# oksuman/sorting-fhe

Measured on AMD Instinct MI355X. Metric: encrypted rank-sort homomorphic comparisons/s (N^2 per DirectSort<N>::sort), higher is better.
Workload: dtype u64 (RNS residues, 40/60-bit primes); 1 GPU; directsort_n256_2e16; N=256, ring_dim=65536, mult_depth=34, scale_bits=40, parallelism=replicas x1

## Files before the change

### sorting-fhe_amd/csrc/core/chebyshev.cpp

```cpp
#include <algorithm>
#include <cmath>
#include <cstdio>
#include <cstdlib>
#include <map>

#include "state.h"

namespace lbcrypto {

uint32_t ChebyshevPSDepth(uint32_t d) {
    if (d <= 1) return 1;
    if (d == 2) return 2;
    static const uint32_t ub[] = {5, 13, 27, 59, 119, 247, 495, 1007, 2031, 4031, 8127, 16255, 32511, 65023};
    for (uint32_t i = 0; i < sizeof(ub) / sizeof(ub[0]); ++i)
        if (d <= ub[i]) return 3 + i;
    SFHE_THROW("Chebyshev degree too large");
}

std::vector<double> EvalChebyshevCoefficients(std::function<double(double)> func, double a,
                                              double b, uint32_t degree) {
    if (!degree) SFHE_THROW("degree must be positive");
    const double bMinusA = 0.5 * (b - a), bPlusA = 0.5 * (b + a);
    const double piByDeg = M_PI / (double)degree;
    std::vector<double> fx(degree);
    for (uint32_t j = 0; j < degree; ++j) fx[j] = func(std::cos(piByDeg * (j + 0.5)) * bMinusA + bPlusA);
    const uint64_t P = 4ull * degree;
    std::vector<double> ctab(P);
    for (uint64_t m = 0; m < P; ++m) ctab[m] = std::cos(M_PI * (double)m / (2.0 * degree));
    std::vector<double> c(degree, 0.0);
    const double mult = 2.0 / (double)degree;
    ParallelFor(degree, [&](size_t i) {
        double acc = 0.0;
        uint64_t step = (2ull * i) % P, idx = i % P;
        for (uint32_t j = 0; j < degree; ++j) {
            acc += fx[j] * ctab[idx];
            idx += step;
            if (idx >= P) idx -= P;
        }
        c[i] = acc * mult;
    });
    return c;
}

namespace {

using Ct = Ciphertext<DCRTPoly>;

struct Val {
    bool isConst = true;
    double c = 0.0;
    Ct ct;
    int node = -1;
};

bool psWaves() {
    static const bool on = [] {
        const char* v = std::getenv("SFHE_PS_WAVES");
        return !v || *v != '0';
    }();
    return on;
}

class PSEvaluator {
  public:
    PSEvaluator(CryptoContextImpl<DCRTPoly>* cc, const Ct& y, uint32_t l, uint32_t D)
        : cc(cc), l(l), k(1u << l), D(D) {
        T.resize(k + 1);
        T[1] = y;
        for (uint32_t half = 1; half < k; half *= 2) {
            const uint32_t lo = half + 1, hi = std::min(k, 2 * half);
            std::vector<Ct> as, bs;
            for (uint32_t j = lo; j <= hi; ++j) {
                as.push_back(doubled(j / 2));
                bs.push_back(j % 2 == 0 ? T[j / 2] : T[j / 2 + 1]);
            }
            std::vector<Ct> prods;
            if (psWaves()) {
                prods = cc->EvalMultMany(as, bs);
            } else {
                for (size_t i = 0; i < as.size(); ++i) prods.push_back(cc->EvalMult(as[i], bs[i]));
            }
            for (uint32_t j = lo; j <= hi; ++j) {
                const Ct& prod = prods[j - lo];
                T[j] = (j % 2 == 0) ? cc->EvalAdd(prod, -1.0) : cc->EvalSub(prod, atLevel(1, prod->GetLevel()));
            }
        }
        giant[l] = T[k];
    }

    void precomputeLeaves(const std::vector<double>& p, uint32_t depth) {
        std::vector<std::pair<std::vector<double>, uint32_t>> leaves;
        plan(p, depth, 0, leaves);
        std::map<uint32_t, std::vector<size_t>> byLevel;
        for (size_t i = 0; i < leaves.size(); ++i) byLevel[leaves[i].second].push_back(i);
        pre.assign(leaves.size(), nullptr);
        for (auto& kv : byLevel) {
            const uint32_t L = kv.first;
            std::vector<uint32_t> js;
            for (uint32_t j = 1; j <= k; ++j)
                for (size_t i : kv.second)
                    if (j < leaves[i].first.size() && leaves[i].first[j] != 0.0) {
                        js.push_back(j);
                        break;
                    }
            std::vector<const uint64_t*> ins0, ins1;
            std::vector<double> sc;
            std::vector<DeviceBufferPtr> keep;
            for (uint32_t j : js) {
                const Ct& t = T[j];
                const uint64_t *r0, *r1;
                cc->RowsAt(t, L, &r0, &r1, keep);
                ins0.push_back(r0);
                ins1.push_back(r1);
                sc.push_back(t->scale);
            }
            for (size_t b0 = 0; b0 < kv.second.size(); b0 += 64) {
                std::vector<std::vector<double>> w;
                const size_t b1 = std::min(kv.second.size(), b0 + 64);
                for (size_t t = b0; t < b1; ++t) {
                    const auto& pl = leaves[kv.second[t]].first;
                    std::vector<double> row;
                    for (uint32_t j : js) row.push_back(j < pl.size() ? pl[j] : 0.0);
                    w.push_back(std::move(row));
                }
                auto cts = cc->LinearWSumRescaleMulti(ins0, ins1, w, L, T[1]->GetSlots(), &sc);
                for (size_t t = b0; t < b1; ++t) pre[kv.second[t]] = cts[t - b0];
            }
        }
        nextLeaf = 0;
    }

    Val eval(std::vector<double> p, uint32_t depth, uint32_t want = 0, int lane = 0, int span = 1) {
        trim(p);
        if (p.empty()) return Val{true, 0.0, nullptr};
        const uint32_t deg = (uint32_t)p.size() - 1;
        if (deg == 0) return Val{true, p[0], nullptr};
        if (deg <= k) return leaf(p, want);
        if (depth >= 1 && deg + (1u << l) <= (1u << (depth - 1))) return eval(p, depth - 1, want, lane, span);
        const uint32_t M = deg >= (1u << (depth - 1)) ? (1u << (depth - 1)) : (1u << (depth - 2));
        std::vector<double> q, r;
        divide(p, M, q, r);
        const uint32_t Lp = productLevel(q, depth, M, want);
        const int half = span / 2;
        if (half) cc->SetLane(lane + half);
        Val qv = eval(q, depth - 1, Lp - 1, half ? lane + half : lane, half ? half : 1);
        const Ct& TM = alignedPower(M, Lp - 1);
        Val out;
        out.isConst = false;
        if (qv.isConst)
            out.ct = cc->EvalMult(TM, qv.c);
        else
            out.ct = cc->EvalMult(qv.ct, TM);
        if (half) cc->SetLane(lane);
        Val rv = eval(r, depth, Lp, lane, half ? half : 1);
        if (std::getenv("SFHE_PS_DEBUG"))
            std::fprintf(stderr, "PSNODE deg %u M %u | q %s lvl %d | TM lvl %u | prod lvl %u | r %s lvl %d\n", deg, M,
                         qv.isConst ? "const" : "ct", qv.isConst ? -1 : (int)qv.ct->GetLevel(), TM->GetLevel(),
                         out.ct->GetLevel(), rv.isConst ? "const" : "ct", rv.isConst ? -1 : (int)rv.ct->GetLevel());
        if (rv.isConst) {
            if (rv.c != 0.0) out.ct = cc->EvalAdd(out.ct, rv.c);
        } else {
            out.ct = cc->EvalAdd(out.ct, rv.ct);
        }
        return out;
    }

    Val build(std::vector<double> p, uint32_t depth, uint32_t want = 0) {
        trim(p);
        if (p.empty()) return Val{true, 0.0, nullptr};
        const uint32_t deg = (uint32_t)p.size() - 1;
        if (deg == 0) return Val{true, p[0], nullptr};
        if (deg <= k) return leaf(p, want);
        if (depth >= 1 && deg + (1u << l) <= (1u << (depth - 1))) return build(p, depth - 1, want);
        const uint32_t M = deg >= (1u << (depth - 1)) ? (1u << (depth - 1)) : (1u << (depth - 2));
        std::vector<double> q, r;
        divide(p, M, q, r);
        const uint32_t Lp = productLevel(q, depth, M, want);
        Node nd;
        nd.q = build(q, depth - 1, Lp - 1);
        nd.r = build(r, depth, Lp);
        nd.M = M;
        nd.Lp = Lp;
        nodes.push_back(std::move(nd));
        Val v;
        v.isConst = false;
        v.node = (int)nodes.size() - 1;
        return v;
    }

    Val run(const Val& root) {
        if (root.node < 0) return root;
        auto ready = [&](const Val& v) { return v.isConst || v.node < 0 || nodes[v.node].hasOut; };
        auto value = [&](const Val& v) -> const Ct& { return v.node < 0 ? v.ct : nodes[v.node].out; };
        while (!nodes[root.node].hasOut) {
            bool progress = false;
            std::map<std::pair<uint32_t, uint32_t>, std::vector<size_t>> waves;
            for (size_t i = 0; i < nodes.size(); ++i)
                if (!nodes[i].hasProd && ready(nodes[i].q)) waves[{nodes[i].M, nodes[i].Lp}].push_back(i);
            for (auto& w : waves) {
                const Ct& TM = alignedPower(w.first.first, w.first.second - 1);
                std::vector<Ct> as, bs;
                std::vector<size_t> which;
                for (size_t i : w.second) {
                    Node& nd = nodes[i];
                    if (nd.q.isConst) {
                        nd.prod = cc->EvalMult(TM, nd.q.c);
                        nd.hasProd = true;
                        continue;
                    }
                    as.push_back(value(nd.q));
                    bs.push_back(TM);
                    which.push_back(i);
                }
                auto prods = cc->EvalMultMany(as, bs);
                for (size_t t = 0; t < which.size(); ++t) {
                    nodes[which[t]].prod = prods[t];
                    nodes[which[t]].hasProd = true;
                }
                progress = true;
            }
            std::vector<Node*> sums;
            for (auto& nd : nodes)
                if (!nd.hasOut && nd.hasProd && ready(nd.r)) sums.push_back(&nd);
            for (size_t b0 = 0; b0 < sums.size(); b0 += batchWidth()) {
                const size_t b1 = std::min(sums.size(), b0 + batchWidth());
                BatchScope bs(cc, (uint32_t)(b1 - b0));
                for (size_t t = b0; t < b1; ++t) {
                    Node& nd = *sums[t];
                    bs.lane((uint32_t)(t - b0));
                    if (nd.r.isConst)
                        nd.out = nd.r.c != 0.0 ? cc->EvalAdd(nd.prod, nd.r.c) : nd.prod;
                    else
                        nd.out = cc->EvalAdd(nd.prod, value(nd.r));
                    nd.hasOut = true;
                    nd.prod = nullptr;
                }
                progress = true;
            }
            if (!progress) SFHE_THROW("internal: Chebyshev wave evaluation stalled");
        }
        Val out;
        out.isConst = false;
        out.ct = nodes[root.node].out;
        nodes.clear();
        return out;
    }

  private:
    struct Node {
        Val q, r;
        uint32_t M = 0, Lp = 0;
        Ct prod, out;
        bool hasProd = false, hasOut = false;
    };
    std::vector<Node> nodes;

    static void divide(const std::vector<double>& p, uint32_t M, std::vector<double>& q, std::vector<double>& r) {
        const uint32_t deg = (uint32_t)p.size() - 1;
        q.assign(deg - M + 1, 0.0);
        r.assign(p.begin(), p.begin() + M);
        for (uint32_t j = M; j <= deg; ++j) {
            if (j == M) {
                q[0] += p[j];
            } else {
                q[j - M] += 2.0 * p[j];
                r[2 * M - j] -= p[j];
            }
        }
    }

    void plan(std::vector<double> p, uint32_t depth, uint32_t want,
              std::vector<std::pair<std::vector<double>, uint32_t>>& leaves) {
        trim(p);
        if (p.size() <= 1) return;
        const uint32_t deg = (uint32_t)p.size() - 1;
        if (deg <= k) {
            const int lv = leafSumLevel(p, want);
            if (lv >= 0) leaves.emplace_back(p, (uint32_t)lv);
            return;
        }
        if (depth >= 1 && deg + (1u << l) <= (1u << (depth - 1))) return plan(p, depth - 1, want, leaves);
        const uint32_t M = deg >= (1u << (depth - 1)) ? (1u << (depth - 1)) : (1u << (depth - 2));
        std::vector<double> q, r;
        divide(p, M, q, r);
        const uint32_t Lp = productLevel(q, depth, M, want);
        plan(q, depth - 1, Lp - 1, leaves);
        plan(r, depth, Lp, leaves);
    }

    uint32_t productLevel(const std::vector<double>& q, uint32_t depth, uint32_t M, uint32_t want) const {
        if (naturalOnly()) want = 0;
        const int nq = natural(q, depth - 1);
        const uint32_t nat = (uint32_t)std::max(nq, (int)powerLevel(M)) + 1;
        return std::max(nat, want);
    }

    int natural(std::vector<double> p, uint32_t depth) const {
        trim(p);
        if (p.size() <= 1) return -1;
        const uint32_t deg = (uint32_t)p.size() - 1;
        if (deg <= k) {
            const int lv = leafSumLevel(p, 0);
            return lv < 0 ? -1 : lv + 1;
        }
        if (depth >= 1 && deg + (1u << l) <= (1u << (depth - 1))) return natural(p, depth - 1);
        const uint32_t M = deg >= (1u << (depth - 1)) ? (1u << (depth - 1)) : (1u << (depth - 2));
        std::vector<double> q, r;
        divide(p, M, q, r);
        const int lp = (int)productLevel(q, depth, M, 0);
        return std::max(lp, natural(r, depth));
    }

    int leafSumLevel(const std::vector<double>& p, uint32_t want) const {
        if (naturalOnly()) want = 0;
        int lev = -1;
        for (uint32_t j = 1; j < p.size(); ++j)
            if (p[j] != 0.0) lev = std::max(lev, (int)T[j]->GetLevel());
        if (lev < 0) return -1;
        return std::max(lev, (int)want - 1);
    }

    static bool naturalOnly() {
        static const bool on = [] {
            const char* v = std::getenv("SFHE_PS_NATURAL");
            return v && *v == '1';
        }();
        return on;
    }

    static void trim(std::vector<double>& p) {
        while (!p.empty() && p.back() == 0.0) p.pop_back();
    }

    uint32_t powerLevel(uint32_t M) const {
        if (M <= k) return T[M]->GetLevel();
        return powerLevel(M / 2) + 1;
    }

    const Ct& power(uint32_t M) {
        if (M <= k) return T[M];
        uint32_t i = (uint32_t)__builtin_ctz(M);
        auto it = giant.find(i);
        if (it != giant.end()) return it->second;
        const Ct& half = power(M / 2);
        const Ct twice = cc->EvalAdd(half, half);
        return giant[i] = cc->EvalAdd(cc->EvalMult(twice, half), -1.0);
    }

    const Ct& doubled(uint32_t j) {
        auto it = twice.find(j);
        if (it != twice.end()) return it->second;
        return twice[j] = cc->EvalAdd(T[j], T[j]);
    }

    const Ct& alignedPower(uint32_t M, uint32_t level) {
        const Ct& t = power(M);
        if (t->GetLevel() >= level) return t;
        auto key = std::make_pair(M, level);
        auto it = alignedPow.find(key);
        if (it != alignedPow.end()) return it->second;
        return alignedPow[key] = cc->AdjustLevel(t, level);
    }

    const Ct& atLevel(uint32_t j, uint32_t level) {
        auto key = std::make_pair(j, level);
        auto it = aligned.find(key);
        if (it != aligned.end()) return it->second;
        return aligned[key] = (T[j]->GetLevel() == level ? T[j] : cc->AdjustLevel(T[j], level));
    }

    Val leaf(const std::vector<double>& p, uint32_t want) {
        if (!pre.empty()) {
            bool any = false;
            for (uint32_t j = 1; j < p.size(); ++j) any = any || p[j] != 0.0;
            if (!any) return Val{true, p[0], nullptr};
            if (nextLeaf >= pre.size()) SFHE_THROW("internal: Chebyshev leaf plan mismatch");
            Val out;
            out.isConst = false;
            out.ct = pre[nextLeaf];
            pre[nextLeaf++] = nullptr;
            if (p[0] != 0.0) out.ct = cc->EvalAdd(out.ct, p[0]);
            return out;
        }
        const int lv = leafSumLevel(p, want);
        if (lv < 0) return Val{true, p[0], nullptr};
        std::vector<const uint64_t*> ins0, ins1;
        std::vector<double> w, sc;
        std::vector<DeviceBufferPtr> keep;
        for (uint32_t j = 1; j < p.size(); ++j) {
            if (p[j] == 0.0) continue;
            const Ct& t = T[j];
            const uint64_t *r0, *r1;
            cc->RowsAt(t, (uint32_t)lv, &r0, &r1, keep);
            ins0.push_back(r0);
            ins1.push_back(r1);
            w.push_back(p[j]);
            sc.push_back(t->scale);
        }
        Val out;
        out.isConst = false;
        out.ct = cc->LinearWSumRescale(ins0, ins1, w, (uint32_t)lv, T[1]->GetSlots(), &sc);
        if (p[0] != 0.0) out.ct = cc->EvalAdd(out.ct, p[0]);
        return out;
    }

    CryptoContextImpl<DCRTPoly>* cc;
    uint32_t l, k, D;
    std::vector<Ct> pre;
    size_t nextLeaf = 0;
    std::vector<Ct> T;
    std::map<uint32_t, Ct> giant;
    std::map<std::pair<uint32_t, uint32_t>, Ct> aligned, alignedPow;
    std::map<uint32_t, Ct> twice;
};

}

Ciphertext<DCRTPoly> CryptoContextImpl<DCRTPoly>::EvalChebyshevSeriesPS(
    const Ciphertext<DCRTPoly>& x, const std::vector<double>& coeffs, double a, double b) {
    OpLock g(st.get());
    static const bool lazyPs = [] {
        const char* v = std::getenv("SFHE_LAZY_PS");
        return v && *v == '1';
    }();
    struct Hold {
        SfheContextState* s;
        bool on;
        ~Hold() {
            if (on) --s->lazyHold;
        }
    } hold{st.get(), !lazyPs};
    if (hold.on) ++st->lazyHold;
    std::vector<double> p(coeffs);
    while (!p.empty() && p.back() == 0.0) p.pop_back();
    if (p.empty()) SFHE_THROW("empty Chebyshev series");
    p[0] *= 0.5;
    Ciphertext<DCRTPoly> y = x;
    if (a != -1.0 || b != 1.0) {
        y = EvalMult(x, 2.0 / (b - a));
        y = EvalAdd(y, -(a + b) / (b - a));
    }
    const uint32_t d = (uint32_t)p.size() - 1;
    if (d == 0) return EvalAdd(EvalMult(y, 0.0), p[0]);
    const uint32_t D = ChebyshevPSDepth(d);
    uint32_t bestL = 1;
    double bestCost = 1e300;
    for (uint32_t l = 1; l + 1 <= D && l <= 6; ++l) {
        if ((1ull << D) - (1ull << l) < d) continue;
        double cost = (double)((1u << l) - 1) + (double)(D - 1 - l) + std::ceil((double)d / (1u << l));
        if (cost < bestCost) {
            bestCost = cost;
            bestL = l;
        }
    }
    static const uint32_t forceL = [] {
        const char* v = std::getenv("SFHE_PS_L");
        return v ? (uint32_t)std::atoi(v) : 0u;
    }();
    if (forceL && d >= 64 && (1ull << D) - (1ull << forceL) >= d && forceL + 1 <= D) bestL = forceL;
    const uint32_t l = std::min(bestL, (uint32_t)(31 - __builtin_clz(std::max<uint32_t>(d, 2))));
    Ciphertext<DCRTPoly> out;
    {
        static const int psLanes = [] {
            const char* v = std::getenv("SFHE_PS_LANES");
            return v ? std::atoi(v) : 0;
        }();
        int lanes = 1;
        if (psLanes > 1 && !st->forkedLanes && d >= 64) {
            lanes = std::min(psLanes, LaneCount());
            lanes = lanes >= 4 ? 4 : (lanes >= 2 ? 2 : 1);
        }
        struct LaneRegion {
            CryptoContextImpl<DCRTPoly>* cc;
            int lanes;
            LaneRegion(CryptoContextImpl<DCRTPoly>* c, int k) : cc(c), lanes(k) {
                if (lanes > 1) cc->ForkLanes(lanes);
            }
            ~LaneRegion() {
                if (lanes > 1) {
                    cc->SetLane(0);
                    cc->JoinLanes();
                }
            }
        } region(this, lanes);
        PSEvaluator ps(this, y, l, D);
        static const bool batched = std::getenv("SFHE_PS_UNBATCHED") == nullptr;
        if (batched) ps.precomputeLeaves(p, D);
        auto v = (lanes == 1 && psWaves()) ? ps.run(ps.build(p, D)) : ps.eval(p, D, 0, 0, lanes);
        out = v.isConst ? EvalAdd(EvalMult(y, 0.0), v.c) : v.ct;
    }
    const uint32_t target = y->GetLevel() + D;
    if (out->GetLevel() > target)
        SFHE_THROW("internal: Chebyshev evaluation exceeded OpenFHE depth");
    if (out->GetLevel() < target) out = AdjustLevel(out, target);
    return out;
}

Ciphertext<DCRTPoly> CryptoContextImpl<DCRTPoly>::EvalChebyshevFunction(
    std::function<double(double)> f, const Ciphertext<DCRTPoly>& x, double a, double b,
    uint32_t degree) {
    auto c = EvalChebyshevCoefficients(f, a, b, degree + 1);
    return EvalChebyshevSeriesPS(x, c, a, b);
}

Ciphertext<DCRTPoly> CryptoContextImpl<DCRTPoly>::EvalPolyLinear(
    const Ciphertext<DCRTPoly>& x, const std::vector<double>& coeffs) {
    OpLock g(st.get());
    std::vector<double> p(coeffs);
    while (!p.empty() && p.back() == 0.0) p.pop_back();
    if (p.size() < 2) SFHE_THROW("EvalPolyLinear needs degree >= 1");
    const uint32_t d = (uint32_t)p.size() - 1;
    std::vector<char> need(d + 1, 0);
    for (uint32_t j = d; j >= 1; --j)
        if (p[j] != 0.0 || need[j]) {
            need[j] = 1;
            if (j >= 2) need[j / 2] = need[j - j / 2] = 1;
        }
    std::vector<Ciphertext<DCRTPoly>> pw(d + 1);
    pw[1] = x;
    for (uint32_t half = 1; half < d; half *= 2) {
        std::vector<Ciphertext<DCRTPoly>> as, bs;
        std::vector<uint32_t> js;
        for (uint32_t j = half + 1; j <= std::min(d, 2 * half); ++j)
            if (need[j]) {
                as.push_back(pw[j / 2]);
                bs.push_back(pw[j - j / 2]);
                js.push_back(j);
            }
        if (psWaves()) {
            auto prods = EvalMultMany(as, bs);
            for (size_t t = 0; t < js.size(); ++t) pw[js[t]] = prods[t];
        } else {
            for (size_t t = 0; t < js.size(); ++t) pw[js[t]] = EvalMult(as[t], bs[t]);
        }
    }
    uint32_t lev = 0;
    for (uint32_t j = 1; j <= d; ++j)
        if (p[j] != 0.0) lev = std::max(lev, pw[j]->GetLevel());
    std::vector<const uint64_t*> i0, i1;
    std::vector<double> w, sc;
    std::vector<DeviceBufferPtr> keep;
    for (uint32_t j = 1; j <= d; ++j) {
        if (p[j] == 0.0) continue;
        const uint64_t *r0, *r1;
        RowsAt(pw[j], lev, &r0, &r1, keep);
        i0.push_back(r0);
        i1.push_back(r1);
        w.push_back(p[j]);
        sc.push_back(pw[j]->scale);
    }
    auto out = LinearWSumRescale(i0, i1, w, lev, x->GetSlots(), &sc);
    if (p[0] != 0.0) out = EvalAdd(out, p[0]);
    return out;
}

}
```

### sorting-fhe_amd/csrc/core/context.cpp

```cpp
#include <algorithm>
#include <atomic>
#include <cmath>
#include <cstdio>
#include <cstdlib>
#include <cstring>
#include <random>

#include "state.h"

namespace lbcrypto {

namespace {

u64 mulmod(u64 a, u64 b, u64 m) { return (u64)((u128)a * b % m); }
u64 powmod(u64 a, u64 e, u64 m) {
    u64 r = 1 % m;
    a %= m;
    while (e) {
        if (e & 1) r = mulmod(r, a, m);
        a = mulmod(a, a, m);
        e >>= 1;
    }
    return r;
}
// ... 333 lines not shown
        if (!lazy(s) || !(isLazy(a) || isLazy(b))) return nullptr;
        const Ct* lz[2] = {&a, &b};
        bool liftIdx[2] = {false, false};
        if (isLazy(a) && isLazy(b)) {
            if (a->level != b->level) return nullptr;
        } else {
            const Ct& c = isLazy(a) ? b : a;
            const Ct& p = isLazy(a) ? a : b;
            if (c->level >= p->level) return nullptr;
            liftIdx[isLazy(a) ? 1 : 0] = true;
        }
        const uint32_t level = a->level > b->level ? a->level : b->level;
        for (int i = 0; i < 2; ++i) {
            materialize(**lz[i], !liftIdx[i]);
            s->dep((*lz[i])->buf.get());
        }
        const uint32_t ell = s->ellOf(level) + 1;
        const sfp_limbs m = s->qmap(ell);
        Ct out = newPendingCt(cc, level, std::max(a->slots, b->slots));
        const uint64_t* x0[2];
        const uint64_t* x1[2];
        std::vector<u64> w(2 * (size_t)m.count);
        DeviceBufferPtr gathered;
        for (int i = 0; i < 2; ++i) {
            const Ct& c = *lz[i];
            x0[i] = c->c0;
            x1[i] = c->c1;
            if (liftIdx[i] && s->shardAt(s->ellOf(c->level)) && !s->shardAt(ell)) {
                gathered = gatherRows(s, c->c0, c->c1, ell);
                x0[i] = gathered->ptr;
                x1[i] = gathered->ptr + (size_t)ell * s->n;
            }
            const std::vector<u64> k = liftIdx[i] ? constResidues(s, s->preScale(level) / c->scale, ell)
                                                  : std::vector<u64>(m.count, 1);
            for (uint32_t r = 0; r < m.count; ++r) {
                const u64 q = s->primes[s->qprime(r, ell)];
                w[(size_t)i * m.count + r] = (sub && i == 1) ? (k[r] ? q - k[r] : 0) : k[r];
            }
        }
        sfp_lin_wsum_multi(s->dev, out->c0, 0, (size_t)(out->c1 - out->c0), x0, x1, 2, w.data(), 1, m);
        s->stats.add++;
        s->countBytes(6.0 * ell * s->n * 8);
        return out;
    }

    static sfp_limbs Q(uint32_t ell) { return sfp_limbs{ell, ell, 0}; }
    static bool packed(const SfheContextState* s, std::initializer_list<const uint64_t*> c0s,
                       std::initializer_list<const uint64_t*> c1s, uint32_t level) {
        const size_t pw = s->polyWords(level);
        auto a = c0s.begin();
        for (auto b = c1s.begin(); b != c1s.end(); ++a, ++b)
            if (*b != *a + pw) return false;
        return true;
    }
    static sfp_limbs both(const SfheContextState* s, uint32_t ell) {
        sfp_limbs m = s->qmap(ell);
        m.count *= 2;
        m.pbase = m.base;
        return m;
    }
    static sfp_limbs Range(uint32_t lo, uint32_t cnt) { return sfp_limbs{cnt, 0, lo}; }

    static Ct newCt(CC* cc, uint32_t level, uint32_t slots) {
        SfheContextState* s = cc->st.get();
        auto ct = std::make_shared<CiphertextImpl<DCRTPoly>>();
        const size_t pw = s->polyWords(level);
        ct->cc = cc->shared_from_this();
        ct->buf = s->alloc(2 * pw);
        ct->c0 = ct->buf->ptr;
        ct->c1 = ct->c0 + pw;
        ct->level = level;
        ct->slots = slots;
        ct->scale = s->scale[level];
        return ct;
    }

    static std::vector<u64> constResidues(SfheContextState* s, double v, uint32_t ell) {
        std::vector<u64> k(s->rows(ell));
        for (uint32_t i = 0; i < k.size(); ++i) k[i] = residueOf(v, s->primes[s->qprime(i, ell)]);
        return k;
    }

    static Ct rescale(CC* cc, const uint64_t* c0, const uint64_t* c1, uint32_t level,
                      uint32_t slots) {
        SfheContextState* s = cc->st.get();
        uint32_t ell = s->ellOf(level);
        if (ell < 2) SFHE_THROW("no levels left to rescale (multiplicative depth exhausted)");
        Ct out = newCt(cc, level + 1, slots);
        if (c1 - c0 < 0) SFHE_THROW("internal: layout");
        if (s->shardAt(ell))
            rescaleShard(s, out->c0, c0, ell, 2, (size_t)(c1 - c0), (size_t)(out->c1 - out->c0));
        else
            sfp_rescale(s->dev, out->c0, c0, ell, s->qInvTable[ell].data(), 2, (size_t)(c1 - c0),
                        (size_t)(out->c1 - out->c0));
        s->stats.rescale++;
        s->countBytes(4.0 * ell * s->n * 8 * 2 / 2);
        return out;
    }

    static Ct adjust(CC* cc, const Ct& ct, uint32_t target, double factor = 1.0) {
        SfheContextState* s = cc->st.get();
        if (target == ct->level && factor == 1.0) return ct;
        if (target <= ct->level && factor != 1.0) SFHE_THROW("a scaled adjustment needs a level to consume");
        if (target < ct->level) SFHE_THROW("cannot raise a ciphertext's level");
        if (target > s->L) SFHE_THROW("target level beyond multiplicative depth");
        uint32_t mid = target - 1;
        uint32_t ell = s->ellOf(mid);
        double K = factor * s->scale[target] * (double)s->primes[ell - 1] / ct->scale;
        auto k = constResidues(s, K, ell);
        s->stats.constmult++;
        s->countBytes(4.0 * ell * s->n * 8);
        if (s->shardAt(s->ellOf(ct->level)) && !s->shardAt(ell)) {
            auto full = gatherRows(s, ct->c0, ct->c1, ell);
            auto v = view(cc, full, full->ptr, full->ptr + (size_t)ell * s->n, ct->level, ct->scale, ct->slots);
            return mulRescale(cc, v, mid, k.data(), nullptr, ct->slots);
        }
        return mulRescale(cc, ct, mid, k.data(), nullptr, ct->slots);
    }

    static bool fusedRescale() {
        static const bool on = [] {
            const char* v = std::getenv("SFHE_FUSED_RESCALE");
            return !v || *v != '0';
        }();
        return on;
    }

    static Ct mulRescale(CC* cc, const Ct& ct, uint32_t level, const u64* k, const uint64_t* m,
                         uint32_t slots) {
        SfheContextState* s = cc->st.get();
        const uint32_t ell = s->ellOf(level);
        if (ell < 2) SFHE_THROW("no levels left to rescale (multiplicative depth exhausted)");
        if (!fusedRescale() || s->shardAt(ell)) {
            const size_t pw = s->polyWords(level);
            auto tmp = s->alloc(2 * pw);
            uint64_t* t0 = tmp->ptr;
            uint64_t* t1 = t0 + pw;
            if (k) {
                sfp_mul_const(s->dev, t0, ct->c0, k, s->qmap(ell));
                sfp_mul_const(s->dev, t1, ct->c1, k, s->qmap(ell));
            } else {
                sfp_mul(s->dev, t0, ct->c0, m, s->qmap(ell));
                sfp_mul(s->dev, t1, ct->c1, m, s->qmap(ell));
            }
            return rescale(cc, t0, t1, level, slots);
        }
        Ct out = newCt(cc, level + 1, slots);
        const size_t inStride = (size_t)(ct->c1 - ct->c0), outStride = (size_t)(out->c1 - out->c0);
        if (k)
            sfp_mul_const_rescale(s->dev, out->c0, ct->c0, k, ell, s->qInvTable[ell].data(), 2, inStride,
                                  outStride);
        else
            sfp_mul_rescale(s->dev, out->c0, ct->c0, m, ell, s->qInvTable[ell].data(), 2, inStride,
                            outStride);
        s->stats.rescale++;
        s->countBytes(4.0 * ell * s->n * 8 * 2 / 2);
        return out;
    }

    static void align(CC* cc, Ct& a, Ct& b) {
        uint32_t l = std::max(a->level, b->level);
        a = adjust(cc, a, l);
        b = adjust(cc, b, l);
    }

    static std::vector<uint32_t> naturalOrder(const SfheContextState* s, uint32_t count, uint32_t per,
                                              uint32_t blocks = 1, uint32_t block = 0) {
        std::vector<uint32_t> r(count);
        for (uint32_t g = 0; g < count; ++g)
            r[g] = ((g % s->world) * blocks + block) * per + g / s->world;
        return r;
    }

    static DeviceBufferPtr gatherRows(SfheContextState* s, const uint64_t* c0, const uint64_t* c1, uint32_t ell) {
// ... 231 lines not shown
        const uint32_t lo = s->owned(ell - 1);
        std::vector<u64> qlinv(lo);
        for (uint32_t i = 0; i < lo; ++i) qlinv[i] = s->qInvTable[ell][s->qprimeShard(i)];
        if (s->shardAt(ell - 1)) {
            sfp_rescale_rows(s->dev, out, in, last->ptr, drop, s->shardMap(ell - 1), qlinv.data(), npoly, inStride,
                             outStride, n);
            return;
        }
        const uint32_t per = (ell - 1 + s->world - 1) / s->world;
        auto mine = s->alloc((size_t)npoly * per * n);
        sfp_rescale_rows(s->dev, mine->ptr, in, last->ptr, drop, s->shardMap(ell - 1), qlinv.data(), npoly, inStride,
                         (size_t)per * n, n);
        auto all = s->alloc((size_t)npoly * per * s->world * n);
        sfp_allgather(s->dev, mine->ptr, all->ptr, (size_t)npoly * per * n * 8);
        for (uint32_t p = 0; p < npoly; ++p) {
            auto idx = naturalOrder(s, ell - 1, per, npoly, p);
            sfp_gather_rows(s->dev, out + p * outStride, all->ptr, idx.data(), ell - 1);
        }
    }

    static Ct localize(CC* cc, const Ct& full) {
        SfheContextState* s = cc->st.get();
        const uint32_t ell = s->ellOf(full->level);
        if (!s->shardAt(ell)) return full;
        const uint32_t lr = s->rows(ell);
        Ct out = newCt(cc, full->level, full->slots);
        out->scale = full->scale;
        std::vector<uint32_t> idx(lr);
        for (uint32_t i = 0; i < lr; ++i) idx[i] = s->qprimeShard(i);
        sfp_gather_rows(s->dev, out->c0, full->c0, idx.data(), lr);
        sfp_gather_rows(s->dev, out->c1, full->c1, idx.data(), lr);
        return out;
    }

    static DeviceBufferPtr gatherFull(SfheContextState* s, const Ct& a) {
        const uint32_t ell = s->ellOf(a->level);
        if (s->shardAt(ell)) return gatherRows(s, a->c0, a->c1, ell);
        auto full = s->alloc((size_t)2 * ell * s->n);
        sfp_d2d(s->dev, full->ptr, a->c0, (size_t)ell * s->n * 8);
        sfp_d2d(s->dev, full->ptr + (size_t)ell * s->n, a->c1, (size_t)ell * s->n * 8);
        return full;
    }

    static int modupInner(CC* cc, uint64_t* acc, const uint64_t* d, uint32_t ell, const DeviceBufferPtr& key,
                          const uint64_t* fold0, const uint64_t* fold1, u64 foldK, int accum,
                          uint32_t invFrom = ~0u) {
        SfheContextState* s = cc->st.get();
        const uint32_t n = s->n, K = s->Kof(key->ksTier);
        const uint32_t beta = (ell + s->alpha - 1) / s->alpha;
        const size_t stride = (size_t)(ell + K) * n;
        auto ext = s->alloc(stride * beta);
        auto scratch = s->alloc((size_t)ell * n);
        auto& convs = modupConv(cc, ell, key->ksTier);
        if (sfp_modup_inner(s->dev, acc, acc + stride, d, ell, K, s->Lq, s->alpha, convs.data(), key->ptr, fold0,
                            fold1, foldK, accum, invFrom, ext->ptr, scratch->ptr) == 0)
            return invFrom != ~0u;
        sfp_modup(s->dev, ext->ptr, d, ell, K, s->Lq, s->alpha, convs.data(), scratch->ptr);
        if (fold0)
            sfp_ks_inner_fold(s->dev, acc, acc + stride, ext->ptr, stride, key->ptr, beta, ell, K, s->Lq, fold0, fold1,
                              foldK);
        else
            (accum ? sfp_ks_inner_acc : sfp_ks_inner)(s->dev, acc, acc + stride, ext->ptr, stride, key->ptr, beta,
                                                       ell, K, s->Lq);
        return 0;
    }

    static void keySwitch(CC* cc, const uint64_t* d, uint32_t ell, const DeviceBufferPtr& key,
                          uint64_t* out0, uint64_t* out1, int add0, int add1) {
        SfheContextState* s = cc->st.get();
        if (s->shardAt(ell)) return keySwitchShard(cc, d, ell, key, out0, out1, add0, add1);
        const int tier = key->ksTier;
        const uint32_t n = s->n, K = s->Kof(tier);
        const uint32_t beta = (ell + s->alpha - 1) / s->alpha;
        const size_t stride = (size_t)(ell + K) * n;
        auto acc = s->alloc(2 * stride);
        const int rowDone = modupInner(cc, acc->ptr, d, ell, key, nullptr, nullptr, 0, 0, ell);
        auto md = s->alloc((size_t)2 * ell * n);
        sfp_moddown2(s->dev, out0, out1, acc->ptr, stride, ell, K, s->Lq, s->moddownConvOf(tier), s->pInvModQof(tier),
                     add0, add1, md->ptr, rowDone);
        s->stats.keyswitch++;
        s->countBytes((3.0 * ell + 2.0 * beta * (ell + K)) * n * 8);
    }

    static Ct relinRescale(CC* cc, uint64_t* d0, uint64_t* d1, const uint64_t* d2, uint32_t level,
                           uint32_t slots) {
        SfheContextState* s = cc->st.get();
        const uint32_t ell = s->ellOf(level);
        if (ell < 2) SFHE_THROW("no levels left to rescale (multiplicative depth exhausted)");
        if (s->shardAt(ell)) {
            keySwitchShard(cc, d2, ell, s->relinKey, d0, d1, 1, 1);
            return rescale(cc, d0, d1, level, slots);
        }
        const DeviceBufferPtr& key = s->relinFor(ell);
        const int tier = key->ksTier;
        const uint32_t n = s->n, K = s->Kof(tier);
        const uint32_t beta = (ell + s->alpha - 1) / s->alpha;
        const size_t stride = (size_t)(ell + K) * n;
        auto acc = s->alloc(2 * stride);
        const int rowDone = modupInner(cc, acc->ptr, d2, ell, key, d0, d1, s->pModQof(tier)[ell - 1], 0, ell - 1);
        Ct out = newCt(cc, level + 1, slots);
        auto scratch = s->alloc((size_t)2 * (ell - 1) * n);
        sfp_moddown_rescale(s->dev, out->c0, out->c1, d0, d1, acc->ptr, stride, ell, K, s->Lq,
                            s->moddownConvOf(tier), s->pInvModQof(tier), s->pModQof(tier),
                            s->qInvTable[ell].data(), scratch->ptr, rowDone);
        s->stats.keyswitch++;
        s->stats.rescale++;
        s->countBytes((3.0 * ell + 2.0 * beta * (ell + K)) * n * 8);
        s->countBytes(4.0 * ell * n * 8);
        return out;
    }

    static Ct multRelinRescale(CC* cc, const uint64_t* a0, const uint64_t* a1, const uint64_t* b0,
                               const uint64_t* b1, uint32_t level, uint32_t slots) {
        SfheContextState* s = cc->st.get();
        const uint32_t ell = s->ellOf(level);
        if (ell < 2) SFHE_THROW("no levels left to rescale (multiplicative depth exhausted)");
        const size_t pw = s->polyWords(level);
        if (!s->shardAt(ell)) {
            const DeviceBufferPtr& key = s->relinFor(ell);
            const int tier = key->ksTier;
            const uint32_t n = s->n, K = s->Kof(tier), beta = (ell + s->alpha - 1) / s->alpha;
            const size_t stride = (size_t)(ell + K) * n;
            Ct out = newCt(cc, level + 1, slots);
            auto acc = s->alloc(2 * stride);
            auto ext = s->alloc(stride * beta);
            auto scratch = s->alloc((size_t)2 * ell * n);
            auto& convs = modupConv(cc, ell, tier);
            if (sfp_mult_relin_rescale(s->dev, out->c0, out->c1, a0, a1, b0, b1, ell, K, s->Lq, s->alpha,
                                       convs.data(), key->ptr, s->moddownConvOf(tier), s->pInvModQof(tier),
                                       s->pModQof(tier), s->qInvTable[ell].data(), acc->ptr, ext->ptr,
                                       scratch->ptr) == 0) {
                s->stats.keyswitch++;
                s->stats.rescale++;
                s->countBytes((3.0 * ell + 2.0 * beta * (ell + K)) * n * 8);
                s->countBytes(4.0 * ell * n * 8);
                return out;
            }
        }
        auto t = s->alloc(3 * pw);
        uint64_t* d0 = t->ptr;
        uint64_t* d1 = d0 + pw;
        uint64_t* d2 = d1 + pw;
        sfp_tensor(s->dev, d0, d1, d2, a0, a1, b0, b1, s->qmap(ell));
        return relinRescale(cc, d0, d1, d2, level, slots);
    }

    static std::vector<Ct> multRelinRescaleMany(CC* cc, const std::vector<const CiphertextImpl<DCRTPoly>*>& a,
                                                const std::vector<const CiphertextImpl<DCRTPoly>*>& b, uint32_t level,
                                                const std::vector<uint32_t>& slots) {
        SfheContextState* s = cc->st.get();
        const size_t cnt = a.size();
        const uint32_t ell = s->ellOf(level);
        std::vector<Ct> out(cnt);
        if (ell < 2) SFHE_THROW("no levels left to rescale (multiplicative depth exhausted)");
        const DeviceBufferPtr& key = s->relinFor(ell);
        const int tier = key->ksTier;
        const uint32_t n = s->n, K = s->Kof(tier), beta = (ell + s->alpha - 1) / s->alpha;
        const size_t stride = (size_t)(ell + K) * n;
        auto& convs = modupConv(cc, ell, tier);
        size_t done = 0;
        {
        BatchScope bs(cc, s->shardAt(ell) ? 0 : (uint32_t)cnt);
        if (bs) {
            for (; done < cnt; ++done) {
                out[done] = newCt(cc, level + 1, slots[done]);
                auto acc = s->alloc(2 * stride);
                auto ext = s->alloc(stride * beta);
                auto scratch = s->alloc((size_t)2 * ell * n);
                bs.lane((uint32_t)done);
                if (sfp_mult_relin_rescale(s->dev, out[done]->c0, out[done]->c1, a[done]->c0, a[done]->c1,
                                           b[done]->c0, b[done]->c1, ell, K, s->Lq, s->alpha, convs.data(),
                                           key->ptr, s->moddownConvOf(tier), s->pInvModQof(tier), s->pModQof(tier),
                                           s->qInvTable[ell].data(), acc->ptr, ext->ptr, scratch->ptr) != 0)
                    break;
                s->stats.keyswitch++;
                s->stats.rescale++;
                s->countBytes((3.0 * ell + 2.0 * beta * (ell + K)) * n * 8);
                s->countBytes(4.0 * ell * n * 8);
            }
        }
        }
        for (size_t i = done; i < cnt; ++i)
            out[i] = multRelinRescale(cc, a[i]->c0, a[i]->c1, b[i]->c0, b[i]->c1, level, slots[i]);
        return out;
    }

    static void innerAndModDown(CC* cc, const uint64_t* ext, size_t stride, uint32_t beta,
                                uint32_t ell, const DeviceBufferPtr& key, uint64_t* out0,
                                uint64_t* out1, int add0, int add1, uint32_t gal = 0) {
        SfheContextState* s = cc->st.get();
        if (s->shardAt(ell)) {
            if (gal) SFHE_THROW("internal: a permuted inner product at a sharded level");
            return innerModDownShard(s, ext, stride, beta, ell, key, out0, out1, add0, add1);
        }
        const int tier = key->ksTier;
        const uint32_t n = s->n, K = s->Kof(tier);
        const size_t accStride = (size_t)(ell + K) * n;
        if (stride != accStride) SFHE_THROW("internal: extended digits of another special-prime tier");
        auto acc = s->alloc(2 * accStride);
        if (gal)
            sfp_ks_inner_aut(s->dev, acc->ptr, acc->ptr + accStride, ext, stride, key->ptr, beta, ell, K, s->Lq, gal);
        else
            sfp_ks_inner(s->dev, acc->ptr, acc->ptr + accStride, ext, stride, key->ptr, beta, ell, K, s->Lq);
        auto scratch = s->alloc((size_t)2 * ell * n);
        sfp_moddown2(s->dev, out0, out1, acc->ptr, accStride, ell, K, s->Lq, s->moddownConvOf(tier),
                     s->pInvModQof(tier), add0, add1, scratch->ptr, 0);
    }

    static std::vector<sfp_conv*>& modupConv(CC* cc, uint32_t ell, int tier = -1) {
        SfheContextState* s = cc->st.get();
        auto& cache = tier < 0 ? s->modupConv : s->tiers[(size_t)tier].modupConv;
        auto it = cache.find(ell);
        if (it != cache.end()) return it->second;
        std::vector<sfp_conv*> v;
        const uint32_t K = s->Kof(tier);
        uint32_t beta = (ell + s->alpha - 1) / s->alpha;
        for (uint32_t j = 0; j < beta; ++j) {
            uint32_t lo = j * s->alpha, hi = std::min(lo + s->alpha, ell);
            std::vector<uint32_t> src, dst, row;
            for (uint32_t i = lo; i < hi; ++i) src.push_back(i);
            for (uint32_t i = 0; i < ell; ++i)
                if (i < lo || i >= hi) dst.push_back(i);
            for (uint32_t k = 0; k < K; ++k) dst.push_back(s->Lq + k);
            for (uint32_t p : dst) row.push_back(p < s->Lq ? p : ell + (p - s->Lq));
            v.push_back(makeConv(s, src, dst, row.data()));
        }
        return cache[ell] = v;
    }

    static void buildTiers(SfheContextState* s) {
        const char* v = std::getenv("SFHE_KS_TIERS");
        const std::string spec = v ? v : "2,4,6,8,10";
        std::vector<uint32_t> bounds;
        for (size_t i = 0; i < spec.size();) {
            size_t j = spec.find(',', i);
            if (j == std::string::npos) j = spec.size();
            const long b = std::strtol(spec.substr(i, j - i).c_str(), nullptr, 10);
            if (b > 0) bounds.push_back((uint32_t)b);
            i = j + 1;
        }
        std::sort(bounds.begin(), bounds.end());
        for (uint32_t b : bounds) {
            if (b > s->alpha || b > s->Lq) break;
            double bits = 0;
            for (uint32_t i = 0; i < b; ++i) bits += std::log2((double)s->primes[i]);
            uint32_t K = 0;
            for (double bp = 0; bp < bits + 20.0 && K < s->K; ++K) bp += std::log2((double)s->primes[s->Lq + K]);
            if (K + 1 >= s->K || (!s->tiers.empty() && K <= s->tiers.back().K)) continue;
            KsTier t;
            t.maxEll = b;
            t.K = K;
            t.pModQ.resize(s->Lq);
            t.pInvModQ.resize(s->Lq);
            for (uint32_t i = 0; i < s->Lq; ++i) {
                const u64 qi = s->primes[i];
                u64 pr = 1;
                for (uint32_t k = 0; k < K; ++k) pr = mulmod(pr, s->primes[s->Lq + k] % qi, qi);
                t.pModQ[i] = pr;
                t.pInvModQ[i] = invmod(pr, qi);
            }
            std::vector<uint32_t> src, dst;
            for (uint32_t k = 0; k < K; ++k) src.push_back(s->Lq + k);
            for (uint32_t i = 0; i < s->Lq; ++i) dst.push_back(i);
            t.moddownConv = makeConv(s, src, dst);
            s->tiers.push_back(std::move(t));
        }
// ... 1473 lines not shown
    const uint64_t* m = SfheInternal::encoded(this, p, a->level);
    return SfheInternal::traced(
        this, SfheInternal::mulRescale(this, a, a->level, nullptr, m, std::max(a->slots, p->slots)), "EvalMult");
}

void CryptoContextImpl<DCRTPoly>::EvalMultInPlace(Ciphertext<DCRTPoly>& a, const Plaintext& p) {
    a = EvalMult(a, p);
}

Ciphertext<DCRTPoly> CryptoContextImpl<DCRTPoly>::EvalMult(const Ciphertext<DCRTPoly>& a0,
                                                          const Ciphertext<DCRTPoly>& b0) {
    OpLock g(st.get());
    SfheInternal::deps(st.get(), {&a0, &b0});
    SfheContextState* s = st.get();
    if (!s->relinKey) SFHE_THROW("EvalMultKeyGen must be called before EvalMult");
    auto a = a0, b = b0;
    SfheInternal::align(this, a, b);
    const uint32_t ell = s->ellOf(a->level);
    if (ell < 2) SFHE_THROW("no levels left (multiplicative depth exhausted)");
    const size_t pw = s->polyWords(a->level);
    s->stats.tensor++;
    s->countBytes(7.0 * ell * s->n * 8);
    const uint32_t slots = std::max(a->slots, b->slots);
    if (SfheInternal::lazy(s) && SfheInternal::fusedRescale()) {
        auto op = std::make_shared<DeferredRelin>();
        op->pa = a->buf;
        op->pb = b->buf;
        op->a0 = a->c0;
        op->a1 = a->c1;
        op->b0 = b->c0;
        op->b1 = b->c1;
        op->level = a->level;
        op->slots = slots;
        return SfheInternal::deferredCt(this, a->level + 1, slots, op);
    }
    if (SfheInternal::fusedRescale())
        return SfheInternal::traced(
            this, SfheInternal::multRelinRescale(this, a->c0, a->c1, b->c0, b->c1, a->level, slots), "EvalMult");
    auto t = s->alloc(3 * pw);
    uint64_t* d0 = t->ptr;
    uint64_t* d1 = d0 + pw;
    uint64_t* d2 = d1 + pw;
    sfp_tensor(s->dev, d0, d1, d2, a->c0, a->c1, b->c0, b->c1, st->qmap(ell));
    SfheInternal::keySwitch(this, d2, ell, s->relinFor(ell), d0, d1, 1, 1);
    return SfheInternal::traced(this, SfheInternal::rescale(this, d0, d1, a->level, slots), "EvalMult");
}

Ciphertext<DCRTPoly> CryptoContextImpl<DCRTPoly>::EvalSquare(const Ciphertext<DCRTPoly>& a) {
    return EvalMult(a, a);
}

std::vector<Ciphertext<DCRTPoly>> CryptoContextImpl<DCRTPoly>::EvalMultMany(
    const std::vector<Ciphertext<DCRTPoly>>& a0, const std::vector<Ciphertext<DCRTPoly>>& b0) {
    OpLock g(st.get());
    SfheContextState* s = st.get();
    if (a0.size() != b0.size()) SFHE_THROW("operand count mismatch");
    const size_t cnt = a0.size();
    std::vector<Ciphertext<DCRTPoly>> out(cnt);
    if (cnt < 2 || !SfheInternal::fusedRescale()) {
        for (size_t i = 0; i < cnt; ++i) out[i] = EvalMult(a0[i], b0[i]);
        return out;
    }
    if (!s->relinKey) SFHE_THROW("EvalMultKeyGen must be called before EvalMult");
    std::vector<Ciphertext<DCRTPoly>> A(a0), B(b0);
    for (size_t i = 0; i < cnt; ++i) {
        SfheInternal::deps(s, {&a0[i], &b0[i]});
        SfheInternal::align(this, A[i], B[i]);
        if (s->ellOf(A[i]->level) < 2) SFHE_THROW("no levels left (multiplicative depth exhausted)");
        s->stats.tensor++;
        s->countBytes(7.0 * s->ellOf(A[i]->level) * s->n * 8);
    }
    for (size_t i = 0; i < cnt;) {
        size_t j = i + 1;
        while (j < cnt && j - i < batchWidth() && A[j]->level == A[i]->level) ++j;
        std::vector<const CiphertextImpl<DCRTPoly>*> pa, pb;
        std::vector<uint32_t> slots;
        for (size_t k = i; k < j; ++k) {
            pa.push_back(A[k].get());
            pb.push_back(B[k].get());
            slots.push_back(std::max(A[k]->slots, B[k]->slots));
        }
        auto r = SfheInternal::multRelinRescaleMany(this, pa, pb, A[i]->level, slots);
        for (size_t k = i; k < j; ++k) out[k] = SfheInternal::traced(this, r[k - i], "EvalMult");
        i = j;
    }
    return out;
}

Ciphertext<DCRTPoly> CryptoContextImpl<DCRTPoly>::EvalMultAddPlain(
    const std::vector<Ciphertext<DCRTPoly>>& a, const std::vector<Plaintext>& p) {
    OpLock g(st.get());
    SfheInternal::depsv(st.get(), a);
    SfheContextState* s = st.get();
    if (a.empty() || a.size() != p.size()) SFHE_THROW("operand count mismatch");
    uint32_t level = 0, slots = 0;
    for (size_t i = 0; i < a.size(); ++i) {
        level = std::max(level, a[i]->level);
        slots = std::max(slots, std::max(a[i]->slots, p[i]->slots));
    }
    const uint32_t ell = s->ellOf(level);
    if (ell < 2) SFHE_THROW("no levels left (multiplicative depth exhausted)");
    std::vector<Ciphertext<DCRTPoly>> al(a.size());
    std::vector<const uint64_t*> x0, x1, m;
    for (size_t i = 0; i < a.size(); ++i) {
        al[i] = SfheInternal::adjust(this, a[i], level);
        x0.push_back(al[i]->c0);
        x1.push_back(al[i]->c1);
    }
    s->stats.ptmult += a.size();
    if (SfheInternal::lazy(s)) {
        auto op = std::make_shared<DeferredMacPlain>();
        for (auto& c : al) op->pins.push_back(c->buf);
        op->x0 = x0;
        op->x1 = x1;
        op->pts = p;
        op->level = level;
        op->slots = slots;
        s->countBytes((3.0 * a.size() + 2.0) * ell * s->n * 8);
        return SfheInternal::deferredCt(this, level + 1, slots, op);
    }
    SfheInternal::encodeBatch(this, p, level);
    for (size_t i = 0; i < a.size(); ++i) m.push_back(SfheInternal::encoded(this, p[i], level));
    const size_t pw = s->polyWords(level);
    auto tmp = s->alloc(2 * pw);
    uint64_t* t0 = tmp->ptr;
    uint64_t* t1 = t0 + pw;
    for (size_t done = 0; done < a.size(); done += SFP_MAX_WSUM) {
        uint32_t take = (uint32_t)std::min<size_t>(SFP_MAX_WSUM, a.size() - done);
        if (done == 0) {
            sfp_mac_plain2(s->dev, t0, t1, x0.data(), x1.data(), m.data(), take, st->qmap(ell));
        } else {
            auto part = s->alloc(2 * pw);
            sfp_mac_plain2(s->dev, part->ptr, part->ptr + pw, x0.data() + done, x1.data() + done,
                           m.data() + done, take, st->qmap(ell));
            sfp_add(s->dev, t0, t0, part->ptr, st->qmap(ell));
            sfp_add(s->dev, t1, t1, part->ptr + pw, st->qmap(ell));
        }
    }
    s->countBytes((3.0 * a.size() + 2.0) * ell * s->n * 8);
    return SfheInternal::traced(this, SfheInternal::rescale(this, t0, t1, level, slots), "EvalMultAddPlain");
}


Ciphertext<DCRTPoly> CryptoContextImpl<DCRTPoly>::EvalRotate(const Ciphertext<DCRTPoly>& a,
                                                            int32_t r) {
    OpLock g(st.get());
    SfheContextState* s = st.get();
    if (!(SfheInternal::lazy(s) && SfheInternal::isLazy(a))) SfheInternal::deps(s, {&a});
    uint32_t gal = GaloisForRotation(r);
    if (gal == 1) return a->Clone();
    if (!s->rotKeys.count(gal))
        SFHE_THROW("EvalKey for index [" + std::to_string(gal) + "] (rotation " +
                   std::to_string(r) + ") is not found");
    const bool pend = SfheInternal::lazy(s) && SfheInternal::isLazy(a);
    if (pend) {
        SfheInternal::materialize(*a, true);
        s->dep(a->buf.get());
    }
    const uint32_t ell = SfheInternal::ctEll(s, *a);
    auto out = pend ? SfheInternal::newPendingCt(this, a->level, a->slots) : SfheInternal::newCt(this, a->level, a->slots);
    auto t = s->alloc((size_t)s->rows(ell) * s->n);
    sfp_automorph(s->dev, out->c0, a->c0, gal, st->qmap(ell));
    sfp_automorph(s->dev, t->ptr, a->c1, gal, st->qmap(ell));
    s->stats.automorph++;
    s->countBytes(3.0 * ell * s->n * 8);
    SfheInternal::keySwitch(this, t->ptr, ell, *s->rotFor(gal, ell), out->c0, out->c1, 1, 0);
// ... 257 lines not shown
                auto scratch = s->alloc((size_t)ell * n);
                sfp_modup(s->dev, ext->ptr, a[t]->c1, ell, K, s->Lq, s->alpha,
                          SfheInternal::modupConv(this, ell).data(), scratch->ptr);
            }
            auto rc0 = s->alloc(pw);
            sfp_automorph(s->dev, rc0->ptr, a[t]->c0, gal, q);
            x0.push_back(rc0->ptr);
            m0.push_back(m);
            keep.push_back(rc0);
            static const bool autFused = [] {
                const char* v = std::getenv("SFHE_KS_AUT");
                return !v || *v != '0';
            }();
            if (autFused) {
                sfp_ks_inner_mul_aut(s->dev, acc->ptr, acc->ptr + stride, ext->ptr, stride, it->second->ptr, beta, ell,
                                     K, s->Lq, SfheInternal::encodedExt(this, pt, level), accOn ? 1 : 0, gal);
            } else {
                auto rext = s->alloc(stride * beta);
                const uint32_t rows = beta * (ell + K);
                sfp_automorph(s->dev, rext->ptr, ext->ptr, gal, sfp_limbs{rows, rows, 0, 0});
                sfp_ks_inner_mul(s->dev, acc->ptr, acc->ptr + stride, rext->ptr, stride, it->second->ptr, beta, ell,
                                 K, s->Lq, SfheInternal::encodedExt(this, pt, level), accOn ? 1 : 0);
            }
            accOn = true;
            s->stats.keyswitch++;
            s->stats.automorph++;
            s->countBytes((3.0 * ell + (2.0 * beta + 5.0) * (ell + K)) * n * 8);
        }
    }
    auto macInto = [&](uint64_t* out, const std::vector<const uint64_t*>& x, const std::vector<const uint64_t*>& m) {
        if (x.empty()) {
            sfp_zero(s->dev, out, pw * 8);
            return;
        }
        for (size_t done = 0; done < x.size(); done += SFP_MAX_WSUM) {
            const uint32_t take = (uint32_t)std::min<size_t>(SFP_MAX_WSUM, x.size() - done);
            if (done == 0) {
                sfp_mac_plain(s->dev, out, x.data(), m.data(), take, q);
            } else {
                auto part = s->alloc(pw);
                sfp_mac_plain(s->dev, part->ptr, x.data() + done, m.data() + done, take, q);
                sfp_add(s->dev, out, out, part->ptr, q);
            }
        }
    };
    macInto(t0, x0, m0);
    macInto(t1, x1, m1);
    s->stats.ptmult += x0.size() + x1.size();
    s->countBytes((2.0 * x0.size() + 2.0 * x1.size() + 2.0) * ell * n * 8);
    if (accOn) {
        auto scratch = s->alloc((size_t)2 * ell * n);
        sfp_moddown2(s->dev, t0, t1, acc->ptr, stride, ell, K, s->Lq, s->moddownConv, s->pInvModQ.data(), 1, 1,
                     scratch->ptr, 0);
    }
    return SfheInternal::traced(this, SfheInternal::rescale(this, t0, t1, level, slots), "EvalRotMultAddHoisted");
}


namespace {
void weightResidues(const SfheContextState* s, double w, uint32_t level, uint32_t ell,
                    std::vector<uint64_t>& kk, double inScale = 0.0) {
    const double K = inScale > 0.0 ? w * s->scale[level] * (s->scale[level] / inScale) : w * s->scale[level];
    const double r = std::nearbyint(K);
    const bool neg = r < 0;
    const double a = std::fabs(r);
    u128 v;
    if (a < 1.8e19) {
        v = (u128)(u64)a;
    } else {
        const double hi = std::floor(std::ldexp(a, -64));
        v = ((u128)(u64)hi << 64) + (u128)(u64)(a - std::ldexp(hi, 64));
    }
    for (uint32_t i = 0; i < s->rows(ell); ++i) {
        const u64 q = s->primes[s->qprime(i, ell)];
        const u64 m = (u64)(v % q);
        kk.push_back(neg ? (m ? q - m : 0) : m);
    }
}
}

std::vector<Ciphertext<DCRTPoly>> CryptoContextImpl<DCRTPoly>::LinearWSumRescaleMulti(
    const std::vector<const uint64_t*>& in0, const std::vector<const uint64_t*>& in1,
    const std::vector<std::vector<double>>& w, uint32_t level, uint32_t slots, const std::vector<double>* inScale) {
    OpLock g(st.get());
    SfheContextState* s = st.get();
    const uint32_t ell = s->ellOf(level), n = s->n;
    const uint32_t nin = (uint32_t)in0.size(), nout = (uint32_t)w.size();
    if (ell < 2) SFHE_THROW("no levels left (multiplicative depth exhausted)");
    if (nin == 0 || nin > SFP_MAX_WSUM || nout == 0) SFHE_THROW("LinearWSumRescaleMulti: bad sizes");
    if (inScale && inScale->size() != nin) SFHE_THROW("LinearWSumRescaleMulti: scale count");
    std::vector<uint64_t> kk;
    kk.reserve((size_t)nout * nin * s->rows(ell));
    for (const auto& row : w) {
        if (row.size() != nin) SFHE_THROW("LinearWSumRescaleMulti: weight row size");
        for (uint32_t j = 0; j < nin; ++j) weightResidues(s, row[j], level, ell, kk, inScale ? (*inScale)[j] : 0.0);
    }
    const size_t pw = s->polyWords(level);
    auto sums = s->alloc((size_t)nout * 2 * pw);
    sfp_lin_wsum_multi(s->dev, sums->ptr, 2 * pw, pw, in0.data(), in1.data(), nin, kk.data(), nout,
                       s->qmap(ell));
    const size_t qw = s->polyWords(level + 1);
    auto res = s->alloc((size_t)nout * 2 * qw);
    if (s->shardAt(ell))
        SfheInternal::rescaleShard(s, res->ptr, sums->ptr, ell, 2 * nout, pw, qw);
    else
        sfp_rescale(s->dev, res->ptr, sums->ptr, ell, s->qInvTable[ell].data(), 2 * nout, pw, qw);
    std::vector<Ciphertext<DCRTPoly>> out(nout);
    for (uint32_t o = 0; o < nout; ++o) {
        auto ct = std::make_shared<CiphertextImpl<DCRTPoly>>();
        ct->cc = shared_from_this();
        ct->buf = res;
        ct->c0 = res->ptr + (size_t)o * 2 * qw;
        ct->c1 = ct->c0 + qw;
        ct->level = level + 1;
        ct->slots = slots;
        ct->scale = s->scale[level + 1];
        out[o] = ct;
    }
    s->stats.wsum_terms += (uint64_t)nin * nout;
    s->stats.rescale += 2 * nout;
    s->countBytes(((double)nin + nout) * 2.0 * pw * 8 + 4.0 * pw * 8 * nout);
    return out;
}

Ciphertext<DCRTPoly> CryptoContextImpl<DCRTPoly>::LinearWSumRescale(
    const std::vector<const uint64_t*>& in0, const std::vector<const uint64_t*>& in1,
    const std::vector<double>& w, uint32_t level, uint32_t slots, const std::vector<double>* inScale) {
    OpLock g(st.get());
    SfheContextState* s = st.get();
    const uint32_t ell = s->ellOf(level);
    if (ell < 2) SFHE_THROW("no levels left (multiplicative depth exhausted)");
    if (inScale && inScale->size() != w.size()) SFHE_THROW("LinearWSumRescale: scale count");
    const size_t pw = s->polyWords(level);
    auto tmp = s->alloc(2 * pw);
    uint64_t* t0 = tmp->ptr;
    uint64_t* t1 = t0 + pw;
    const sfp_limbs q = s->qmap(ell);
    size_t done = 0;
    bool first = true;
    while (done < w.size()) {
        size_t take = std::min<size_t>(w.size() - done, SFP_MAX_WSUM - (first ? 0 : 1));
        std::vector<const uint64_t*> a0, a1;
        std::vector<uint64_t> kk;
        if (!first) {
            a0.push_back(t0);
            a1.push_back(t1);
            for (uint32_t i = 0; i < s->rows(ell); ++i) kk.push_back(1);
        }
        for (size_t j = done; j < done + take; ++j) {
            a0.push_back(in0[j]);
            a1.push_back(in1[j]);
            weightResidues(s, w[j], level, ell, kk, inScale ? (*inScale)[j] : 0.0);
        }
        sfp_lin_wsum(s->dev, t0, a0.data(), kk.data(), (uint32_t)a0.size(), q);
        sfp_lin_wsum(s->dev, t1, a1.data(), kk.data(), (uint32_t)a1.size(), q);
        s->stats.wsum_terms += take;
        s->countBytes((double)(a0.size() + 1) * 2.0 * ell * s->n * 8);
        done += take;
        first = false;
    }
    return SfheInternal::traced(this, SfheInternal::rescale(this, t0, t1, level, slots), "LinearWSumRescale");
}



Ciphertext<DCRTPoly> CryptoContextImpl<DCRTPoly>::Rescale(const Ciphertext<DCRTPoly>& a) {
    Settle(a);
    return a->Clone();
}

void CryptoContextImpl<DCRTPoly>::Settle(const Ciphertext<DCRTPoly>& ct) {
    if (!ct) return;
    OpLock g(st.get());
    SfheInternal::deps(st.get(), {&ct});
}

void CryptoContextImpl<DCRTPoly>::LevelReduceInPlace(Ciphertext<DCRTPoly>& a, std::nullptr_t,
                                                     size_t levels) {
    a = AdjustLevel(a, a->level + (uint32_t)levels);
}

Ciphertext<DCRTPoly> CryptoContextImpl<DCRTPoly>::AdjustLevel(const Ciphertext<DCRTPoly>& a,
                                                             uint32_t targetLevel) {
    OpLock g(st.get());
    SfheInternal::deps(st.get(), {&a});
    auto r = SfheInternal::adjust(this, a, targetLevel);
    return r == a ? a->Clone() : r;
}

Ciphertext<DCRTPoly> CryptoContextImpl<DCRTPoly>::AdjustLevelScaled(const Ciphertext<DCRTPoly>& a,
                                                                   uint32_t targetLevel, double factor) {
    OpLock g(st.get());
    SfheInternal::deps(st.get(), {&a});
    auto r = SfheInternal::adjust(this, a, targetLevel, factor);
    return r == a ? a->Clone() : r;
}

Ciphertext<DCRTPoly> CryptoContextImpl<DCRTPoly>::ModRaise(const Ciphertext<DCRTPoly>& a) {
    OpLock g(st.get());
    SfheInternal::deps(st.get(), {&a});
    SfheContextState* s = st.get();
    if (s->sharded) SFHE_THROW("bootstrapping a limb-sharded context is not supported");
    if (s->ellOf(a->level) != 1) SFHE_THROW("ModRaise needs a ciphertext at the last level (one limb)");
    const uint32_t n = s->n;
    auto t = s->alloc(2 * (size_t)n);
    sfp_d2d(s->dev, t->ptr, a->c0, (size_t)n * 8);
    sfp_d2d(s->dev, t->ptr + n, a->c1, (size_t)n * 8);
    sfp_ntt(s->dev, t->ptr, sfp_limbs{1, 1, 0, 0, 0}, 1);
    sfp_ntt(s->dev, t->ptr + n, sfp_limbs{1, 1, 0, 0, 0}, 1);
    auto out = SfheInternal::newCt(this, 0, a->slots);
    const size_t pw = s->polyWords(0);
    auto zero = s->alloc(2 * pw);
    sfp_zero(s->dev, zero->ptr, 2 * pw * 8);
    std::vector<uint64_t> minus1(s->Lq);
    for (uint32_t i = 0; i < s->Lq; ++i) minus1[i] = s->primes[i] - 1;
    sfp_rescale_rows(s->dev, out->c0, zero->ptr, t->ptr, 0, s->qmap(s->Lq), minus1.data(), 2, pw,
                     (size_t)(out->c1 - out->c0), n);
    s->wrote(out->buf.get());
    return SfheInternal::traced(this, out, "ModRaise");
}

Ciphertext<DCRTPoly> CryptoContextImpl<DCRTPoly>::EvalConjugate(const Ciphertext<DCRTPoly>& a) {
    OpLock g(st.get());
    SfheInternal::deps(st.get(), {&a});
    SfheContextState* s = st.get();
    const uint32_t gal = 2 * s->n - 1;
    auto it = s->rotKeys.find(gal);
    if (it == s->rotKeys.end()) SFHE_THROW("conjugation key not found (EvalConjugateKeyGen)");
    const uint32_t ell = s->ellOf(a->level);
    auto out = SfheInternal::newCt(this, a->level, a->slots);
    auto t = s->alloc(s->polyWords(a->level));
    sfp_automorph(s->dev, out->c0, a->c0, gal, st->qmap(ell));
    sfp_automorph(s->dev, t->ptr, a->c1, gal, st->qmap(ell));
    s->stats.automorph++;
    SfheInternal::keySwitch(this, t->ptr, ell, it->second, out->c0, out->c1, 1, 0);
    return SfheInternal::traced(this, out, "EvalConjugate");
}

void CryptoContextImpl<DCRTPoly>::EvalConjugateKeyGen(const PrivateKey<DCRTPoly>& sk) {
    OpLock g(st.get());
    SfheContextState* s = st.get();
    const uint32_t gal = 2 * s->n - 1;
    if (s->rotKeys.count(gal)) return;
    const uint32_t NP = s->Lq + s->K;
// ... 256 lines not shown
```

### sorting-fhe_amd/csrc/core/openfhe.h

```cpp
#pragma once

#include <algorithm>
#include <charconv>
#include <complex>
#include <cstddef>
#include <locale>
#include <fstream>
#include <cstdint>
#include <functional>
#include <iostream>
#include <map>
#include <memory>
#include <mutex>
#include <set>
#include <stdexcept>
#include <string>
#include <thread>
#include <vector>

#include "prims.h"

namespace lbcrypto {

using usint = uint32_t;
// ... 203 lines not shown
class CryptoContextImpl<DCRTPoly> : public std::enable_shared_from_this<CryptoContextImpl<DCRTPoly>> {
  public:
    explicit CryptoContextImpl(const CCParams<CryptoContextCKKSRNS>& p);
    ~CryptoContextImpl();

    void Enable(PKESchemeFeature f) { enabled |= f; }
    void Enable(uint32_t mask) { enabled |= mask; }

    uint32_t GetRingDimension() const;
    uint32_t GetCyclotomicOrder() const { return 2 * GetRingDimension(); }
    EncodingParams GetEncodingParams() const;
    uint32_t GetMultiplicativeDepth() const;

    KeyPair<DCRTPoly> KeyGen();
    void EvalMultKeyGen(const PrivateKey<DCRTPoly>& sk);
    void EvalRotateKeyGen(const PrivateKey<DCRTPoly>& sk, const std::vector<int32_t>& idx,
                          const PublicKey<DCRTPoly>& pk = nullptr);
    void EvalAtIndexKeyGen(const PrivateKey<DCRTPoly>& sk, const std::vector<int32_t>& idx) {
        EvalRotateKeyGen(sk, idx);
    }
    void ClearEvalMultKeys();
    void ClearEvalAutomorphismKeys();
    static bool SerializeEvalMultKey(std::ostream& os, SerType::Kind k, const std::string& keyTag = "");
    static bool DeserializeEvalMultKey(std::istream& is, SerType::Kind k);
    static bool SerializeEvalAutomorphismKey(std::ostream& os, SerType::Kind k, const std::string& keyTag = "");
    static bool DeserializeEvalAutomorphismKey(std::istream& is, SerType::Kind k);
    uint64_t Fingerprint() const;
    uint64_t KeyTag() const;
    const CCParams<CryptoContextCKKSRNS>& GetParams() const;
    uint32_t GetEnabledMask() const { return enabled; }

    Plaintext MakeCKKSPackedPlaintext(const std::vector<double>& v, uint32_t scaleDeg = 1,
                                      uint32_t level = 0, const void* params = nullptr,
                                      uint32_t slots = 0) const;
    Plaintext MakeCKKSPackedPlaintext(const std::vector<std::complex<double>>& v,
                                      uint32_t scaleDeg = 1, uint32_t level = 0,
                                      const void* params = nullptr, uint32_t slots = 0) const;
    Ciphertext<DCRTPoly> Encrypt(const PublicKey<DCRTPoly>& pk, const Plaintext& pt);
    Ciphertext<DCRTPoly> Encrypt(const Plaintext& pt, const PublicKey<DCRTPoly>& pk) {
        return Encrypt(pk, pt);
    }
    void Decrypt(const PrivateKey<DCRTPoly>& sk, const Ciphertext<DCRTPoly>& ct, Plaintext* out);
    void Decrypt(const Ciphertext<DCRTPoly>& ct, const PrivateKey<DCRTPoly>& sk, Plaintext* out) {
        Decrypt(sk, ct, out);
    }

    Ciphertext<DCRTPoly> EvalAdd(const Ciphertext<DCRTPoly>& a, const Ciphertext<DCRTPoly>& b);
    Ciphertext<DCRTPoly> EvalAdd(const Ciphertext<DCRTPoly>& a, double c);
    Ciphertext<DCRTPoly> EvalAdd(double c, const Ciphertext<DCRTPoly>& a) { return EvalAdd(a, c); }
    Ciphertext<DCRTPoly> EvalAdd(const Ciphertext<DCRTPoly>& a, const Plaintext& p);
    Ciphertext<DCRTPoly> EvalAdd(const Plaintext& p, const Ciphertext<DCRTPoly>& a) {
        return EvalAdd(a, p);
    }
    void EvalAddInPlace(Ciphertext<DCRTPoly>& a, const Ciphertext<DCRTPoly>& b);
    void EvalAddInPlace(Ciphertext<DCRTPoly>& a, double c);
    void EvalAddInPlace(Ciphertext<DCRTPoly>& a, const Plaintext& p);
    Ciphertext<DCRTPoly> EvalSub(const Ciphertext<DCRTPoly>& a, const Ciphertext<DCRTPoly>& b);
    Ciphertext<DCRTPoly> EvalSub(const Ciphertext<DCRTPoly>& a, double c) { return EvalAdd(a, -c); }
    Ciphertext<DCRTPoly> EvalSub(double c, const Ciphertext<DCRTPoly>& a);
    Ciphertext<DCRTPoly> EvalSub(const Ciphertext<DCRTPoly>& a, const Plaintext& p);
    Ciphertext<DCRTPoly> EvalSub(const Plaintext& p, const Ciphertext<DCRTPoly>& a);
    void EvalSubInPlace(Ciphertext<DCRTPoly>& a, const Ciphertext<DCRTPoly>& b);
    void EvalSubInPlace(Ciphertext<DCRTPoly>& a, double c) { EvalAddInPlace(a, -c); }
    Ciphertext<DCRTPoly> EvalNegate(const Ciphertext<DCRTPoly>& a);
    void EvalNegateInPlace(Ciphertext<DCRTPoly>& a);
    Ciphertext<DCRTPoly> EvalAddMany(const std::vector<Ciphertext<DCRTPoly>>& v);

    Ciphertext<DCRTPoly> EvalMult(const Ciphertext<DCRTPoly>& a, const Ciphertext<DCRTPoly>& b);
    Ciphertext<DCRTPoly> EvalMult(const Ciphertext<DCRTPoly>& a, double c);
    Ciphertext<DCRTPoly> EvalMult(double c, const Ciphertext<DCRTPoly>& a) { return EvalMult(a, c); }
    Ciphertext<DCRTPoly> EvalMult(const Ciphertext<DCRTPoly>& a, const Plaintext& p);
    Ciphertext<DCRTPoly> EvalMult(const Plaintext& p, const Ciphertext<DCRTPoly>& a) {
        return EvalMult(a, p);
    }
    void EvalMultInPlace(Ciphertext<DCRTPoly>& a, double c);
    void EvalMultInPlace(Ciphertext<DCRTPoly>& a, const Plaintext& p);
    Ciphertext<DCRTPoly> EvalMultAndRelinearize(const Ciphertext<DCRTPoly>& a,
                                                const Ciphertext<DCRTPoly>& b) {
        return EvalMult(a, b);
    }
    Ciphertext<DCRTPoly> EvalSquare(const Ciphertext<DCRTPoly>& a);
    std::vector<Ciphertext<DCRTPoly>> EvalMultMany(const std::vector<Ciphertext<DCRTPoly>>& a,
                                                   const std::vector<Ciphertext<DCRTPoly>>& b);
    Ciphertext<DCRTPoly> EvalMultAddPlain(const std::vector<Ciphertext<DCRTPoly>>& a,
                                          const std::vector<Plaintext>& p);

    Ciphertext<DCRTPoly> EvalRotate(const Ciphertext<DCRTPoly>& a, int32_t r);
    Ciphertext<DCRTPoly> EvalAtIndex(const Ciphertext<DCRTPoly>& a, int32_t r) {
        return EvalRotate(a, r);
    }
    std::shared_ptr<FastRotationPrecomp> EvalFastRotationPrecompute(const Ciphertext<DCRTPoly>& a);
    Ciphertext<DCRTPoly> EvalFastRotation(const Ciphertext<DCRTPoly>& a, int32_t r, uint32_t m,
                                          const std::shared_ptr<FastRotationPrecomp>& pre);
    Ciphertext<DCRTPoly> EvalRotateSum(const std::vector<Ciphertext<DCRTPoly>>& a,
                                       const std::vector<int32_t>& r);
    Ciphertext<DCRTPoly> EvalRotMultAddHoisted(
        const std::vector<Ciphertext<DCRTPoly>>& a,
        const std::vector<std::vector<std::pair<int32_t, Plaintext>>>& terms);

    Ciphertext<DCRTPoly> EvalChebyshevSeriesPS(const Ciphertext<DCRTPoly>& x,
                                               const std::vector<double>& coeffs, double a,
                                               double b);
    Ciphertext<DCRTPoly> EvalChebyshevSeries(const Ciphertext<DCRTPoly>& x,
                                             const std::vector<double>& coeffs, double a,
                                             double b) {
        return EvalChebyshevSeriesPS(x, coeffs, a, b);
    }
    Ciphertext<DCRTPoly> EvalChebyshevFunction(std::function<double(double)> f,
                                               const Ciphertext<DCRTPoly>& x, double a, double b,
                                               uint32_t degree);
    Ciphertext<DCRTPoly> EvalPolyLinear(const Ciphertext<DCRTPoly>& x,
                                        const std::vector<double>& coeffs);
    Ciphertext<DCRTPoly> EvalPoly(const Ciphertext<DCRTPoly>& x,
                                  const std::vector<double>& coeffs) {
        return EvalPolyLinear(x, coeffs);
    }

    Ciphertext<DCRTPoly> Rescale(const Ciphertext<DCRTPoly>& a);
    Ciphertext<DCRTPoly> ModReduce(const Ciphertext<DCRTPoly>& a) { return Rescale(a); }
    void LevelReduceInPlace(Ciphertext<DCRTPoly>& a, std::nullptr_t, size_t levels);
    Ciphertext<DCRTPoly> AdjustLevel(const Ciphertext<DCRTPoly>& a, uint32_t targetLevel);
    Ciphertext<DCRTPoly> AdjustLevelScaled(const Ciphertext<DCRTPoly>& a, uint32_t targetLevel, double factor);
    Ciphertext<DCRTPoly> ModRaise(const Ciphertext<DCRTPoly>& a);
    Ciphertext<DCRTPoly> EvalConjugate(const Ciphertext<DCRTPoly>& a);
    void EvalConjugateKeyGen(const PrivateKey<DCRTPoly>& sk);

    void EvalBootstrapSetup(std::vector<uint32_t> levelBudget, std::vector<uint32_t> dim1 = {0, 0},
                            uint32_t slots = 0, uint32_t correctionFactor = 0);
    void EvalBootstrapKeyGen(const PrivateKey<DCRTPoly>& sk, uint32_t slots);
    Ciphertext<DCRTPoly> EvalBootstrap(const Ciphertext<DCRTPoly>& ct, uint32_t numIterations = 1,
                                       uint32_t precision = 0);
    uint32_t GetBootstrapDepth(const std::vector<uint32_t>& levelBudget, uint32_t slots = 0) const;
    Ciphertext<DCRTPoly> BootstrapOnce(const Ciphertext<DCRTPoly>& ct, double inFactor, double outFactor);
    Ciphertext<DCRTPoly> bootstrapIters(const Ciphertext<DCRTPoly>& ct, uint32_t numIterations, uint32_t precision);
    Ciphertext<DCRTPoly> bootstrapReplay(const Ciphertext<DCRTPoly>& ct, uint32_t numIterations, uint32_t precision);
    size_t BootstrapGraphs() const;
    using BootstrapSlotMap = std::map<uint32_t, std::vector<std::complex<double>>>;
    using BootstrapTap =
        std::function<void(const char* stage, const Ciphertext<DCRTPoly>& ct, const BootstrapSlotMap* map)>;
    void SetBootstrapTap(BootstrapTap tap) { bootTap = std::move(tap); }
    static double BootstrapOverflowBound();
    static uint32_t BootstrapDoubleAngles();
    static uint32_t BootstrapChebDegree();

    SfheContextState* state() const { return st.get(); }
    uint32_t GaloisForRotation(int32_t r) const;
    bool HasRotationKey(int32_t r) const;
    Ciphertext<DCRTPoly> LinearWSumRescale(const std::vector<const uint64_t*>& in0,
                                           const std::vector<const uint64_t*>& in1,
                                           const std::vector<double>& w, uint32_t level,
                                           uint32_t slots, const std::vector<double>* inScale = nullptr);
    std::vector<Ciphertext<DCRTPoly>> LinearWSumRescaleMulti(
        const std::vector<const uint64_t*>& in0, const std::vector<const uint64_t*>& in1,
        const std::vector<std::vector<double>>& w, uint32_t level, uint32_t slots,
        const std::vector<double>* inScale = nullptr);
    void Synchronize();
    void Settle(const Ciphertext<DCRTPoly>& ct);
    int LaneCount() const;
    void EnableSharding(int rank, int world, bool shardAtOne = false);
    int ShardRank() const;
    int ShardWorld() const;
    bool IsSharded() const;
    uint32_t ShardTailLimbs() const;
    uint32_t SwitchKeyRows() const;
    void EnableBatchGroups(int group, int groups, bool gatherAtOne = false);
    int BatchGroup() const;
    int BatchGroups() const;
    bool BatchGather() const;
    std::vector<Ciphertext<DCRTPoly>> GatherGroups(const Ciphertext<DCRTPoly>& ct);
    void RowsAt(const Ciphertext<DCRTPoly>& ct, uint32_t level, const uint64_t** c0, const uint64_t** c1,
                std::vector<DeviceBufferPtr>& keep);
    void DownloadRows(const Ciphertext<DCRTPoly>& ct, uint64_t* out);
    void ForkLanes(int count, bool stacked = false);
    bool BeginBatch(uint32_t count);
    void BatchLane(uint32_t i);
    void EndBatch();
    uint32_t BatchWidth() const;
    void SetLane(int lane);
    void JoinLanes();
    void SetPlaintextCache(bool on);
    struct OpStats {
        uint64_t keyswitch = 0, rescale = 0, tensor = 0, ptmult = 0, constmult = 0, add = 0,
                 automorph = 0, ntt_limbs = 0, wsum_terms = 0;
        uint64_t dev_encodes = 0, host_encodes = 0;
        double algo_bytes = 0.0;
        uint64_t pool_bytes = 0;
    };
    OpStats GetOpStats() const;
    void ResetOpStats();
    struct CapturedGraph;
    bool BeginCapture();
    std::shared_ptr<CapturedGraph> EndCapture(const Ciphertext<DCRTPoly>& keep);
    void Launch(const std::shared_ptr<CapturedGraph>& g);
    void ReleaseGraph(CapturedGraph& g);
    static int LiveContexts();
    void releaseBootstrapGraphs();
    size_t GraphNodes(const std::shared_ptr<CapturedGraph>& g) const;
    bool GraphFamilyTime(const std::shared_ptr<CapturedGraph>& g, uint32_t family, int reps, double* ms,
                         uint64_t* launches, double* bytes);
    void CopyCiphertextInto(const Ciphertext<DCRTPoly>& dst, const Ciphertext<DCRTPoly>& src);

  private:
    std::unique_ptr<SfheContextState> st;
    uint32_t enabled = 0;
    BootstrapTap bootTap;
    friend class SfheInternal;
};

class BatchScope {
  public:
    BatchScope(CryptoContextImpl<DCRTPoly>* cc, uint32_t count)
        : cc_(cc), on_(count > 1 && cc->BeginBatch(count)) {}
    ~BatchScope() {
        if (on_) cc_->EndBatch();
    }
    BatchScope(const BatchScope&) = delete;
    BatchScope& operator=(const BatchScope&) = delete;
    explicit operator bool() const { return on_; }
    void lane(uint32_t i) {
        if (on_) cc_->BatchLane(i);
    }

  private:
    CryptoContextImpl<DCRTPoly>* cc_;
    bool on_;
};

void RegisterCryptoContext(const CryptoContext<DCRTPoly>& cc);

#define SFHE_FACADE_ABI_VERSION 5
#ifndef SFHE_LAYOUT_SALT
#define SFHE_LAYOUT_SALT 0
#endif
#pragma GCC diagnostic push
#pragma GCC diagnostic ignored "-Winvalid-offsetof"
inline uint64_t SfheFacadeLayout() {
    uint64_t h = 1469598103934665603ull;
    auto mix = [&h](uint64_t x) { h = (h ^ x) * 1099511628211ull; };
    using Ct = CiphertextImpl<DCRTPoly>;
    using Pk = PublicKeyImpl<DCRTPoly>;
    using Sk = PrivateKeyImpl<DCRTPoly>;
    using Cc = CryptoContextImpl<DCRTPoly>;
    const uint64_t v[] = {
        SFHE_FACADE_ABI_VERSION, SFHE_LAYOUT_SALT,
        sizeof(std::string), sizeof(std::mutex), sizeof(std::shared_ptr<int>), sizeof(std::vector<int>),
        sizeof(std::map<int, int>), sizeof(std::set<int>), sizeof(std::function<void()>), sizeof(std::complex<double>),
        sizeof(CCParams<CryptoContextCKKSRNS>), alignof(CCParams<CryptoContextCKKSRNS>),
        sizeof(EncodingParamsImpl), sizeof(KeyPair<DCRTPoly>),
        sizeof(PlaintextImpl), alignof(PlaintextImpl), offsetof(PlaintextImpl, values), offsetof(PlaintextImpl, slots),
        offsetof(PlaintextImpl, level), offsetof(PlaintextImpl, length), offsetof(PlaintextImpl, logPrecision),
        offsetof(PlaintextImpl, logError), offsetof(PlaintextImpl, realCache), offsetof(PlaintextImpl, encoded),
        offsetof(PlaintextImpl, encMutex),
        sizeof(Ct), alignof(Ct), offsetof(Ct, cc), offsetof(Ct, buf), offsetof(Ct, c0), offsetof(Ct, c1),
        offsetof(Ct, level), offsetof(Ct, slots), offsetof(Ct, scale), offsetof(Ct, def), offsetof(Ct, pend),
        offsetof(Ct, undo), sizeof(Ct::CaptureUndo),
        sizeof(Pk), offsetof(Pk, b), offsetof(Pk, a), offsetof(Pk, cc), offsetof(Pk, tag),
        sizeof(Sk), offsetof(Sk, s), offsetof(Sk, ternary), offsetof(Sk, cc), offsetof(Sk, tag),
        sizeof(FastRotationPrecomp), offsetof(FastRotationPrecomp, ext), offsetof(FastRotationPrecomp, level),
        offsetof(FastRotationPrecomp, pend), offsetof(FastRotationPrecomp, beta), offsetof(FastRotationPrecomp, stride),
        offsetof(FastRotationPrecomp, pinBuf), offsetof(FastRotationPrecomp, pinC0),
        sizeof(Cc), alignof(Cc), sizeof(Cc::OpStats), sizeof(Cc::BootstrapTap),
    };
    for (uint64_t x : v) mix(x);
    return h;
}
#pragma GCC diagnostic pop
void SfheCheckLayout(uint64_t callerStamp);

inline CryptoContext<DCRTPoly> GenCryptoContext(const CCParams<CryptoContextCKKSRNS>& p) {
    SfheCheckLayout(SfheFacadeLayout());
    auto cc = std::make_shared<CryptoContextImpl<DCRTPoly>>(p);
    RegisterCryptoContext(cc);
    return cc;
}

class Serial {
  public:
    static bool Serialize(const CryptoContext<DCRTPoly>& cc, std::ostream& os, SerType::Kind k);
    static bool Deserialize(CryptoContext<DCRTPoly>& cc, std::istream& is, SerType::Kind k);
    static bool Serialize(const PublicKey<DCRTPoly>& pk, std::ostream& os, SerType::Kind k);
    static bool Deserialize(PublicKey<DCRTPoly>& pk, std::istream& is, SerType::Kind k);
    static bool Serialize(const PrivateKey<DCRTPoly>& sk, std::ostream& os, SerType::Kind k);
    static bool Deserialize(PrivateKey<DCRTPoly>& sk, std::istream& is, SerType::Kind k);
    static bool Serialize(const Ciphertext<DCRTPoly>& ct, std::ostream& os, SerType::Kind k);
    static bool Deserialize(Ciphertext<DCRTPoly>& ct, std::istream& is, SerType::Kind k);

    template <class T>
    static bool SerializeToFile(const std::string& path, const T& obj, SerType::Kind k) {
        std::ofstream f(path, std::ios::out | std::ios::binary | std::ios::trunc);
        if (!f.is_open()) return false;
        return Serialize(obj, f, k) && f.good();
    }
    template <class T>
    static bool DeserializeFromFile(const std::string& path, T& obj, SerType::Kind k) {
        std::ifstream f(path, std::ios::in | std::ios::binary);
        if (!f.is_open()) return false;
        return Deserialize(obj, f, k);
    }
};

template <class E>
class CryptoContextFactory {
  public:
// ... 59 lines not shown
```

### sorting-fhe_amd/csrc/core/state.h

```cpp
#pragma once
#include <algorithm>
#include <atomic>
#include <cmath>
#include <cstdlib>
#include <cstring>
#include <map>
#include <mutex>
#include <thread>
#include <unordered_map>
#include <unordered_set>
#include <vector>

#include "modarith.h"
#include "openfhe.h"

namespace lbcrypto {

class DeviceBuffer {
  public:
    DeviceBuffer(SfheContextState* s, uint64_t* p, size_t w, int l, uint64_t r)
        : st(s), ptr(p), words(w), lane(l), region(r) {}
    ~DeviceBuffer();
    SfheContextState* st;
    uint64_t* ptr;
// ... 43 lines not shown
    uint32_t extIdx = 0;
    std::vector<uint64_t> extInvModQ;
    std::vector<uint64_t> extModQ;
    std::vector<sf_barrett> bar;
    std::vector<double> scale;
    sfp_dev* dev = nullptr;

    std::map<uint32_t, std::vector<sfp_conv*>> modupConv;
    sfp_conv* moddownConv = nullptr;
    std::vector<uint64_t> pInvModQ;
    std::vector<uint64_t> pModQ;
    std::vector<std::vector<uint64_t>> qInvTable;
    uint32_t tablePrimes() const { return Lq + K + (ext ? 1 : 0); }

    uint64_t keyTag = 0;
    DeviceBufferPtr relinKey;
    std::map<uint32_t, DeviceBufferPtr> rotKeys;
    std::set<int32_t> rotIndices;
    std::vector<KsTier> tiers;
    bool tiersReady = true;
    int tierAt(uint32_t ell) const {
        if (!tiersReady || shardAt(ell)) return -1;
        for (size_t t = 0; t < tiers.size(); ++t)
            if (ell <= tiers[t].maxEll) return (int)t;
        return -1;
    }
    uint32_t Kof(int t) const { return t < 0 ? K : tiers[(size_t)t].K; }
    const uint64_t* pModQof(int t) const { return t < 0 ? pModQ.data() : tiers[(size_t)t].pModQ.data(); }
    const uint64_t* pInvModQof(int t) const { return t < 0 ? pInvModQ.data() : tiers[(size_t)t].pInvModQ.data(); }
    sfp_conv* moddownConvOf(int t) const { return t < 0 ? moddownConv : tiers[(size_t)t].moddownConv; }
    const DeviceBufferPtr& relinFor(uint32_t ell) const {
        const int t = tierAt(ell);
        return t >= 0 && tiers[(size_t)t].relinKey ? tiers[(size_t)t].relinKey : relinKey;
    }
    const DeviceBufferPtr* rotFor(uint32_t gal, uint32_t ell) const {
        const int t = tierAt(ell);
        if (t >= 0) {
            auto it = tiers[(size_t)t].rotKeys.find(gal);
            if (it != tiers[(size_t)t].rotKeys.end()) return &it->second;
        }
        auto it = rotKeys.find(gal);
        return it == rotKeys.end() ? nullptr : &it->second;
    }
    std::map<uint32_t, std::shared_ptr<BootstrapPrecomp>> boot;

    std::mutex poolMu;
    std::map<size_t, std::vector<uint64_t*>> freeList[SFP_MAX_LANES];
    std::vector<std::pair<size_t, uint64_t*>> deferredFree;
    struct BatchFreed {
        size_t words;
        uint64_t* ptr;
        int lane;
        uint64_t region;
    };
    uint32_t batchDepth = 0;
    std::thread::id batchThread;
    std::vector<BatchFreed> batchFree;
    void poolReturn(size_t words, uint64_t* p, int lane, uint64_t region, int freer);
    std::map<size_t, std::vector<uint64_t*>> forkPool;
    int lane = 0;
    int forkedLanes = 0;
    uint64_t region = 0;
    uint64_t regionCount = 0;
    uint64_t laneSeq[SFP_MAX_LANES] = {};
    uint64_t synced[SFP_MAX_LANES][SFP_MAX_LANES] = {};
    uint64_t regionDepWaits = 0;
    void laneWait(int waiter, int waitee);
    int myLane() const;
    void setMyLane(int l);
    void dep(DeviceBuffer* b);
    void wrote(DeviceBuffer* b);
    size_t poolBytes = 0;

    std::recursive_mutex opMu;

    bool ptCacheOn = true;
    size_t ptCacheBytes = 0;
    size_t ptCacheLimit = (size_t)48 << 30;
    std::unordered_map<uint64_t, std::vector<PtCacheEntry>> ptCache;

    bool capturing = false;
    uint64_t captureEpoch = 0, epochCount = 0;
    uint32_t lazyHold = 0;
    std::set<uint64_t> abandonedEpochs;
    std::vector<std::pair<uint64_t*, size_t>> capAllocs;
    std::unordered_map<uint64_t*, bool> graphOwned;

    std::atomic<uint64_t> seedCounter{1};
    uint64_t seed = 0;
    CryptoContextImpl<DCRTPoly>::OpStats stats;

    int rank = 0, world = 1;
    int bgroup = 0, bgroups = 1;
    bool bgatherAtOne = false;
    bool sharded = false;
    uint32_t tailLimbs = 0;
    bool fullScope = false;
    std::vector<DeviceBufferPtr> scopeKeep;
    sfp_key_geom kgeom{};
    uint32_t keyRows() const { return kgeom.rows ? kgeom.rows : Lq + K; }
    std::map<uint32_t, std::vector<sfp_conv*>> modupConvShard;
    std::map<uint32_t, std::vector<std::pair<sfp_conv*, sfp_conv*>>> modupConvSplit;
    sfp_conv* moddownConvShard = nullptr;

    uint32_t ellOf(uint32_t level) const { return Lq - level; }
    double preScale(uint32_t level) const { return scale[level] * (double)primes[ellOf(level)]; }
    uint32_t owned(uint32_t count) const {
        return (uint32_t)rank < count ? (count - rank + world - 1) / world : 0;
    }
    bool shardAt(uint32_t ell) const { return sharded && ell > tailLimbs; }
    uint32_t rows(uint32_t ell) const { return shardAt(ell) ? owned(ell) : ell; }
    uint32_t prows(uint32_t ell) const { return shardAt(ell) ? owned(K) : K; }
    uint32_t qprime(uint32_t i, uint32_t ell) const { return shardAt(ell) ? rank + i * world : i; }
    uint32_t qprimeShard(uint32_t i) const { return rank + i * world; }
    sfp_limbs shardMap(uint32_t ell) const {
        return sfp_limbs{owned(ell), owned(ell), 0, (uint32_t)rank, (uint32_t)world};
    }
    sfp_limbs qmap(uint32_t ell) const { return shardAt(ell) ? shardMap(ell) : sfp_limbs{ell, ell, 0, 0, 1}; }
    sfp_limbs extmap(uint32_t ell) const {
        return shardAt(ell) ? sfp_limbs{owned(ell) + owned(K), owned(ell), Lq + (uint32_t)rank, (uint32_t)rank,
                                        (uint32_t)world}
                            : sfp_limbs{ell + K, ell, Lq, 0, 1};
    }
    size_t polyWords(uint32_t level) const { return (size_t)rows(ellOf(level)) * n; }
    uint64_t nextSeed() { return seed ^ (0x9E3779B97F4A7C15ULL * (seedCounter++)); }
    DeviceBufferPtr alloc(size_t words);
    void releaseAll();
    void countBytes(double b) { stats.algo_bytes += b; }
};

class FullScope {
  public:
    explicit FullScope(SfheContextState* s)
        : s_(s), rank_(s->rank), world_(s->world), sharded_(s->sharded), was_(s->fullScope) {
        s->rank = 0;
        s->world = 1;
        s->sharded = false;
        s->fullScope = true;
    }
    ~FullScope() {
        s_->rank = rank_;
        s_->world = world_;
        s_->sharded = sharded_;
        s_->fullScope = was_;
        if (!was_) s_->scopeKeep.clear();
    }

  private:
    SfheContextState* s_;
    int rank_, world_;
    bool sharded_, was_;
};

inline uint32_t batchWidth() {
    static const uint32_t w = [] {
        const char* v = std::getenv("SFHE_BATCH_WIDTH");
        const long x = v && *v ? std::strtol(v, nullptr, 10) : SFP_BATCH_MAX;
        return (uint32_t)std::max(2L, std::min<long>(x, SFP_BATCH_MAX));
    }();
    return w;
}

class OpLock {
  public:
    explicit OpLock(SfheContextState* s) : s_(s), g_(s->opMu) {
        s_->lane = s_->myLane();
        sfp_set_lane(s_->dev, s_->lane);
    }

  private:
    SfheContextState* s_;
    std::lock_guard<std::recursive_mutex> g_;
};

static inline uint64_t sf_splitmix64(uint64_t x) {
    x += 0x9E3779B97F4A7C15ULL;
    x = (x ^ (x >> 30)) * 0xBF58476D1CE4E5B9ULL;
    x = (x ^ (x >> 27)) * 0x94D049BB133111EBULL;
    return x ^ (x >> 31);
}

int ckks_encode(const std::vector<std::complex<double>>& v, uint32_t slots, uint32_t n,
                double scale, std::vector<int64_t>& coeffs);
void ckks_decode(const std::vector<double>& coeffs, uint32_t slots, uint32_t n,
                 std::vector<std::complex<double>>& out);
void ckks_encoder_tables(uint32_t n, const uint64_t** rot, const double** ksi);

}
```

### sorting-fhe_amd/csrc/hip/prims_hip.hip

```cpp
#include <hip/hip_runtime.h>
#include <dlfcn.h>
#include <rccl/rccl.h>

#include <algorithm>
#include <cstdio>
#include <cstdlib>
#include <cstring>
#include <functional>
#include <map>
#include <memory>
#include <mutex>
#include <unordered_set>
#include <unordered_map>
#include <string>
#include <type_traits>
#include <vector>

#include "../modarith.h"
#include "../prims.h"

#define SFP_CHECK(call)                                                     \
    do {                                                                    \
        hipError_t e_ = (call);                                             \
        if (e_ != hipSuccess) record(d, #call, e_);                          \
// ... 549 lines not shown
            }
        }
#pragma unroll
        for (int j = 0; j < M; ++j) s[a0 ^ ldsOff<COL>(j * h, Cc)] = v[j];
    }
}

template <bool INV, bool COL, int LE, int TILE>
__device__ __forceinline__ void nttRoundDynFP(int b, double* s, const NttTile& T, uint32_t S0, uint32_t k0,
                                              double q, const double* w, double qinv) {
    if constexpr (LE >= 4) {
        if (b == 4) return nttRoundFP<INV, COL, LE, 4, TILE>(s, T, S0, k0, q, w, qinv);
    }
    if constexpr (LE >= 3) {
        if (b == 3) return nttRoundFP<INV, COL, LE, 3, TILE>(s, T, S0, k0, q, w, qinv);
    }
    if (b == 2) return nttRoundFP<INV, COL, LE, 2, TILE>(s, T, S0, k0, q, w, qinv);
    nttRoundFP<INV, COL, LE, 1, TILE>(s, T, S0, k0, q, w, qinv);
}


struct RowTw {
    double L[12];
    double R[2];
};
__device__ __forceinline__ void rowTwIssue(RowTw& W, const double* __restrict__ gd, const double* __restrict__ rd,
                                           const NttTile& T, uint32_t S0) {
    const uint32_t gid = threadIdx.x;
    const uint32_t row = __builtin_amdgcn_readfirstlane(T.r0 + (gid >> 6));
    const uint32_t rowsLog = __builtin_amdgcn_readfirstlane(T.logn - 8);
#pragma unroll
    for (int t = 0; t < 2; ++t) W.R[t] = rd[((uint32_t)(6 + t) << rowsLog) + row];
#pragma unroll
    for (int r = 0; r < 4; ++r) {
        const uint32_t k0 = 2 * r, logh = 8 - k0 - 2;
        const uint32_t lo = gid & ((1u << logh) - 1);
        const uint32_t hi = (gid >> logh) & ((1u << k0) - 1);
        const uint32_t u = hi * (256u >> k0) + lo;
        const uint32_t x0 = (T.r0 + (gid >> 6)) * 256u + u;
#pragma unroll
        for (int t = 0; t < 2; ++t) {
            const uint32_t k = k0 + t;
            const uint32_t b = r == 3 ? (1u << (S0 + k)) + (u >> (8 - k)) : (1u << (S0 + k)) + (x0 >> (8 - k));
#pragma unroll
            for (int qd = 0; qd < (1 << t); ++qd) W.L[3 * r + (1 << t) - 1 + qd] = gd[b + qd];
        }
    }
}
__device__ __forceinline__ void rowTwFinish(double* PW, const RowTw& W, double q, double qi) {
#pragma unroll
    for (int i = 0; i < 9; ++i) PW[i] = W.L[i];
#pragma unroll
    for (int t = 0; t < 2; ++t) {
        const double rf = W.R[t], rfq = rf * qi;
#pragma unroll
        for (int qd = 0; qd < (1 << t); ++qd) {
            const int i = 9 + (1 << t) - 1 + qd;
            PW[i] = fpMulMod(W.L[i], rf, rfq, q);
        }
    }
}

struct RowPtr {
    const u64* base;
    long long ps, is;
};
struct RowGroup {
    uint32_t P, R;
    sfp_limbs pm;
    RowPtr src, dst, copy, ein, eout;
    uint32_t copyByAlpha;
    uint32_t alpha;
    uint32_t skipEll;
    uint32_t lift, liftPrime;
    uint32_t epi, addMask;
    RowPtr eadd;
    const u64 *tA0, *tA1, *tB0, *tB1;
    RowPtr pre, emul;
    const u64 *k, *kS, *k2, *k2S, *liftSub, *preK, *preKS, *emK, *emKS;
    const u64* cy;
    const double *cmD, *cmQ, *chD, *chQ;
    const u64* cmI;
    uint32_t cRows, cBig;
    const u64 *postK, *postKS;
    const double *postD, *postQ;
    const struct MdColArgs* md;
    uint32_t icol;
    const u64 *iTw, *iTwS;
    const double* iTwD;
};

template <class T, int NG>
struct ArgSet {
    T a[NG];
    uint32_t start[NG];
    uint32_t inter;
};
template <class T, int NG>
__device__ __forceinline__ uint32_t argSel(const ArgSet<T, NG>& S, uint32_t& row) {
    const uint32_t y = blockIdx.y;
    if (NG == 1) {
        row = y;
        return 0;
    }
    if (S.inter) {
        row = y / NG;
        return y % NG;
    }
    uint32_t sel = 0;
#pragma unroll
    for (int i = 1; i < NG; ++i)
        if (y >= S.start[i]) sel = (uint32_t)i;
    row = y - S.start[sel];
    return sel;
}
template <int NG>
using RowGroupSet = ArgSet<RowGroup, NG>;

__device__ __forceinline__ u64* rowAt(const RowPtr& r, uint32_t p, uint32_t i) {
    return const_cast<u64*>(r.base) + p * r.ps + i * r.is;
}

#ifdef SFHE_NTT_TRACE
constexpr int kTraceSlots = 256;
__device__ unsigned long long g_nttTrace[kTraceSlots][4][8];
__device__ unsigned long long g_mdrsTrace[kTraceSlots][8];
#define NTT_MARK(i)                                                          \
    {                                                                        \
        const unsigned long long t_ = clock64();                             \
        tacc[(i)] += t_ - tprev;                                             \
        tprev = t_;                                                          \
    }
#else
#define NTT_MARK(i)
#endif

template <bool INV, bool COL, int LE, int TILE, int NG = 1, bool CONV = false, bool ICOL = false>
__global__ __launch_bounds__(TILE >> LE) void k_ntt(const RowGroupSet<NG> GS, const sf_barrett* __restrict__ bar,
                                                  const u64* __restrict__ tw, const u64* __restrict__ twS,
                                                  const u64* __restrict__ ninv,
                                                  const u64* __restrict__ ninvS, uint32_t logn,
                                                  const double* __restrict__ twD,
                                                  const double* __restrict__ qinvD,
                                                  const double* __restrict__ ninvD,
                                                  const double* __restrict__ ninvQ, int useFp,
                                                  const double* __restrict__ rowD) {
    __shared__ u64 s[TILE];
    __shared__ u64 tW[COL ? kNttColTw : 1], tX[COL ? kNttColTw : 1];
    __shared__ u64 tWi[ICOL ? kNttColTw : 1], tXi[ICOL ? kNttColTw : 1];
    static_assert(!ICOL || (!INV && COL && !CONV), "the inverse COL prologue feeds the forward COL pass");
#ifdef SFHE_NTT_TRACE
    unsigned long long tprev = clock64(), tacc[6] = {0, 0, 0, 0, 0, 0};
#endif
    constexpr bool FIRST = (COL != INV);
    const uint32_t n = 1u << logn;
    const uint32_t logR = logn - 8;
    uint32_t rid;
    const RowGroup& G = GS.a[argSel(GS, rid)];
    const uint32_t pp = rid / G.R, ii = rid % G.R;
    if (G.skipEll && ii >= G.alpha * pp && ii < min(G.alpha * (pp + 1), G.skipEll)) return;
    const uint32_t prime = primeOf(G.pm, ii);
    NttTile T;
    T.logn = logn;
    T.d = COL ? logR : 8u;
    T.logC = COL ? (uint32_t)__builtin_ctz(TILE) - logR : 0u;
    T.C = 1u << T.logC;
    const uint32_t tile = (gridDim.x & 7) ? blockIdx.x : (blockIdx.x & 7) * (gridDim.x >> 3) + (blockIdx.x >> 3);
    T.c0 = COL ? tile * T.C : 0u;
    T.r0 = COL ? 0u : tile * (TILE / 256);
    const uint32_t S0 = COL ? 0u : logR;
    constexpr int NT = TILE >> LE, NPAIR = (1 << LE) / 2;

    const u64* in = FIRST ? rowAt(G.src, pp, ii) : rowAt(G.dst, pp, ii);
    const u64* pre = FIRST && G.pre.base ? rowAt(G.pre, pp, ii) : nullptr;
    const bool epi = !FIRST && G.epi;
    const u64* ein = epi ? rowAt(G.ein, pp, ii) : nullptr;
    auto tileOff = [&](int k) -> size_t {
        const uint32_t e = 2 * (threadIdx.x + k * NT);
        return COL ? (size_t)(e >> T.logC) * 256 + T.c0 + (e & (T.C - 1)) : (size_t)T.r0 * 256 + e;
    };
    ulonglong2 xr[NPAIR], mr[NPAIR];
    if constexpr (CONV) {
        static_assert(!INV && COL, "the conversion feeds the forward COL pass");
        const uint32_t ns = min(G.alpha, G.skipEll - pp * G.alpha);
        const u64* yb = G.cy + (size_t)pp * G.alpha * n;
        const size_t tb = (size_t)pp * G.alpha * G.cRows + ii;
        const u64 qc = bar[prime].q;
        const bool big0 = G.cBig && pp == 0;
        constexpr int GRP = 4;
        if (useFp && qc < kFpPrimeBound) {
            const double qd = (double)qc, qi = qinvD[prime];
            double acc[2 * NPAIR];
#pragma unroll
            for (int w = 0; w < 2 * NPAIR; ++w) acc[w] = 0.0;
            for (uint32_t s0 = 0; s0 < ns; s0 += GRP) {
                ulonglong2 v[GRP][NPAIR];
#pragma unroll
                for (int g = 0; g < GRP; ++g)
                    if (s0 + g < ns)
#pragma unroll
// ... 180 lines not shown
        for (uint32_t ri = 0; ri < nr; ++ri) {
            const uint32_t r = nr - 1 - ri;
            const uint32_t k0 = LE * r;
            const int b = (int)min((uint32_t)LE, T.d - k0);
            if (fpL)
                nttRoundDynFP<true, true, LE, TILE>(b, reinterpret_cast<double*>(s), T, 0u, k0, qLd,
                                                    reinterpret_cast<const double*>(tWi), qLi);
            else
                nttRoundDyn<true, true, LE, TILE>(b, s, T, 0u, k0, qL, tWi, tXi);
            __syncthreads();
        }
        const u64 niL = ninv[lp], niLS = ninvS[lp];
        const double niLD = ninvD[lp], niLQ = ninvQ[lp];
#pragma unroll
        for (int k = 0; k < NPAIR; ++k) {
            const uint32_t e = 2 * (threadIdx.x + k * NT);
#pragma unroll
            for (int h = 0; h < 2; ++h) {
                u64 v = s[ldsSw(e + h)];
                if (fpL) {
                    v = d2u(fpReduce(fpMulMod(__longlong_as_double(v), niLD, niLQ, qLd), qLd, qLi));
                } else {
                    v = sf_mul_shoup_lazy(v, niL, niLS, qL);
                    v = v >= qL ? v - qL : v;
                }
                u64 rr = sf_reduce128(v, 0, &LB);
                if (v > lhalf) rr = sf_sub(rr, lsub, q);
                s[ldsSw(e + h)] = fp ? __double_as_longlong(u2d(rr)) : rr;
            }
        }
        __syncthreads();
    }
    if constexpr (kPfBuild) {
        if (rowPf) {
#pragma unroll
            for (int ri = 0; ri < kPfRounds; ++ri) {
                const int r = INV ? kPfRounds - 1 - ri : ri;
                nttRoundFP<INV, false, 2, 2, TILE, true, 8>(reinterpret_cast<double*>(s), T, S0, 2 * r,
                                                            (double)q, nullptr, qinvD[prime], PW + 3 * r);
                __syncthreads();
                NTT_MARK(1 + ri);
            }
        }
    }
    constexpr bool kColUnrollBuild = COL && LE == 2;
    const bool colUnroll = kColUnrollBuild && fp && T.d == 8u;
    if constexpr (kColUnrollBuild) {
        if (colUnroll) {
#pragma unroll
            for (int ri = 0; ri < 4; ++ri) {
                const int r = INV ? 3 - ri : ri;
                nttRoundFP<INV, true, 2, 2, TILE, false, 8>(reinterpret_cast<double*>(s), T, S0, 2 * r, (double)q,
                                                            reinterpret_cast<const double*>(rw), qinvD[prime]);
                __syncthreads();
                NTT_MARK(1 + ri);
            }
        }
    }
    for (uint32_t ri = 0; ri < ((rowPf || colUnroll) ? 0u : nr); ++ri) {
        const uint32_t r = INV ? nr - 1 - ri : ri;
        const uint32_t k0 = LE * r;
        const int b = (int)min((uint32_t)LE, T.d - k0);
        if (fp)
            nttRoundDynFP<INV, COL, LE, TILE>(b, reinterpret_cast<double*>(s), T, S0, k0, (double)q,
                                              reinterpret_cast<const double*>(rw), qinvD[prime]);
        else
            nttRoundDyn<INV, COL, LE, TILE>(b, s, T, S0, k0, q, rw, rx);
        __syncthreads();
        NTT_MARK(1 + ri);
    }
    const bool scale = INV && COL;
    const bool post = scale && G.postK;
    const u64 ni = post ? G.postK[ii] : scale ? ninv[prime] : 0, niS = post ? G.postKS[ii] : scale ? ninvS[prime] : 0;
    u64* out = epi ? rowAt(G.eout, pp, ii) : rowAt(G.dst, pp, ii);
    const u64 ek = epi ? G.k[ii] : 0, ekS = epi ? G.kS[ii] : 0;
    const u64* ead = epi && G.eadd.base ? rowAt(G.eadd, pp, ii) : nullptr;
    const bool tens = epi && G.tA0;
    const u64 ek2 = (ead || tens) ? G.k2[ii] : 0, ek2S = (ead || tens) ? G.k2S[ii] : 0;
    const u64* emul = epi && G.emul.base ? rowAt(G.emul, pp, ii) : nullptr;
    const bool emK = epi && G.emK;
    const u64 emk = emK ? G.emK[ii] : 0, emkS = emK ? G.emKS[ii] : 0;
    const sf_barrett EB = (emul || tens) ? loadBar(bar, prime) : sf_barrett{};
    const size_t trow = (size_t)ii << logn;
#pragma unroll
    for (int k = 0; k < NPAIR; ++k) {
        const uint32_t e = 2 * (threadIdx.x + k * NT);
        const size_t g = tileOff(k);
        ulonglong2 x;
        x.x = s[ldsSw(e)];
        x.y = s[ldsSw(e + 1)];
        if (fp) {
            const double qd = (double)q, qi = qinvD[prime];
            double a0 = __longlong_as_double(x.x), a1 = __longlong_as_double(x.y);
            if (post) {
                const double pd = G.postD[ii], pq = G.postQ[ii];
                x.x = __double_as_longlong(fpReduce(fpMulMod(a0, pd, pq, qd), qd, qi));
                x.y = __double_as_longlong(fpReduce(fpMulMod(a1, pd, pq, qd), qd, qi));
            } else {
                if (scale) {
                    a0 = fpMulMod(a0, ninvD[prime], ninvQ[prime], qd);
                    a1 = fpMulMod(a1, ninvD[prime], ninvQ[prime], qd);
                }
                x.x = d2u(fpReduce(a0, qd, qi));
                x.y = d2u(fpReduce(a1, qd, qi));
            }
        } else if (!FIRST) {
            if (scale) {
                x.x = sf_mul_shoup_lazy(x.x, ni, niS, q);
                x.y = sf_mul_shoup_lazy(x.y, ni, niS, q);
            } else {
                x.x = x.x >= 2 * q ? x.x - 2 * q : x.x;
                x.y = x.y >= 2 * q ? x.y - 2 * q : x.y;
            }
            x.x = x.x >= q ? x.x - q : x.x;
            x.y = x.y >= q ? x.y - q : x.y;
        }
        if (epi) {
            ulonglong2 a = *reinterpret_cast<const ulonglong2*>(ein + g);
            if (emul) {
                const ulonglong2 m = *reinterpret_cast<const ulonglong2*>(emul + g);
                a.x = bmul(a.x, m.x, EB);
                a.y = bmul(a.y, m.y, EB);
            }
            if (emK) {
                a.x = sf_mul_shoup(a.x, emk, emkS, q);
                a.y = sf_mul_shoup(a.y, emk, emkS, q);
            }
            x.x = sf_mul_shoup(sf_sub(a.x, x.x, q), ek, ekS, q);
            x.y = sf_mul_shoup(sf_sub(a.y, x.y, q), ek, ekS, q);
            if ((G.addMask >> pp) & 1u) {
                const ulonglong2 o = *reinterpret_cast<const ulonglong2*>(out + g);
                x.x = sf_add(x.x, o.x, q);
                x.y = sf_add(x.y, o.y, q);
            }
            if (ead || tens) {
                ulonglong2 o;
                if (tens) {
                    const ulonglong2 a0 = *reinterpret_cast<const ulonglong2*>(G.tA0 + trow + g);
                    const ulonglong2 b0 = *reinterpret_cast<const ulonglong2*>(G.tB0 + trow + g);
                    if (pp == 0) {
                        o.x = bmul(a0.x, b0.x, EB);
                        o.y = bmul(a0.y, b0.y, EB);
                    } else {
                        const ulonglong2 a1 = *reinterpret_cast<const ulonglong2*>(G.tA1 + trow + g);
                        const ulonglong2 b1 = *reinterpret_cast<const ulonglong2*>(G.tB1 + trow + g);
                        Acc t{0, 0}, u{0, 0};
                        macc(t, a0.x, b1.x);
                        macc(t, a1.x, b0.x);
                        macc(u, a0.y, b1.y);
                        macc(u, a1.y, b0.y);
                        o.x = sf_reduce128_acc(t.lo, t.hi, &EB);
                        o.y = sf_reduce128_acc(u.lo, u.hi, &EB);
                    }
                } else {
                    o = *reinterpret_cast<const ulonglong2*>(ead + g);
                }
                x.x = sf_add(x.x, sf_mul_shoup(o.x, ek2, ek2S, q), q);
                x.y = sf_add(x.y, sf_mul_shoup(o.y, ek2, ek2S, q), q);
            }
        }
        *reinterpret_cast<ulonglong2*>(out + g) = x;
    }
    NTT_MARK(5);
#ifdef SFHE_NTT_TRACE
    if (threadIdx.x == 0) {
        auto& slot = g_nttTrace[(blockIdx.x + blockIdx.y * gridDim.x) % kTraceSlots][INV * 2 + COL];
        for (int i = 0; i < 6; ++i) atomicAdd(&slot[i], tacc[i]);
        atomicAdd(&slot[7], 1ull);
    }
#endif
}

#ifndef SFHE_MODUP_TG
#define SFHE_MODUP_TG 4
#endif
constexpr int kModupTg = SFHE_MODUP_TG;
template <int TILE, int NG, int TG>
__global__ __launch_bounds__(TILE >> 2) void k_modup_col(const RowGroupSet<NG> GS, const sf_barrett* __restrict__ bar,
                                                         const u64* __restrict__ tw, const u64* __restrict__ twS,
                                                         const u64* __restrict__, const u64* __restrict__,
                                                         uint32_t logn, const double* __restrict__ twD,
                                                         const double* __restrict__ qinvD,
                                                         const double* __restrict__, const double* __restrict__,
                                                         int useFp, const double* __restrict__) {
    constexpr int LE = 2, NT = TILE >> LE, NPAIR = (1 << LE) / 2;
    __shared__ u64 s[TILE];
    __shared__ u64 tW[kNttColTw], tX[kNttColTw];
    const uint32_t n = 1u << logn;
    const uint32_t logR = logn - 8;
    uint32_t rid;
    const RowGroup& G = GS.a[argSel(GS, rid)];
    const uint32_t RG = (G.R + TG - 1) / TG;
    const uint32_t pp = rid / RG, g0 = (rid % RG) * TG;
    const uint32_t own0 = pp * G.alpha, own1 = min(own0 + G.alpha, G.skipEll);
    bool live[TG];
    bool any = false;
#pragma unroll
    for (int u = 0; u < TG; ++u) {
        const uint32_t ii = g0 + u;
        live[u] = ii < G.R && !(ii >= own0 && ii < own1);
        any = any || live[u];
    }
    if (!any) return;
    NttTile T;
    T.logn = logn;
    T.d = logR;
    T.logC = (uint32_t)__builtin_ctz(TILE) - logR;
    T.C = 1u << T.logC;
    const uint32_t tile = (gridDim.x & 7) ? blockIdx.x : (blockIdx.x & 7) * (gridDim.x >> 3) + (blockIdx.x >> 3);
    T.c0 = tile * T.C;
    T.r0 = 0;
    auto tileOff = [&](int k) -> size_t {
        const uint32_t e = 2 * (threadIdx.x + k * NT);
        return (size_t)(e >> T.logC) * 256 + T.c0 + (e & (T.C - 1));
    };
    const uint32_t ns = own1 - own0;
    const u64* yb = G.cy + (size_t)own0 * n;
    const bool big0 = G.cBig && pp == 0;
    uint32_t prime[TG];
    double qd[TG], qi[TG];
    bool fpT[TG];
    int nfp = 0;
#pragma unroll
    for (int u = 0; u < TG; ++u) {
        prime[u] = primeOf(G.pm, min(g0 + u, G.R - 1));
        const u64 q = bar[prime[u]].q;
        fpT[u] = useFp && q < kFpPrimeBound;
        qd[u] = (double)q;
        qi[u] = qinvD[prime[u]];
        nfp += live[u] && fpT[u];
    }
    double acc[TG][2 * NPAIR];
#pragma unroll
    for (int u = 0; u < TG; ++u)
#pragma unroll
        for (int w = 0; w < 2 * NPAIR; ++w) acc[u][w] = 0.0;
    if (nfp) {
        constexpr int GRP = 4;
        for (uint32_t s0 = 0; s0 < ns; s0 += GRP) {
            ulonglong2 v[GRP][NPAIR];
#pragma unroll
// ... 108 lines not shown
        }
        u64* out = rowAt(G.dst, pp, ii);
#pragma unroll
        for (int k = 0; k < NPAIR; ++k) {
            const uint32_t e = 2 * (threadIdx.x + k * NT);
            ulonglong2 x;
            x.x = s[ldsSw(e)];
            x.y = s[ldsSw(e + 1)];
            if (fp) {
                x.x = d2u(fpReduce(__longlong_as_double(x.x), qd[u], qi[u]));
                x.y = d2u(fpReduce(__longlong_as_double(x.y), qd[u], qi[u]));
            }
            *reinterpret_cast<ulonglong2*>(out + tileOff(k)) = x;
        }
    }
}

constexpr int kNttSmallThreads = 256;
template <bool INV>
__global__ __launch_bounds__(kNttSmallThreads) void k_ntt_small(const RowGroup G, const sf_barrett* __restrict__ bar,
                                                               const u64* __restrict__ tw, const u64* __restrict__ twS,
                                                               const u64* __restrict__ ninv,
                                                               const u64* __restrict__ ninvS, uint32_t logn) {
    __shared__ u64 s[kNttTile];
    const uint32_t n = 1u << logn;
    const uint32_t rid = blockIdx.y;
    const uint32_t pp = rid / G.R, ii = rid % G.R;
    if (G.skipEll && ii >= G.alpha * pp && ii < min(G.alpha * (pp + 1), G.skipEll)) return;
    const uint32_t prime = primeOf(G.pm, ii);
    const u64 q = bar[prime].q;
    const u64* in = rowAt(G.src, pp, ii);
    u64* cp = nullptr;
    if (G.copy.base)
        cp = G.copyByAlpha ? const_cast<u64*>(G.copy.base) + (ii / G.alpha) * G.copy.ps + ii * G.copy.is
                           : rowAt(G.copy, pp, ii);
    const u64* pre = G.pre.base ? rowAt(G.pre, pp, ii) : nullptr;
    const bool preK = G.preK != nullptr;
    const u64 pk = preK ? G.preK[ii] : 0, pkS = preK ? G.preKS[ii] : 0;
    const sf_barrett LB = (G.lift || pre) ? loadBar(bar, prime) : sf_barrett{};
    const u64 lsub = G.lift ? G.liftSub[ii] : 0;
    const u64 lhalf = G.lift ? (bar[G.liftPrime].q >> 1) : 0;
    for (uint32_t x = threadIdx.x; x < n; x += kNttSmallThreads) {
        u64 v = in[x];
        if (cp) cp[x] = v;
        if (pre) v = bmul(v, pre[x], LB);
        if (preK) v = sf_mul_shoup(v, pk, pkS, q);
        if (G.lift) {
            u64 r = sf_reduce128(v, 0, &LB);
            v = v > lhalf ? sf_sub(r, lsub, q) : r;
        }
        s[x] = v;
    }
    __syncthreads();
    const u64* w = tw + (size_t)prime * n;
    const u64* wS = twS + (size_t)prime * n;
    for (uint32_t st = 0; st < logn; ++st) {
        const uint32_t m = INV ? (n >> (st + 1)) : (1u << st);
        const uint32_t t = (n >> 1) / m;
        for (uint32_t b = threadIdx.x; b < n / 2; b += kNttSmallThreads) {
            const uint32_t i = b / t, j = b % t, x = 2 * i * t + j;
            const u64 S = w[m + i], Sp = wS[m + i];
            const u64 U = s[x], V = s[x + t];
            if (INV) {
                s[x] = sf_add(U, V, q);
                s[x + t] = sf_mul_shoup(sf_sub(U, V, q), S, Sp, q);
            } else {
                const u64 VW = sf_mul_shoup(V, S, Sp, q);
                s[x] = sf_add(U, VW, q);
                s[x + t] = sf_sub(U, VW, q);
            }
        }
        __syncthreads();
    }
    const bool epi = G.epi != 0;
    u64* out = epi ? rowAt(G.eout, pp, ii) : rowAt(G.dst, pp, ii);
    const u64* ein = epi ? rowAt(G.ein, pp, ii) : nullptr;
    const u64 ek = epi ? G.k[ii] : 0, ekS = epi ? G.kS[ii] : 0;
    const u64* ead = epi && G.eadd.base ? rowAt(G.eadd, pp, ii) : nullptr;
    const u64 ek2 = ead ? G.k2[ii] : 0, ek2S = ead ? G.k2S[ii] : 0;
    const u64* emul = epi && G.emul.base ? rowAt(G.emul, pp, ii) : nullptr;
    const bool emK = epi && G.emK;
    const u64 emk = emK ? G.emK[ii] : 0, emkS = emK ? G.emKS[ii] : 0;
    const sf_barrett EB = emul ? loadBar(bar, prime) : sf_barrett{};
    for (uint32_t x = threadIdx.x; x < n; x += kNttSmallThreads) {
        u64 v = s[x];
        if (INV) v = sf_mul_shoup(v, ninv[prime], ninvS[prime], q);
        if (epi) {
            u64 a = ein[x];
            if (emul) a = bmul(a, emul[x], EB);
            if (emK) a = sf_mul_shoup(a, emk, emkS, q);
            v = sf_mul_shoup(sf_sub(a, v, q), ek, ekS, q);
            if ((G.addMask >> pp) & 1u) v = sf_add(v, out[x], q);
            if (ead) v = sf_add(v, sf_mul_shoup(ead[x], ek2, ek2S, q), q);
        }
        out[x] = v;
    }
}


enum EwOp { EW_ADD, EW_SUB, EW_NEG, EW_MUL, EW_MULADD, EW_MULC, EW_ADDC };

struct KsArgs {
    const u64* in;
    const u64* inMul;
    const u64* ext;
    long long extStride;
    const u64* key;
    uint32_t keyRows, keyQ;
    u64* acc0;
    u64* acc1;
    const u64* fold0;
    const u64* fold1;
    u64 foldK;
    const u64 *fa0, *fa1, *fb0, *fb1;
    uint32_t ell, Lq, alpha, beta;
    int accum;
    uint32_t invFrom;
    const u64 *itw, *itwS;
    const double* itwD;
};

template <int LE, int TILE, int NG = 1>
__global__ __launch_bounds__(TILE >> LE) void k_ntt_ks(const ArgSet<KsArgs, NG> AS, const sf_barrett* __restrict__ bar,
                                                     const u64* __restrict__ tw, const u64* __restrict__ twS,
                                                     uint32_t logn, const double* __restrict__ twD,
                                                     const double* __restrict__ qinvD, int useFp,
                                                     const double* __restrict__ rowD) {
    __shared__ u64 s[2 * TILE];
    constexpr int NT = TILE >> LE;
    constexpr int NPAIR = (1 << LE) / 2;
    const uint32_t n = 1u << logn;
    const uint32_t logR = logn - 8;
    uint32_t t;
    const KsArgs& A = AS.a[argSel(AS, t)];
    const uint32_t prime = t < A.ell ? t : A.Lq + (t - A.ell);
    const sf_barrett B = loadBar(bar, prime);
    const u64 q = B.q;
    const bool fp = useFp && q < kFpPrimeBound;
    NttTile T;
    T.logn = logn;
    T.d = 8u;
    T.logC = 0;
    T.C = 1;
    const uint32_t tile = (gridDim.x & 7) ? blockIdx.x : (blockIdx.x & 7) * (gridDim.x >> 3) + (blockIdx.x >> 3);
    T.c0 = 0;
    T.r0 = tile * (TILE / 256);
    const uint32_t S0 = logR;
    const u64* gw = fp ? reinterpret_cast<const u64*>(twD) + (size_t)prime * n : tw + (size_t)prime * n;
    const u64* gx = twS + (size_t)prime * n;
    constexpr bool kPfBuild = LE == 2;
    constexpr int kPfRounds = 4;
#ifndef SFHE_KS_PW_LOOP
#define SFHE_KS_PW_LOOP 1
#endif
    auto loadPW = [&](double* PW) {
        if constexpr (kPfBuild) {
            const double* gd = reinterpret_cast<const double*>(gw);
#pragma unroll
            for (int r = 0; r < kPfRounds; ++r) {
                const uint32_t k0 = 2 * r, logh = 8 - k0 - 2;
                const uint32_t lo = threadIdx.x & ((1u << logh) - 1);
                const uint32_t rest = threadIdx.x >> logh;
                const uint32_t hi = rest & ((1u << k0) - 1);
                const uint32_t st = rest >> k0;
                const uint32_t x0 = nttGlobal<false>(T, st, hi * (256u >> k0) + lo);
#pragma unroll
                for (int tt = 0; tt < 2; ++tt) {
                    const uint32_t tb = twIndex<false>(T, S0, k0 + tt, x0);
#pragma unroll
                    for (int qd = 0; qd < (1 << tt); ++qd) PW[3 * r + (1 << tt) - 1 + qd] = gd[tb + qd];
                }
            }
        }
    };
    double PW[kPfBuild ? kPfRounds * 3 : 1];
    if (!SFHE_KS_PW_LOOP && fp) loadPW(PW);
// ... 3457 lines not shown
    if (!ng || ng > SFP_MAC_MULTI_G || !nin || nin > SFP_MAC_MULTI_N) return -1;
    if (!m.count) return 0;
    if (!limbsOk(d, m, "mac_plain2_multi")) return 0;
    PtrListM L;
    std::memset(&L, 0, sizeof L);
    for (uint32_t j = 0; j < nin; ++j) {
        L.a[j] = a0[j];
        L.c[j] = a1[j];
        for (uint32_t g = 0; g < ng; ++g) L.b[g * nin + j] = b[(size_t)g * nin + j];
    }
    for (uint32_t g = 0; g < ng; ++g) {
        L.o0[g] = out0[g];
        L.o1[g] = out1[g];
    }
    const size_t total = (size_t)m.count * d->n;
    const dim3 grid(ewGrid(total / 2));
    switch (ng) {
        case 1: SFP_GO(k_mac_plain2_multi<1>, grid, dim3(kThreads), L, nin, m, d->bar, d->logn, d->qinvD); break;
        case 2: SFP_GO(k_mac_plain2_multi<2>, grid, dim3(kThreads), L, nin, m, d->bar, d->logn, d->qinvD); break;
        case 3: SFP_GO(k_mac_plain2_multi<3>, grid, dim3(kThreads), L, nin, m, d->bar, d->logn, d->qinvD); break;
        case 4: SFP_GO(k_mac_plain2_multi<4>, grid, dim3(kThreads), L, nin, m, d->bar, d->logn, d->qinvD); break;
        case 5: SFP_GO(k_mac_plain2_multi<5>, grid, dim3(kThreads), L, nin, m, d->bar, d->logn, d->qinvD); break;
        case 6: SFP_GO(k_mac_plain2_multi<6>, grid, dim3(kThreads), L, nin, m, d->bar, d->logn, d->qinvD); break;
        case 7: SFP_GO(k_mac_plain2_multi<7>, grid, dim3(kThreads), L, nin, m, d->bar, d->logn, d->qinvD); break;
        default: SFP_GO(k_mac_plain2_multi<8>, grid, dim3(kThreads), L, nin, m, d->bar, d->logn, d->qinvD); break;
    }
    checkLaunch(d, "mac_plain2_multi");
    return 0;
}

void sfp_mac_plain(sfp_dev* d, uint64_t* out, const uint64_t* const* a, const uint64_t* const* b,
                   uint32_t nin, sfp_limbs m) {
    if (!limbsOk(d, m, "mac_plain")) return;
    if (nin > SFP_MAX_WSUM) {
        record(d, "mac_plain", hipErrorInvalidValue);
        return;
    }
    PtrList2 pl;
    for (uint32_t j = 0; j < nin; ++j) {
        pl.a[j] = a[j];
        pl.b[j] = b[j];
    }
    const size_t total = (size_t)m.count * d->n;
    SFP_GO(k_mac_plain, dim3(ewGrid(total)), dim3(kThreads), out, pl, nin, m,
                       d->bar, d->logn);
    checkLaunch(d, "mac_plain");
}

void sfp_automorph(sfp_dev* d, uint64_t* out, const uint64_t* in, uint32_t g, sfp_limbs m) {
    const size_t total = (size_t)m.count * d->n;
    issueY<AutArgs>(d, k_automorph<1>, k_automorph<2>, k_automorph<4>, dim3(ewGrid(total)), AutArgs{out, in, g, m.count});
    checkLaunch(d, "automorph");
}

static u64* scratch(sfp_dev* d, size_t words) {
    std::lock_guard<std::mutex> g(d->scrMu);
    const int l = d->cur;
    if (d->scrWords[l] >= words) return d->scr[l];
    const size_t grow = std::max(words, d->scrWords[l] + d->scrWords[l] / 2);
    u64* p = nullptr;
    if (hipMalloc((void**)&p, grow * 8) != hipSuccess) {
        hipGetLastError();
        p = nullptr;
        if (hipMalloc((void**)&p, words * 8) != hipSuccess) {
            record(d, "scratch allocation", hipErrorOutOfMemory);
            return nullptr;
        }
        d->scrWords[l] = words;
    } else {
        d->scrWords[l] = grow;
    }
    if (d->scr[l]) d->retired.push_back(d->scr[l]);
    d->scr[l] = p;
    return p;
}

void sfp_rescale(sfp_dev* d, uint64_t* out, const uint64_t* in, uint32_t ell, const uint64_t* qlinv,
                 uint32_t npoly, size_t inStride, size_t outStride) {
    sfp_rescale_ext(d, out, in, ell, ell - 1, qlinv, npoly, inStride, outStride);
}

static void rescaleCore(sfp_dev* d, uint64_t* out, const uint64_t* in, uint32_t ell, uint32_t dropPrime,
                        const uint64_t* qlinv, uint32_t npoly, size_t inStride, size_t outStride,
                        const uint64_t* mulRows, const uint64_t* mulK) {
    const uint32_t n = d->n;
    const uint32_t cnt = ell - 1;
    if (cnt > SFP_MAX_LIMBS || ell < 2) {
        record(d, "rescale (limb count)", hipErrorInvalidValue);
        return;
    }
    u64* last = scratch(d, (size_t)npoly * n + (size_t)npoly * cnt * n);
    if (!last) return;
    u64* tmp = last + (size_t)npoly * n;
    RowGroup A = rowsOf(npoly, 1, sfp_limbs{1, 0, dropPrime, 0});
    A.src = RowPtr{in + (size_t)cnt * n, (long long)inStride, 0};
    A.dst = RowPtr{last, (long long)n, 0};
    u64 mk[2 * SFP_MAX_LIMBS + 2];
    const u64* dmk = nullptr;
    if (mulRows) A.pre = RowPtr{mulRows + (size_t)cnt * n, 0, 0};
    if (mulK) {
        for (uint32_t i = 0; i < cnt; ++i) {
            mk[i] = mulK[i];
            mk[cnt + i] = sf_shoup_precomp(mulK[i], d->hbar[i].q);
        }
        mk[2 * cnt] = mulK[cnt];
        mk[2 * cnt + 1] = sf_shoup_precomp(mulK[cnt], d->hbar[dropPrime].q);
        dmk = devConst(d, mk, 2 * cnt + 2);
        A.preK = dmk + 2 * cnt;
        A.preKS = dmk + 2 * cnt + 1;
    }
    const bool icol = icolPath(d, npoly * cnt);
    nttRows(d, A, 1, icol ? 1 : 3);
    RowGroup B = rowsOf(npoly, cnt, sfp_limbs{cnt, cnt, 0, 0});
    B.src = RowPtr{last, (long long)n, 0};
    B.lift = 1;
    B.liftPrime = dropPrime;
    if (icol) {
        B.icol = 1;
        B.iTw = d->ipsi;
        B.iTwS = d->ipsiS;
        B.iTwD = d->ipsiD;
    }
    B.dst = RowPtr{tmp, (long long)cnt * n, (long long)n};
    B.epi = 1;
    B.ein = RowPtr{in, (long long)inStride, (long long)n};
    B.eout = RowPtr{out, (long long)outStride, (long long)n};
    const u64 ql = d->hbar[dropPrime].q;
    u64 kS[SFP_MAX_LIMBS], lsub[SFP_MAX_LIMBS];
    for (uint32_t i = 0; i < cnt; ++i) {
        const u64 q = d->hbar[i].q;
        kS[i] = sf_shoup_precomp(qlinv[i], q);
        lsub[i] = ql % q;
    }
    B.k = devConst(d, qlinv, cnt);
    B.kS = devConst(d, kS, cnt);
    B.liftSub = devConst(d, lsub, cnt);
    if (mulRows) B.emul = RowPtr{mulRows, 0, (long long)n};
    if (mulK) {
        B.emK = dmk;
        B.emKS = dmk + cnt;
    }
    nttRows(d, B, 0);
}

void sfp_rescale_ext(sfp_dev* d, uint64_t* out, const uint64_t* in, uint32_t ell, uint32_t dropPrime,
                     const uint64_t* qlinv, uint32_t npoly, size_t inStride, size_t outStride) {
    rescaleCore(d, out, in, ell, dropPrime, qlinv, npoly, inStride, outStride, nullptr, nullptr);
}

void sfp_mul_const_rescale(sfp_dev* d, uint64_t* out, const uint64_t* in, const uint64_t* k, uint32_t ell,
                           const uint64_t* qlinv, uint32_t npoly, size_t inStride, size_t outStride) {
    rescaleCore(d, out, in, ell, ell - 1, qlinv, npoly, inStride, outStride, nullptr, k);
}

void sfp_mul_rescale(sfp_dev* d, uint64_t* out, const uint64_t* in, const uint64_t* m, uint32_t ell,
                     const uint64_t* qlinv, uint32_t npoly, size_t inStride, size_t outStride) {
    rescaleCore(d, out, in, ell, ell - 1, qlinv, npoly, inStride, outStride, m, nullptr);
}

sfp_conv* sfp_upload_conv(sfp_dev* d, uint32_t ns, const uint32_t* src, uint32_t nt,
                          const uint32_t* dst, const uint32_t* drow, const uint64_t* inv,
                          const uint64_t* mod) {
    if (ns > (uint32_t)kMaxConvSrc) {
        record(d, "upload_conv (too many source primes)", hipErrorInvalidValue);
        return nullptr;
    }
    auto* c = new sfp_conv;
    c->ns = ns;
    c->nt = nt;
    c->hsrc.assign(src, src + ns);
    c->hdst.assign(dst, dst + nt);
    c->hinv.assign(inv, inv + ns);
    c->hmod.assign(mod, mod + (size_t)ns * nt);
    for (uint32_t t = 0; t < nt; ++t) c->hrow.push_back(drow ? drow[t] : t);
    bool ok = true;
    auto dmalloc = [&](auto*& dp, size_t bytes) {
        if (!ok) return;
        if (hipMalloc((void**)&dp, bytes + 8) != hipSuccess) {
            hipGetLastError();
            dp = nullptr;
            ok = false;
        }
    };
    dmalloc(c->src, ns * 4);
    dmalloc(c->dst, nt * 4);
    dmalloc(c->inv, ns * 8);
    dmalloc(c->mod, (size_t)ns * nt * 8);
    dmalloc(c->drow, nt * 4);
    dmalloc(c->sprod, nt * 8);
    if (!ok) {
        record(d, "upload_conv allocation", hipErrorOutOfMemory);
        sfp_free_conv(d, c);
        return nullptr;
    }
    std::vector<uint32_t> rows(nt);
    for (uint32_t t = 0; t < nt; ++t) rows[t] = drow ? drow[t] : t;
    hostToDev(d, c->drow, rows.data(), nt * 4);
    hostToDev(d, c->src, src, ns * 4);
    hostToDev(d, c->dst, dst, nt * 4);
    hostToDev(d, c->inv, inv, ns * 8);
    hostToDev(d, c->mod, mod, (size_t)ns * nt * 8);
    std::vector<u64> sp(nt);
    for (uint32_t t = 0; t < nt; ++t) {
        const sf_barrett& B = d->hbar[dst[t]];
        u64 r = 1;
        for (uint32_t i = 0; i < ns; ++i) r = sf_mul(r, d->hbar[src[i]].q % B.q, &B);
        sp[t] = r;
    }
    hostToDev(d, c->sprod, sp.data(), nt * 8);
    for (uint32_t t = 0; t < nt; ++t)
        (d->hbar[dst[t]].q < kFpPrimeBound ? c->hFpT : c->hIntT).push_back(t);
    std::vector<uint32_t> bigs;
    for (uint32_t i = 0; i < ns; ++i)
        if (d->hbar[src[i]].q >= kFpPrimeBound) bigs.push_back(i);
    c->nbig = (uint32_t)bigs.size();
    c->fpOk = bigs.size() <= (size_t)kMaxConvBig;
    const size_t nf = c->hFpT.size();
    std::vector<double> invD(ns), invQ(ns), vD(ns * nf + 1), vQ(ns * nf + 1), hD(kMaxConvBig * nf + 1, 0.0),
        hQ(kMaxConvBig * nf + 1, 0.0);
    for (uint32_t i = 0; i < ns; ++i) {
        invD[i] = (double)inv[i];
        invQ[i] = (double)inv[i] / (double)d->hbar[src[i]].q;
        for (size_t k = 0; k < nf; ++k) {
            const uint32_t t = c->hFpT[k];
            const u64 m = mod[(size_t)i * nt + t];
// ... 537 lines not shown
        pd[r] = (double)k;
        pq[r] = (double)k / (double)B.q;
    }
    A.postK = devConst(d, pk, rows);
    A.postKS = devConst(d, pks, rows);
    A.postD = reinterpret_cast<const double*>(devConst(d, reinterpret_cast<const u64*>(pd), rows));
    A.postQ = reinterpret_cast<const double*>(devConst(d, reinterpret_cast<const u64*>(pq), rows));
    MdColArgs a;
    std::memset(&a, 0, sizeof a);
    a.sidx = c->src;
    a.invD = c->invD;
    a.invQ = c->invQ;
    a.mD = c->mdD;
    a.mQ = c->mdQ;
    a.mI = c->mod;
    a.sprod = c->sprod;
    a.spD = c->mdSpD;
    a.spQ = c->mdSpQ;
    a.ns = c->ns;
    a.nt = c->nt;
    a.l = l;
    a.rs = rs ? 1u : 0u;
    if (rs) {
        double pd[SFP_MAX_LIMBS], pq[SFP_MAX_LIMBS];
        for (uint32_t i = 0; i < l; ++i) {
            pd[i] = (double)pmod[i];
            pq[i] = (double)pmod[i] / (double)d->hbar[i].q;
        }
        a.pmod = devConst(d, pmod, l);
        a.lsub = devConst(d, lsub, l);
        a.pmD = reinterpret_cast<const double*>(devConst(d, reinterpret_cast<const u64*>(pd), l));
        a.pmQ = reinterpret_cast<const double*>(devConst(d, reinterpret_cast<const u64*>(pq), l));
        a.pinvl = pinvl;
    }
    static_assert(sizeof(MdColArgs) % 8 == 0, "MdColArgs in 8-byte words");
    return reinterpret_cast<const MdColArgs*>(devConst(d, reinterpret_cast<const u64*>(&a), sizeof a / 8));
}

void sfp_moddown2(sfp_dev* d, uint64_t* out0, uint64_t* out1, uint64_t* acc, size_t accStride,
                  uint32_t ell, uint32_t K, uint32_t Lq, const sfp_conv* c, const uint64_t* pinv,
                  int add0, int add1, uint64_t* scr, int rowDone) {
    const uint32_t n = d->n;
    if (ell > SFP_MAX_LIMBS) {
        record(d, "moddown (too many limbs)", hipErrorInvalidValue);
        return;
    }
    u64* pRows = acc + (size_t)ell * n;
    RowGroup A = rowsOf(2, K, sfp_limbs{K, 0, Lq, 0});
    A.src = A.dst = RowPtr{pRows, (long long)accStride, (long long)n};
    const MdColArgs* md = mdColArgs(d, c, ell, false, 0, Lq, nullptr, nullptr, 0, A);
    nttRows(d, A, 1, rowDone ? 2 : 3);
    if (!md) {
        ConvJobs J;
        J.j[0] = convJob(c, scr, pRows, ell, 1);
        J.j[1] = convJob(c, scr + (size_t)ell * n, pRows + accStride, ell, 1);
        convLaunch(d, J, 2, c->fpOk);
    }
    RowGroup B = rowsOf(2, ell, sfp_limbs{ell, ell, 0, 0});
    B.src = B.dst = RowPtr{scr, (long long)ell * n, (long long)n};
    if (md) {
        B.md = md;
        B.copy = RowPtr{pRows, (long long)accStride, (long long)n};
        B.cRows = c->ns;
    }
    B.epi = 1;
    B.addMask = (add0 ? 1u : 0u) | (add1 ? 2u : 0u);
    B.ein = RowPtr{acc, (long long)accStride, (long long)n};
    B.eout = RowPtr{out0, (long long)(out1 - out0), (long long)n};
    u64 kS[SFP_MAX_LIMBS];
    for (uint32_t i = 0; i < ell; ++i) kS[i] = sf_shoup_precomp(pinv[i], d->hbar[i].q);
    B.k = devConst(d, pinv, ell);
    B.kS = devConst(d, kS, ell);
    nttRows(d, B, 0);
}

static bool mdrsiOn() {
    static const bool on = [] {
        const char* v = std::getenv("SFHE_MDRSI");
        return !v || *v != '0';
    }();
    return on;
}

static void moddownRescaleCore(sfp_dev* d, uint64_t* out0, uint64_t* out1, const uint64_t* d0, const uint64_t* d1,
                               const uint64_t* const* T, uint64_t* acc, size_t accStride, uint32_t ell, uint32_t K,
                               uint32_t Lq, const sfp_conv* c, const uint64_t* pinv, const uint64_t* pmod,
                               const uint64_t* qlinv, uint64_t* scr, int rowDone) {
    const uint32_t n = d->n, l = ell - 1;
    if (ell < 2 || ell > SFP_MAX_LIMBS || !c || c->ns > (uint32_t)kMaxConvSrc || c->nt < ell ||
        !limbsOk(d, sfp_limbs{K + 1, 1, Lq, l}, "moddown_rescale")) {
        record(d, "moddown_rescale", hipErrorInvalidValue);
        return;
    }
    RowGroup A = rowsOf(2, K + 1, sfp_limbs{K + 1, 1, Lq, l});
    A.src = A.dst = RowPtr{acc + (size_t)l * n, (long long)accStride, (long long)n};
    MdrsArgs M;
    std::memset(&M, 0, sizeof M);
    for (int p = 0; p < 2; ++p) {
        const u64* ap = acc + (size_t)p * accStride;
        M.j[p] = MdrsJob{ap + (size_t)ell * n, ap, scr + (size_t)p * l * n};
    }
    u64 lsub[SFP_MAX_LIMBS], k1[SFP_MAX_LIMBS], k1S[SFP_MAX_LIMBS], k2S[SFP_MAX_LIMBS];
    const u64 ql = d->hbar[l].q;
    for (uint32_t i = 0; i < l; ++i) {
        const u64 q = d->hbar[i].q;
        lsub[i] = ql % q;
        k1[i] = (u64)((unsigned __int128)pinv[i] * qlinv[i] % q);
        k1S[i] = sf_shoup_precomp(k1[i], q);
        k2S[i] = sf_shoup_precomp(qlinv[i], q);
    }
    const MdColArgs* md = mdColArgs(d, c, l, true, l, Lq, pmod, lsub, pinv[l], A);
    nttRows(d, A, 1, rowDone ? 2 : 3);
    if (!md) {
        M.sidx = c->src;
        M.inv = c->inv;
        M.mod = c->mod;
        M.sprod = c->sprod;
        M.pmod = devConst(d, pmod, l);
        M.lsub = devConst(d, lsub, l);
        M.pinvl = pinv[l];
        M.ns = c->ns;
        M.nt = c->nt;
        M.l = l;
        const auto lpos = std::lower_bound(c->hFpT.begin(), c->hFpT.end(), l);
        const bool fp = nttFp() && c->fpOk && c->nbig == 0 && lpos != c->hFpT.end() && *lpos == l;
        uint32_t zc = (l + kConvChunk - 1) / kConvChunk;
        if (fp) {
            M.fpT = c->fpT;
            M.intT = c->intT;
            M.invD = c->invD;
            M.invQ = c->invQ;
            M.vD = c->vD;
            M.vQ = c->vQ;
            M.nFpAll = (uint32_t)c->hFpT.size();
            M.lD = c->vD + (lpos - c->hFpT.begin());
            M.lQ = c->vQ + (lpos - c->hFpT.begin());
            M.nFp = (uint32_t)(lpos - c->hFpT.begin());
            M.nInt = (uint32_t)(std::lower_bound(c->hIntT.begin(), c->hIntT.end(), l) - c->hIntT.begin());
            double pd[SFP_MAX_LIMBS], pq[SFP_MAX_LIMBS];
            for (uint32_t i = 0; i < l; ++i) {
                pd[i] = (double)pmod[i];
                pq[i] = (double)pmod[i] / (double)d->hbar[i].q;
            }
            M.pmodD = reinterpret_cast<const double*>(devConst(d, reinterpret_cast<const u64*>(pd), l));
            M.pmodQ = reinterpret_cast<const double*>(devConst(d, reinterpret_cast<const u64*>(pq), l));
            zc = (M.nFp + kConvChunk - 1) / kConvChunk +
             (mdrsIntFolded(false, M.nFp, M.nInt) ? 0 : (M.nInt + kConvChunk - 1) / kConvChunk);
        }
        const bool bigl = !fp && nttFp() && c->fpOk && c->nbig == 0 && d->hbar[l].q >= kFpPrimeBound &&
                          (c->hFpT.empty() || c->hFpT.front() > l);
        if (bigl) {
            M.intT = c->intT;
            M.invD = c->invD;
            M.invQ = c->invQ;
            M.nFp = 0;
            M.nFpAll = (uint32_t)c->hFpT.size();
            M.nInt = (uint32_t)(std::lower_bound(c->hIntT.begin(), c->hIntT.end(), l) - c->hIntT.begin());
            zc = (M.nInt + kConvChunk - 1) / kConvChunk;
        }
        const dim3 g((fp || bigl || mdrsiOn()) ? n / kConvCoefs : n / (2 * kThreads), 2, zc);
        timedLaunch(d, SFP_FAM_CONV, 8.0 * n * 2 * (K + 1 + l), [&] {
            MdrsKern k = (bigl && c->ns <= 13) ? k_mdrsf<13, true>
                         : (bigl && c->ns <= 16) ? k_mdrsf<16, true>
                         : bigl                  ? k_mdrsf<kMaxConvSrc, true>
                         : (fp && c->ns <= 13)   ? k_mdrsf<13>
                         : (fp && c->ns <= 16)   ? k_mdrsf<16>
                         : fp                    ? k_mdrsf<kMaxConvSrc>
                         : !mdrsiOn()            ? k_conv_mdrs
                         : c->ns <= 16           ? k_mdrsi<16>
                                                 : k_mdrsi<kMaxConvSrc>;
            StackRec r;
            r.go = [=](hipStream_t s_) { hipLaunchKernelGGL(k, g, dim3(kThreads), 0, s_, M, d->bar, d->qinvD, d->logn); };
            if (d->stackOn) {
                auto P = std::make_shared<MdrsPay>();
                P->M = M;
                P->g = g;
                P->k = reinterpret_cast<ConvKern>(k);
                r.cls = STK_MDRS;
                r.key = stkKey((const void*)k, g.x, g.z);
                r.pay = std::move(P);
            }
            issueRec(d, std::move(r));
        });
        checkLaunch(d, "conv_mdrs");
    }
    RowGroup B = rowsOf(2, l, sfp_limbs{l, l, 0, 0});
    B.src = B.dst = RowPtr{scr, (long long)l * n, (long long)n};
    if (md) {
        B.md = md;
        B.copy = RowPtr{acc + (size_t)ell * n, (long long)accStride, (long long)n};
        B.pre = RowPtr{acc + (size_t)l * n, (long long)accStride, (long long)n};
        B.cRows = c->ns + 1;
    }
    B.epi = 1;
    B.ein = RowPtr{acc, (long long)accStride, (long long)n};
    B.eout = RowPtr{out0, (long long)(out1 - out0), (long long)n};
    if (T) {
        B.tA0 = T[0];
        B.tA1 = T[1];
        B.tB0 = T[2];
        B.tB1 = T[3];
    } else {
        B.eadd = RowPtr{d0, (long long)(d1 - d0), (long long)n};
    }
    B.k = devConst(d, k1, l);
    B.kS = devConst(d, k1S, l);
    B.k2 = devConst(d, qlinv, l);
    B.k2S = devConst(d, k2S, l);
    nttRows(d, B, 0);
}

void sfp_moddown_rescale(sfp_dev* d, uint64_t* out0, uint64_t* out1, const uint64_t* d0,
                         const uint64_t* d1, uint64_t* acc, size_t accStride, uint32_t ell,
                         uint32_t K, uint32_t Lq, const sfp_conv* c, const uint64_t* pinv,
                         const uint64_t* pmod, const uint64_t* qlinv, uint64_t* scr, int rowDone) {
    moddownRescaleCore(d, out0, out1, d0, d1, nullptr, acc, accStride, ell, K, Lq, c, pinv, pmod, qlinv, scr,
                       rowDone);
}

int sfp_mult_relin_rescale(sfp_dev* d, uint64_t* out0, uint64_t* out1, const uint64_t* a0, const uint64_t* a1,
                           const uint64_t* b0, const uint64_t* b1, uint32_t ell, uint32_t K, uint32_t Lq,
                           uint32_t alpha, const sfp_conv* const* convs, const uint64_t* key, const sfp_conv* c,
                           const uint64_t* pinv, const uint64_t* pmod, const uint64_t* qlinv, uint64_t* acc,
                           uint64_t* ext, uint64_t* scr) {
    const uint32_t beta = (ell + alpha - 1) / alpha;
    if (!ksFuse() || d->n <= (uint32_t)kNttTile) return -1;
    if (ell < 2 || beta > (uint32_t)kMaxConvJobs || ell + K > SFP_MAX_LIMBS) {
        record(d, "mult_relin_rescale (too many digits / limbs)", hipErrorInvalidValue);
        return 0;
    }
    const uint64_t* T[4] = {a0, a1, b0, b1};
    modupInnerCore(d, acc, acc + (size_t)(ell + K) * d->n, a1, b1, ell, K, Lq, alpha, convs, key, nullptr, nullptr,
                   T, pmod[ell - 1], 0, ell - 1, ext, scr);
    moddownRescaleCore(d, out0, out1, nullptr, nullptr, T, acc, (size_t)(ell + K) * d->n, ell, K, Lq, c, pinv, pmod,
                       qlinv, scr, 1);
    return 0;
}

void sfp_sample_uniform(sfp_dev* d, uint64_t* p, sfp_limbs m, uint64_t seed) {
    if (!limbsOk(d, m, "uniform")) return;
    const size_t total = (size_t)m.count * d->n;
    SFP_GO(k_uniform, dim3(ewGrid(total)), dim3(kThreads), p, m, seed, d->bar,
                       d->logn);
    checkLaunch(d, "uniform");
}

void sfp_load_i64(sfp_dev* d, uint64_t* p, const int64_t* c, sfp_limbs m) {
    if (!limbsOk(d, m, "load_i64")) return;
    syncAll(d);
    std::memcpy(d->bounce, c, (size_t)d->n * 8);
    SFP_GO(k_load_i64, dim3(ewGrid(d->n)), dim3(kThreads), p,
                       (const int64_t*)d->bounce, m, d->bar, d->logn);
    checkLaunch(d, "load_i64");
}



constexpr uint32_t kEncTile = 2048;

__device__ __forceinline__ void encButterfly(double2& a, double2& b, uint32_t j, uint32_t len, const u64* rot,
                                             const double2* ksi, u64 M) {
#pragma clang fp contract(off)
    const u64 lenq = (u64)len << 2;
    const u64 idx = (lenq - (rot[j] & (lenq - 1))) * (M / lenq);
    const double2 k = ksi[idx];
    const double2 u = make_double2(a.x + b.x, a.y + b.y);
    const double dre = a.x - b.x, dim = a.y - b.y;
    const double wre = dre * k.x - dim * k.y;
    const double wim = dre * k.y + dim * k.x;
    a = u;
    b = make_double2(wre, wim);
}

__global__ __launch_bounds__(kThreads) void k_enc_load(double2* __restrict__ v, const double* __restrict__ vals,
                                                       uint32_t nvals, int real, uint32_t S) {
    v += (size_t)blockIdx.y * S;
    if (vals) vals += (size_t)blockIdx.y * nvals * (real ? 1 : 2);
    for (uint32_t i = blockIdx.x * kThreads + threadIdx.x; i < S; i += gridDim.x * kThreads) {
        double2 x = make_double2(0.0, 0.0);
        if (i < nvals) x = real ? make_double2(vals[i], 0.0) : make_double2(vals[2 * i], vals[2 * i + 1]);
        v[i] = x;
    }
}

__global__ __launch_bounds__(kThreads) void k_enc_stage(double2* __restrict__ v, uint32_t S, uint32_t len,
                                                        const u64* __restrict__ rot,
                                                        const double2* __restrict__ ksi, u64 M) {
    v += (size_t)blockIdx.y * S;
    const uint32_t lenh = len >> 1;
    for (uint32_t t = blockIdx.x * kThreads + threadIdx.x; t < S / 2; t += gridDim.x * kThreads) {
        const uint32_t j = t % lenh, i = (t / lenh) * len;
        double2 a = v[i + j], b = v[i + j + lenh];
        encButterfly(a, b, j, len, rot, ksi, M);
        v[i + j] = a;
        v[i + j + lenh] = b;
    }
}

__global__ __launch_bounds__(kThreads) void k_enc_tile(double2* __restrict__ v, uint32_t T,
                                                       const u64* __restrict__ rot, const double2* __restrict__ ksi,
                                                       u64 M) {
    __shared__ double2 sh[kEncTile];
    double2* g = v + (size_t)blockIdx.y * gridDim.x * T + (size_t)blockIdx.x * T;
    for (uint32_t i = threadIdx.x; i < T; i += kThreads) sh[i] = g[i];
    __syncthreads();
    for (uint32_t len = T; len >= 2; len >>= 1) {
        const uint32_t lenh = len >> 1;
        for (uint32_t t = threadIdx.x; t < T / 2; t += kThreads) {
            const uint32_t j = t % lenh, i = (t / lenh) * len;
            double2 a = sh[i + j], b = sh[i + j + lenh];
            encButterfly(a, b, j, len, rot, ksi, M);
            sh[i + j] = a;
            sh[i + j + lenh] = b;
        }
        __syncthreads();
    }
    for (uint32_t i = threadIdx.x; i < T; i += kThreads) g[i] = sh[i];
}
// ... 322 lines not shown
```

### sorting-fhe_amd/csrc/prims.h

```cpp
#pragma once
#include <stddef.h>
#include <stdint.h>

#ifdef __cplusplus
extern "C" {
#endif

#define SFP_MAX_LIMBS 96
#define SFP_MAX_WSUM 80

typedef struct sfp_dev sfp_dev;

typedef struct {
    uint32_t count;
    uint32_t split;
    uint32_t pbase;
    uint32_t base;
    uint32_t stride;
} sfp_limbs;

static inline uint32_t sfp_prime_of(sfp_limbs m, uint32_t i) {
    const uint32_t st = m.stride ? m.stride : 1;
    return i < m.split ? m.base + i * st : m.pbase + (i - m.split) * st;
}
// ... 46 lines not shown

void sfp_mac_plain(sfp_dev* d, uint64_t* out, const uint64_t* const* a, const uint64_t* const* b,
                   uint32_t nin, sfp_limbs m);
void sfp_mac_plain2(sfp_dev* d, uint64_t* out0, uint64_t* out1, const uint64_t* const* a0,
                    const uint64_t* const* a1, const uint64_t* const* b, uint32_t nin, sfp_limbs m);
#define SFP_MAC_MULTI_G 8
#define SFP_MAC_MULTI_N 32
int sfp_mac_plain2_multi(sfp_dev* d, uint64_t* const* out0, uint64_t* const* out1, const uint64_t* const* a0,
                         const uint64_t* const* a1, const uint64_t* const* b, uint32_t nin, uint32_t ng,
                         sfp_limbs m);

void sfp_automorph(sfp_dev* d, uint64_t* out, const uint64_t* in, uint32_t galois, sfp_limbs m);

void sfp_rescale(sfp_dev* d, uint64_t* out, const uint64_t* in, uint32_t ell, const uint64_t* qlinv,
                 uint32_t npoly, size_t in_stride, size_t out_stride);
void sfp_rescale_ext(sfp_dev* d, uint64_t* out, const uint64_t* in, uint32_t ell,
                     uint32_t drop_prime, const uint64_t* qlinv, uint32_t npoly, size_t in_stride,
                     size_t out_stride);

void sfp_mul_const_rescale(sfp_dev* d, uint64_t* out, const uint64_t* in, const uint64_t* k,
                           uint32_t ell, const uint64_t* qlinv, uint32_t npoly, size_t in_stride,
                           size_t out_stride);
void sfp_mul_rescale(sfp_dev* d, uint64_t* out, const uint64_t* in, const uint64_t* m, uint32_t ell,
                     const uint64_t* qlinv, uint32_t npoly, size_t in_stride, size_t out_stride);

sfp_conv* sfp_upload_conv(sfp_dev* d, uint32_t ns, const uint32_t* src_idx, uint32_t nt,
                          const uint32_t* dst_idx, const uint32_t* dst_row,
                          const uint64_t* shat_inv, const uint64_t* shat_mod);
void sfp_free_conv(sfp_dev* d, sfp_conv* c);
void sfp_conv_apply(sfp_dev* d, uint64_t* dst, const uint64_t* src, const sfp_conv* c);
void sfp_conv_apply_centered(sfp_dev* d, uint64_t* dst, const uint64_t* src, const sfp_conv* c,
                             uint32_t nt_use);

void sfp_modup(sfp_dev* d, uint64_t* ext, const uint64_t* in, uint32_t ell, uint32_t K,
               uint32_t Lq, uint32_t alpha, const sfp_conv* const* convs, uint64_t* scratch);

int sfp_modup_inner(sfp_dev* d, uint64_t* acc0, uint64_t* acc1, const uint64_t* in, uint32_t ell, uint32_t K,
                    uint32_t Lq, uint32_t alpha, const sfp_conv* const* convs, const uint64_t* key,
                    const uint64_t* fold0, const uint64_t* fold1, uint64_t fold_k, int accum, uint32_t inv_from,
                    uint64_t* ext, uint64_t* scratch);
int sfp_modup_inner_phase(sfp_dev* d, uint64_t* acc0, uint64_t* acc1, const uint64_t* in, uint32_t ell, uint32_t K,
                          uint32_t Lq, uint32_t alpha, const sfp_conv* const* convs, const uint64_t* key,
                          const uint64_t* fold0, const uint64_t* fold1, uint64_t fold_k, int accum,
                          uint32_t inv_from, uint64_t* ext, uint64_t* scratch, int phases);

void sfp_modup_prepare(sfp_dev* d, const sfp_conv* const* convs, uint32_t ell, uint32_t K, uint32_t alpha);

void sfp_ks_inner(sfp_dev* d, uint64_t* acc0, uint64_t* acc1, const uint64_t* ext,
                  size_t ext_stride, const uint64_t* key, uint32_t beta, uint32_t ell, uint32_t K,
                  uint32_t Lq);
void sfp_ks_inner_aut(sfp_dev* d, uint64_t* acc0, uint64_t* acc1, const uint64_t* ext,
                      size_t ext_stride, const uint64_t* key, uint32_t beta, uint32_t ell, uint32_t K,
                      uint32_t Lq, uint32_t gal);
void sfp_ks_inner_mul(sfp_dev* d, uint64_t* acc0, uint64_t* acc1, const uint64_t* ext,
                      size_t ext_stride, const uint64_t* key, uint32_t beta, uint32_t ell, uint32_t K,
                      uint32_t Lq, const uint64_t* pm, int accum);
void sfp_ks_inner_mul_aut(sfp_dev* d, uint64_t* acc0, uint64_t* acc1, const uint64_t* ext,
                          size_t ext_stride, const uint64_t* key, uint32_t beta, uint32_t ell, uint32_t K,
                          uint32_t Lq, const uint64_t* pm, int accum, uint32_t gal);
void sfp_ks_inner_acc(sfp_dev* d, uint64_t* acc0, uint64_t* acc1, const uint64_t* ext,
                      size_t ext_stride, const uint64_t* key, uint32_t beta, uint32_t ell, uint32_t K,
                      uint32_t Lq);

void sfp_moddown2(sfp_dev* d, uint64_t* out0, uint64_t* out1, uint64_t* acc, size_t acc_stride,
                  uint32_t ell, uint32_t K, uint32_t Lq, const sfp_conv* c, const uint64_t* pinv,
                  int add0, int add1, uint64_t* scratch, int row_done);

void sfp_ks_inner_fold(sfp_dev* d, uint64_t* acc0, uint64_t* acc1, const uint64_t* ext,
                       size_t ext_stride, const uint64_t* key, uint32_t beta, uint32_t ell,
                       uint32_t K, uint32_t Lq, const uint64_t* fold0, const uint64_t* fold1,
                       uint64_t fold_k);

void sfp_moddown_rescale(sfp_dev* d, uint64_t* out0, uint64_t* out1, const uint64_t* d0,
                         const uint64_t* d1, uint64_t* acc, size_t acc_stride, uint32_t ell,
                         uint32_t K, uint32_t Lq, const sfp_conv* c, const uint64_t* pinv,
                         const uint64_t* pmod, const uint64_t* qlinv, uint64_t* scratch, int row_done);

int sfp_mult_relin_rescale(sfp_dev* d, uint64_t* out0, uint64_t* out1, const uint64_t* a0, const uint64_t* a1,
                           const uint64_t* b0, const uint64_t* b1, uint32_t ell, uint32_t K, uint32_t Lq,
                           uint32_t alpha, const sfp_conv* const* convs, const uint64_t* key, const sfp_conv* c,
                           const uint64_t* pinv, const uint64_t* pmod, const uint64_t* qlinv, uint64_t* acc,
                           uint64_t* ext, uint64_t* scratch);

void sfp_sample_uniform(sfp_dev* d, uint64_t* p, sfp_limbs m, uint64_t seed);
void sfp_load_i64(sfp_dev* d, uint64_t* p, const int64_t* coeffs, sfp_limbs m);

void sfp_encode_setup(sfp_dev* d, const uint64_t* rot, const double* ksi);
void sfp_encode(sfp_dev* d, uint64_t* p, const double* vals, uint32_t nvals, int real, uint32_t slots,
                double scale, sfp_limbs m, uint64_t* scratch);
void sfp_encode_batch(sfp_dev* d, uint64_t* dst, size_t dstStride, const double* vals, uint32_t nvals,
                      uint32_t count, int real, uint32_t slots, double scale, sfp_limbs m, uint64_t* scratch);
void sfp_ntt_batch(sfp_dev* d, uint64_t* p, size_t stride, uint32_t count, sfp_limbs m, int inverse);

#define SFP_MAX_LANES 16
typedef struct sfp_event sfp_event;
int sfp_lanes(sfp_dev* d);
void sfp_set_lane(sfp_dev* d, int lane);
int sfp_get_lane(sfp_dev* d);
sfp_event* sfp_event_record(sfp_dev* d);
void sfp_event_wait(sfp_dev* d, const sfp_event* e);
int sfp_event_done(sfp_dev* d, const sfp_event* e);
void sfp_event_free(sfp_dev* d, sfp_event* e);
void sfp_lane_wait(sfp_dev* d, int waiter, int waitee);

void sfp_stack_begin(sfp_dev* d);
void sfp_stack_end(sfp_dev* d);
void sfp_stack_stats(sfp_dev* d, uint64_t* merged, uint64_t* single);

#define SFP_BATCH_MAX 8
int sfp_batch_begin(sfp_dev* d, uint32_t count);
void sfp_batch_lane(sfp_dev* d, uint32_t i);
void sfp_batch_end(sfp_dev* d);

typedef void (*sfp_host_allgather_fn)(void* user, const void* send, void* recv, size_t bytes);
typedef void (*sfp_host_bcast_fn)(void* user, void* buf, size_t bytes, int root);
int sfp_comm_uid(void* uid128);
int sfp_comm_init_rccl(sfp_dev* d, int rank, int world, const void* uid128);
void sfp_comm_set_host(sfp_dev* d, int rank, int world, sfp_host_allgather_fn ag, sfp_host_bcast_fn bc,
                       void* user);
int sfp_comm_capturable(sfp_dev* d);
void sfp_allgather(sfp_dev* d, const void* send, void* recv, size_t bytes);
void sfp_bcast(sfp_dev* d, void* buf, size_t bytes, int root);

int sfp_group_init_rccl(sfp_dev* d, int group, int groups, const void* uid128);
void sfp_group_set_host(sfp_dev* d, int group, int groups, sfp_host_allgather_fn ag, void* user);
void sfp_group_allgather(sfp_dev* d, const void* send, void* recv, size_t bytes);

void sfp_comm_stats_reset(sfp_dev* d, int timed);
void sfp_comm_stats(sfp_dev* d, uint64_t* calls, double* bytes, double* ms);

void sfp_gather_rows(sfp_dev* d, uint64_t* dst, const uint64_t* src, const uint32_t* rows, uint32_t count);

void sfp_rescale_rows(sfp_dev* d, uint64_t* out, const uint64_t* in, const uint64_t* last,
                      uint32_t drop_prime, sfp_limbs m, const uint64_t* qlinv, uint32_t npoly,
                      size_t in_stride, size_t out_stride, size_t last_stride);

#define SFP_KEY_ROW_BY_PRIME 0xFFFFFFFFu

typedef struct {
    uint32_t rows, pstart, tail, world, first, lq;
} sfp_key_geom;
void sfp_set_key_geom(sfp_dev* d, const sfp_key_geom* g);
static inline uint32_t sfp_key_row(const sfp_key_geom* g, uint32_t p) {
    if (!g->rows) return p;
    return p < g->tail ? p : p < g->lq ? g->tail + (p - g->first) / g->world : g->pstart + (p - g->lq);
}
void sfp_ks_inner_map(sfp_dev* d, uint64_t* acc0, uint64_t* acc1, const uint64_t* ext,
                      size_t ext_stride, const uint64_t* key, uint32_t beta, sfp_limbs pm,
                      uint32_t keyQ, uint32_t key_rows, int accum);

typedef struct sfp_graph sfp_graph;
int sfp_capture_begin(sfp_dev* d);
void sfp_clear_error(sfp_dev* d);
sfp_graph* sfp_capture_end(sfp_dev* d);
int sfp_capturing(sfp_dev* d);
void sfp_graph_launch(sfp_dev* d, sfp_graph* g);
size_t sfp_graph_nodes(const sfp_graph* g);
int sfp_graph_family_time(sfp_dev* d, sfp_graph* g, uint32_t fam, int reps, double* ms, uint64_t* launches,
                          double* bytes);
void sfp_graph_destroy(sfp_dev* d, sfp_graph* g);

enum { SFP_FAM_NTT = 0, SFP_FAM_CONV = 1, SFP_FAM_KSINNER = 2, SFP_FAM_NTTKS = 3, SFP_FAM_COUNT = 4, SFP_FAM_ALL = 5 };
void sfp_prof_set(sfp_dev* d, uint32_t fam, uint32_t period);
int sfp_prof_read(sfp_dev* d, uint32_t fam, uint64_t* launches, uint64_t* timed, double* ms,
                  double* bytes);
void sfp_serialize(sfp_dev* d, int on);
// ... 5 lines not shown
```

Before: 1.918 million cmp/s.

## Fuse ciphertext/constant additions into mult-relin-rescale and rescale epilogues

Adds fused multiply-add entry points that fold a following ciphertext or constant addition into the moddown/rescale epilogue of homomorphic multiplication. Paterson-Stockmeyer power generation, tree nodes and the wave scheduler now use them. Linear weighted sums also absorb their constant term into the rescale. The aim is to remove separate elementwise add kernels and their extra passes over memory. In exchange, the recursive path skips lane splitting when folding, which may reduce stream parallelism.

```diff
diff --git a/sorting-fhe_amd/csrc/core/chebyshev.cpp b/sorting-fhe_amd/csrc/core/chebyshev.cpp
--- a/sorting-fhe_amd/csrc/core/chebyshev.cpp
+++ b/sorting-fhe_amd/csrc/core/chebyshev.cpp
@@ -45,6 +45,7 @@
 namespace {
 
 using Ct = Ciphertext<DCRTPoly>;
+using Addend = CryptoContextImpl<DCRTPoly>::MultAddend;
 
 struct Val {
     bool isConst = true;
@@ -74,6 +75,22 @@
                 as.push_back(doubled(j / 2));
                 bs.push_back(j % 2 == 0 ? T[j / 2] : T[j / 2 + 1]);
             }
+            uint32_t top = 0;
+            for (size_t i = 0; i < as.size(); ++i) top = std::max(top, std::max(as[i]->GetLevel(), bs[i]->GetLevel()) + 1);
+            if (psFma() && top <= cc->GetMultiplicativeDepth()) {
+                std::vector<Addend> adds;
+                for (uint32_t j = lo; j <= hi; ++j) {
+                    const uint32_t lv = std::max(as[j - lo]->GetLevel(), bs[j - lo]->GetLevel()) + 1;
+                    adds.push_back(j % 2 == 0 ? Addend{nullptr, 1, -1.0} : Addend{atLevel(1, lv), -1, 0.0});
+                }
+                if (psWaves()) {
+                    auto ts = cc->EvalMultManyAdd(as, bs, adds);
+                    for (uint32_t j = lo; j <= hi; ++j) T[j] = ts[j - lo];
+                } else {
+                    for (uint32_t j = lo; j <= hi; ++j) T[j] = cc->EvalMultAdd(as[j - lo], bs[j - lo], adds[j - lo]);
+                }
+                continue;
+            }
             std::vector<Ct> prods;
             if (psWaves()) {
                 prods = cc->EvalMultMany(as, bs);
@@ -94,6 +111,7 @@
         std::map<uint32_t, std::vector<size_t>> byLevel;
         for (size_t i = 0; i < leaves.size(); ++i) byLevel[leaves[i].second].push_back(i);
         pre.assign(leaves.size(), nullptr);
+        preConst.assign(leaves.size(), 0);
         for (auto& kv : byLevel) {
             const uint32_t L = kv.first;
             std::vector<uint32_t> js;
@@ -116,15 +134,21 @@
             }
             for (size_t b0 = 0; b0 < kv.second.size(); b0 += 64) {
                 std::vector<std::vector<double>> w;
+                std::vector<double> c0;
                 const size_t b1 = std::min(kv.second.size(), b0 + 64);
                 for (size_t t = b0; t < b1; ++t) {
                     const auto& pl = leaves[kv.second[t]].first;
                     std::vector<double> row;
                     for (uint32_t j : js) row.push_back(j < pl.size() ? pl[j] : 0.0);
                     w.push_back(std::move(row));
-                }
-                auto cts = cc->LinearWSumRescaleMulti(ins0, ins1, w, L, T[1]->GetSlots(), &sc);
-                for (size_t t = b0; t < b1; ++t) pre[kv.second[t]] = cts[t - b0];
+                    c0.push_back(pl[0]);
+                }
+                bool added = false;
+                auto cts = cc->LinearWSumRescaleMulti(ins0, ins1, w, L, T[1]->GetSlots(), &sc, &c0, &added);
+                for (size_t t = b0; t < b1; ++t) {
+                    pre[kv.second[t]] = cts[t - b0];
+                    preConst[kv.second[t]] = added;
+                }
             }
         }
         nextLeaf = 0;
@@ -145,18 +169,25 @@
         if (half) cc->SetLane(lane + half);
         Val qv = eval(q, depth - 1, Lp - 1, half ? lane + half : lane, half ? half : 1);
         const Ct& TM = alignedPower(M, Lp - 1);
-        Val out;
+        const bool fold = !half && psFma() && !qv.isConst;
+        Val out, rv;
         out.isConst = false;
-        if (qv.isConst)
-            out.ct = cc->EvalMult(TM, qv.c);
-        else
-            out.ct = cc->EvalMult(qv.ct, TM);
-        if (half) cc->SetLane(lane);
-        Val rv = eval(r, depth, Lp, lane, half ? half : 1);
+        if (fold) {
+            rv = eval(r, depth, Lp, lane, 1);
+            out.ct = cc->EvalMultAdd(qv.ct, TM, rv.isConst ? Addend{nullptr, 1, rv.c} : Addend{rv.ct, 1, 0.0});
+        } else {
+            if (qv.isConst)
+                out.ct = cc->EvalMult(TM, qv.c);
+            else
+                out.ct = cc->EvalMult(qv.ct, TM);
+            if (half) cc->SetLane(lane);
+            rv = eval(r, depth, Lp, lane, half ? half : 1);
+        }
         if (std::getenv("SFHE_PS_DEBUG"))
             std::fprintf(stderr, "PSNODE deg %u M %u | q %s lvl %d | TM lvl %u | prod lvl %u | r %s lvl %d\n", deg, M,
                          qv.isConst ? "const" : "ct", qv.isConst ? -1 : (int)qv.ct->GetLevel(), TM->GetLevel(),
                          out.ct->GetLevel(), rv.isConst ? "const" : "ct", rv.isConst ? -1 : (int)rv.ct->GetLevel());
+        if (fold) return out;
         if (rv.isConst) {
             if (rv.c != 0.0) out.ct = cc->EvalAdd(out.ct, rv.c);
         } else {
@@ -200,7 +231,9 @@
             for (auto& w : waves) {
                 const Ct& TM = alignedPower(w.first.first, w.first.second - 1);
                 std::vector<Ct> as, bs;
+                std::vector<Addend> adds;
                 std::vector<size_t> which;
+                bool anyAdd = false;
                 for (size_t i : w.second) {
                     Node& nd = nodes[i];
                     if (nd.q.isConst) {
@@ -211,11 +244,21 @@
                     as.push_back(value(nd.q));
                     bs.push_back(TM);
                     which.push_back(i);
-                }
-                auto prods = cc->EvalMultMany(as, bs);
+                    const bool fold = psFma() && ready(nd.r);
+                    adds.push_back(!fold ? Addend{} : nd.r.isConst ? Addend{nullptr, 1, nd.r.c} : Addend{value(nd.r), 1, 0.0});
+                    nd.sumInProd = fold;
+                    anyAdd = anyAdd || fold;
+                }
+                auto prods = anyAdd ? cc->EvalMultManyAdd(as, bs, adds) : cc->EvalMultMany(as, bs);
                 for (size_t t = 0; t < which.size(); ++t) {
-                    nodes[which[t]].prod = prods[t];
-                    nodes[which[t]].hasProd = true;
+                    Node& nd = nodes[which[t]];
+                    nd.hasProd = true;
+                    if (nd.sumInProd) {
+                        nd.out = prods[t];
+                        nd.hasOut = true;
+                    } else {
+                        nd.prod = prods[t];
+                    }
                 }
                 progress = true;
             }
@@ -251,7 +294,7 @@
         Val q, r;
         uint32_t M = 0, Lp = 0;
         Ct prod, out;
-        bool hasProd = false, hasOut = false;
+        bool hasProd = false, hasOut = false, sumInProd = false;
     };
     std::vector<Node> nodes;
 
@@ -344,7 +387,7 @@
         if (it != giant.end()) return it->second;
         const Ct& half = power(M / 2);
         const Ct twice = cc->EvalAdd(half, half);
-        return giant[i] = cc->EvalAdd(cc->EvalMult(twice, half), -1.0);
+        return giant[i] = cc->EvalMultAdd(twice, half, Addend{nullptr, 1, -1.0});
     }
 
     const Ct& doubled(uint32_t j) {
@@ -378,8 +421,9 @@
             Val out;
             out.isConst = false;
             out.ct = pre[nextLeaf];
+            const bool constIn = preConst[nextLeaf];
             pre[nextLeaf++] = nullptr;
-            if (p[0] != 0.0) out.ct = cc->EvalAdd(out.ct, p[0]);
+            if (p[0] != 0.0 && !constIn) out.ct = cc->EvalAdd(out.ct, p[0]);
             return out;
         }
         const int lv = leafSumLevel(p, want);
@@ -399,20 +443,28 @@
         }
         Val out;
         out.isConst = false;
-        out.ct = cc->LinearWSumRescale(ins0, ins1, w, (uint32_t)lv, T[1]->GetSlots(), &sc);
-        if (p[0] != 0.0) out.ct = cc->EvalAdd(out.ct, p[0]);
+        out.ct = cc->LinearWSumRescale(ins0, ins1, w, (uint32_t)lv, T[1]->GetSlots(), &sc, p[0]);
         return out;
     }
 
     CryptoContextImpl<DCRTPoly>* cc;
     uint32_t l, k, D;
     std::vector<Ct> pre;
+    std::vector<char> preConst;
     size_t nextLeaf = 0;
     std::vector<Ct> T;
     std::map<uint32_t, Ct> giant;
     std::map<std::pair<uint32_t, uint32_t>, Ct> aligned, alignedPow;
     std::map<uint32_t, Ct> twice;
 };
+
+void psDebugCounts(const CryptoContextImpl<DCRTPoly>* cc, const char* where) {
+    if (!std::getenv("SFHE_PS_DEBUG")) return;
+    uint64_t sums = 0, consts = 0, pairs = 0;
+    cc->FusedSumCounts(&sums, &consts, &pairs);
+    std::fprintf(stderr, "PSFMA %s | fused sums %llu | fused constants %llu | paired weighted sums %llu\n", where,
+                 (unsigned long long)sums, (unsigned long long)consts, (unsigned long long)pairs);
+}
 
 }
 
@@ -493,6 +545,7 @@
     if (out->GetLevel() > target)
         SFHE_THROW("internal: Chebyshev evaluation exceeded OpenFHE depth");
     if (out->GetLevel() < target) out = AdjustLevel(out, target);
+    psDebugCounts(this, "EvalChebyshevSeriesPS");
     return out;
 }
 
@@ -549,8 +602,8 @@
         w.push_back(p[j]);
         sc.push_back(pw[j]->scale);
     }
-    auto out = LinearWSumRescale(i0, i1, w, lev, x->GetSlots(), &sc);
-    if (p[0] != 0.0) out = EvalAdd(out, p[0]);
+    auto out = LinearWSumRescale(i0, i1, w, lev, x->GetSlots(), &sc, p[0]);
+    psDebugCounts(this, "EvalPolyLinear");
     return out;
 }
 
diff --git a/sorting-fhe_amd/csrc/core/context.cpp b/sorting-fhe_amd/csrc/core/context.cpp
--- a/sorting-fhe_amd/csrc/core/context.cpp
+++ b/sorting-fhe_amd/csrc/core/context.cpp
@@ -439,7 +439,7 @@
     }
 
     static Ct rescale(CC* cc, const uint64_t* c0, const uint64_t* c1, uint32_t level,
-                      uint32_t slots) {
+                      uint32_t slots, const uint64_t* cst = nullptr, bool* cstDone = nullptr) {
         SfheContextState* s = cc->st.get();
         uint32_t ell = s->ellOf(level);
         if (ell < 2) SFHE_THROW("no levels left to rescale (multiplicative depth exhausted)");
@@ -447,6 +447,10 @@
         if (c1 - c0 < 0) SFHE_THROW("internal: layout");
         if (s->shardAt(ell))
             rescaleShard(s, out->c0, c0, ell, 2, (size_t)(c1 - c0), (size_t)(out->c1 - out->c0));
+        else if (cst && sfp_rescale_add &&
+                 sfp_rescale_add(s->dev, out->c0, c0, ell, s->qInvTable[ell].data(), 2, (size_t)(c1 - c0),
+                                 (size_t)(out->c1 - out->c0), cst) == 0)
+            *cstDone = true;
         else
             sfp_rescale(s->dev, out->c0, c0, ell, s->qInvTable[ell].data(), 2, (size_t)(c1 - c0),
                         (size_t)(out->c1 - out->c0));
@@ -844,8 +848,29 @@
         s->countBytes((3.0 * ell + 2.0 * beta * (ell + K)) * n * 8);
     }
 
+    struct Fma {
+        const uint64_t *r0 = nullptr, *r1 = nullptr;
+        int sign = 1;
+        const uint64_t* cst = nullptr;
+        bool done = false;
+        explicit operator bool() const { return r0 || cst; }
+    };
+
+    static void countFused(SfheContextState* s, const CC::MultAddend& add, uint32_t ell) {
+        if (add.r) {
+            s->fusedSums++;
+            s->stats.add++;
+            s->countBytes(6.0 * ell * s->n * 8);
+        }
+        if (add.c != 0.0) {
+            s->fusedConsts++;
+            s->stats.add++;
+            s->countBytes(4.0 * ell * s->n * 8);
+        }
+    }
+
     static Ct relinRescale(CC* cc, uint64_t* d0, uint64_t* d1, const uint64_t* d2, uint32_t level,
-                           uint32_t slots) {
+                           uint32_t slots, Fma* f = nullptr) {
         SfheContextState* s = cc->st.get();
         const uint32_t ell = s->ellOf(level);
         if (ell < 2) SFHE_THROW("no levels left to rescale (multiplicative depth exhausted)");
@@ -862,9 +887,16 @@
         const int rowDone = modupInner(cc, acc->ptr, d2, ell, key, d0, d1, s->pModQof(tier)[ell - 1], 0, ell - 1);
         Ct out = newCt(cc, level + 1, slots);
         auto scratch = s->alloc((size_t)2 * (ell - 1) * n);
-        sfp_moddown_rescale(s->dev, out->c0, out->c1, d0, d1, acc->ptr, stride, ell, K, s->Lq,
-                            s->moddownConvOf(tier), s->pInvModQof(tier), s->pModQof(tier),
-                            s->qInvTable[ell].data(), scratch->ptr, rowDone);
+        if (f && *f && sfp_moddown_rescale_add &&
+            sfp_moddown_rescale_add(s->dev, out->c0, out->c1, d0, d1, acc->ptr, stride, ell, K, s->Lq,
+                                    s->moddownConvOf(tier), s->pInvModQof(tier), s->pModQof(tier),
+                                    s->qInvTable[ell].data(), scratch->ptr, rowDone, f->r0, f->r1, f->sign,
+                                    f->cst) == 0)
+            f->done = true;
+        else
+            sfp_moddown_rescale(s->dev, out->c0, out->c1, d0, d1, acc->ptr, stride, ell, K, s->Lq,
+                                s->moddownConvOf(tier), s->pInvModQof(tier), s->pModQof(tier),
+                                s->qInvTable[ell].data(), scratch->ptr, rowDone);
         s->stats.keyswitch++;
         s->stats.rescale++;
         s->countBytes((3.0 * ell + 2.0 * beta * (ell + K)) * n * 8);
@@ -873,7 +905,7 @@
     }
 
     static Ct multRelinRescale(CC* cc, const uint64_t* a0, const uint64_t* a1, const uint64_t* b0,
-                               const uint64_t* b1, uint32_t level, uint32_t slots) {
+                               const uint64_t* b1, uint32_t level, uint32_t slots, Fma* f = nullptr) {
         SfheContextState* s = cc->st.get();
         const uint32_t ell = s->ellOf(level);
         if (ell < 2) SFHE_THROW("no levels left to rescale (multiplicative depth exhausted)");
@@ -888,10 +920,20 @@
             auto ext = s->alloc(stride * beta);
             auto scratch = s->alloc((size_t)2 * ell * n);
             auto& convs = modupConv(cc, ell, tier);
-            if (sfp_mult_relin_rescale(s->dev, out->c0, out->c1, a0, a1, b0, b1, ell, K, s->Lq, s->alpha,
-                                       convs.data(), key->ptr, s->moddownConvOf(tier), s->pInvModQof(tier),
-                                       s->pModQof(tier), s->qInvTable[ell].data(), acc->ptr, ext->ptr,
-                                       scratch->ptr) == 0) {
+            int rc = -1;
+            if (f && *f && sfp_mult_relin_rescale_add) {
+                rc = sfp_mult_relin_rescale_add(s->dev, out->c0, out->c1, a0, a1, b0, b1, ell, K, s->Lq, s->alpha,
+                                                convs.data(), key->ptr, s->moddownConvOf(tier),
+                                                s->pInvModQof(tier), s->pModQof(tier), s->qInvTable[ell].data(),
+                                                acc->ptr, ext->ptr, scratch->ptr, f->r0, f->r1, f->sign, f->cst);
+                if (rc == 0) f->done = true;
+            }
+            if (rc != 0)
+                rc = sfp_mult_relin_rescale(s->dev, out->c0, out->c1, a0, a1, b0, b1, ell, K, s->Lq, s->alpha,
+                                            convs.data(), key->ptr, s->moddownConvOf(tier), s->pInvModQof(tier),
+                                            s->pModQof(tier), s->qInvTable[ell].data(), acc->ptr, ext->ptr,
+                                            scratch->ptr);
+            if (rc == 0) {
                 s->stats.keyswitch++;
                 s->stats.rescale++;
                 s->countBytes((3.0 * ell + 2.0 * beta * (ell + K)) * n * 8);
@@ -904,12 +946,12 @@
         uint64_t* d1 = d0 + pw;
         uint64_t* d2 = d1 + pw;
         sfp_tensor(s->dev, d0, d1, d2, a0, a1, b0, b1, s->qmap(ell));
-        return relinRescale(cc, d0, d1, d2, level, slots);
+        return relinRescale(cc, d0, d1, d2, level, slots, f);
     }
 
     static std::vector<Ct> multRelinRescaleMany(CC* cc, const std::vector<const CiphertextImpl<DCRTPoly>*>& a,
                                                 const std::vector<const CiphertextImpl<DCRTPoly>*>& b, uint32_t level,
-                                                const std::vector<uint32_t>& slots) {
+                                                const std::vector<uint32_t>& slots, std::vector<Fma>* fs = nullptr) {
         SfheContextState* s = cc->st.get();
         const size_t cnt = a.size();
         const uint32_t ell = s->ellOf(level);
@@ -930,11 +972,23 @@
                 auto ext = s->alloc(stride * beta);
                 auto scratch = s->alloc((size_t)2 * ell * n);
                 bs.lane((uint32_t)done);
-                if (sfp_mult_relin_rescale(s->dev, out[done]->c0, out[done]->c1, a[done]->c0, a[done]->c1,
-                                           b[done]->c0, b[done]->c1, ell, K, s->Lq, s->alpha, convs.data(),
-                                           key->ptr, s->moddownConvOf(tier), s->pInvModQof(tier), s->pModQof(tier),
-                                           s->qInvTable[ell].data(), acc->ptr, ext->ptr, scratch->ptr) != 0)
-                    break;
+                Fma* f = fs && (*fs)[done] ? &(*fs)[done] : nullptr;
+                int rc = -1;
+                if (f && sfp_mult_relin_rescale_add) {
+                    rc = sfp_mult_relin_rescale_add(s->dev, out[done]->c0, out[done]->c1, a[done]->c0, a[done]->c1,
+                                                    b[done]->c0, b[done]->c1, ell, K, s->Lq, s->alpha, convs.data(),
+                                                    key->ptr, s->moddownConvOf(tier), s->pInvModQof(tier),
+                                                    s->pModQof(tier), s->qInvTable[ell].data(), acc->ptr, ext->ptr,
+                                                    scratch->ptr, f->r0, f->r1, f->sign, f->cst);
+                    if (rc == 0) f->done = true;
+                }
+                if (rc != 0)
+                    rc = sfp_mult_relin_rescale(s->dev, out[done]->c0, out[done]->c1, a[done]->c0, a[done]->c1,
+                                                b[done]->c0, b[done]->c1, ell, K, s->Lq, s->alpha, convs.data(),
+                                                key->ptr, s->moddownConvOf(tier), s->pInvModQof(tier),
+                                                s->pModQof(tier), s->qInvTable[ell].data(), acc->ptr, ext->ptr,
+                                                scratch->ptr);
+                if (rc != 0) break;
                 s->stats.keyswitch++;
                 s->stats.rescale++;
                 s->countBytes((3.0 * ell + 2.0 * beta * (ell + K)) * n * 8);
@@ -943,7 +997,8 @@
         }
         }
         for (size_t i = done; i < cnt; ++i)
-            out[i] = multRelinRescale(cc, a[i]->c0, a[i]->c1, b[i]->c0, b[i]->c1, level, slots[i]);
+            out[i] = multRelinRescale(cc, a[i]->c0, a[i]->c1, b[i]->c0, b[i]->c1, level, slots[i],
+                                      fs ? &(*fs)[i] : nullptr);
         return out;
     }
 
@@ -2583,6 +2638,129 @@
         }
         auto r = SfheInternal::multRelinRescaleMany(this, pa, pb, A[i]->level, slots);
         for (size_t k = i; k < j; ++k) out[k] = SfheInternal::traced(this, r[k - i], "EvalMult");
+        i = j;
+    }
+    return out;
+}
+
+namespace {
+Ciphertext<DCRTPoly> addAfter(CryptoContextImpl<DCRTPoly>* cc, Ciphertext<DCRTPoly> prod,
+                              const CryptoContextImpl<DCRTPoly>::MultAddend& add) {
+    if (add.r) prod = add.sign < 0 ? cc->EvalSub(prod, add.r) : cc->EvalAdd(prod, add.r);
+    if (add.c != 0.0) prod = cc->EvalAdd(prod, add.c);
+    return prod;
+}
+}
+
+bool CryptoContextImpl<DCRTPoly>::multAddFusable(const Ciphertext<DCRTPoly>& a, const Ciphertext<DCRTPoly>& b,
+                                                 const MultAddend& add) const {
+    SfheContextState* s = st.get();
+    if (!psFma() || !SfheInternal::fusedRescale() || SfheInternal::lazy(s) || !s->relinKey) return false;
+    if (!add.r && add.c == 0.0) return false;
+    if (SfheInternal::isLazy(a) || SfheInternal::isLazy(b)) return false;
+    const uint32_t level = std::max(a->level, b->level);
+    const uint32_t ell = s->ellOf(level);
+    if (ell < 2 || s->shardAt(ell) || level + 1 > s->L) return false;
+    if (add.r) {
+        const auto& r = add.r;
+        if (SfheInternal::isLazy(r) || r->level != level + 1 || r->scale != s->scale[level + 1] ||
+            r->c1 - r->c0 != (ptrdiff_t)s->polyWords(level + 1))
+            return false;
+    }
+    return true;
+}
+
+Ciphertext<DCRTPoly> CryptoContextImpl<DCRTPoly>::EvalMultAdd(const Ciphertext<DCRTPoly>& a0,
+                                                             const Ciphertext<DCRTPoly>& b0,
+                                                             const MultAddend& add) {
+    OpLock g(st.get());
+    if (!multAddFusable(a0, b0, add)) return addAfter(this, EvalMult(a0, b0), add);
+    SfheContextState* s = st.get();
+    SfheInternal::deps(s, {&a0, &b0, &add.r});
+    auto a = a0, b = b0;
+    SfheInternal::align(this, a, b);
+    const uint32_t ell = s->ellOf(a->level), slots = std::max(a->slots, b->slots);
+    s->stats.tensor++;
+    s->countBytes(7.0 * ell * s->n * 8);
+    std::vector<uint64_t> k;
+    SfheInternal::Fma f;
+    if (add.r) {
+        f.r0 = add.r->c0;
+        f.r1 = add.r->c1;
+        f.sign = add.sign;
+    }
+    if (add.c != 0.0) {
+        k = SfheInternal::constResidues(s, add.c * s->scale[a->level + 1], ell - 1);
+        f.cst = k.data();
+    }
+    auto out = SfheInternal::traced(
+        this, SfheInternal::multRelinRescale(this, a->c0, a->c1, b->c0, b->c1, a->level, slots, &f), "EvalMult");
+    if (!f.done) return addAfter(this, out, add);
+    SfheInternal::countFused(s, add, ell - 1);
+    return out;
+}
+
+std::vector<Ciphertext<DCRTPoly>> CryptoContextImpl<DCRTPoly>::EvalMultManyAdd(
+    const std::vector<Ciphertext<DCRTPoly>>& a0, const std::vector<Ciphertext<DCRTPoly>>& b0,
+    const std::vector<MultAddend>& adds) {
+    OpLock g(st.get());
+    SfheContextState* s = st.get();
+    if (a0.size() != b0.size() || a0.size() != adds.size()) SFHE_THROW("operand count mismatch");
+    const size_t cnt = a0.size();
+    std::vector<Ciphertext<DCRTPoly>> out(cnt);
+    if (cnt < 2) {
+        for (size_t i = 0; i < cnt; ++i) out[i] = EvalMultAdd(a0[i], b0[i], adds[i]);
+        return out;
+    }
+    if (!psFma() || !SfheInternal::fusedRescale() || SfheInternal::lazy(s)) {
+        out = EvalMultMany(a0, b0);
+        for (size_t i = 0; i < cnt; ++i) out[i] = addAfter(this, out[i], adds[i]);
+        return out;
+    }
+    if (!s->relinKey) SFHE_THROW("EvalMultKeyGen must be called before EvalMult");
+    std::vector<Ciphertext<DCRTPoly>> A(a0), B(b0);
+    std::vector<char> fuse(cnt);
+    for (size_t i = 0; i < cnt; ++i) {
+        fuse[i] = multAddFusable(a0[i], b0[i], adds[i]);
+        SfheInternal::deps(s, {&a0[i], &b0[i]});
+        if (fuse[i]) SfheInternal::deps(s, {&adds[i].r});
+        SfheInternal::align(this, A[i], B[i]);
+        if (s->ellOf(A[i]->level) < 2) SFHE_THROW("no levels left (multiplicative depth exhausted)");
+        s->stats.tensor++;
+        s->countBytes(7.0 * s->ellOf(A[i]->level) * s->n * 8);
+    }
+    for (size_t i = 0; i < cnt;) {
+        size_t j = i + 1;
+        while (j < cnt && j - i < batchWidth() && A[j]->level == A[i]->level) ++j;
+        const uint32_t level = A[i]->level, ell = s->ellOf(level);
+        std::vector<const CiphertextImpl<DCRTPoly>*> pa, pb;
+        std::vector<uint32_t> slots;
+        std::vector<SfheInternal::Fma> fs(j - i);
+        std::vector<std::vector<uint64_t>> ks(j - i);
+        for (size_t k = i; k < j; ++k) {
+            pa.push_back(A[k].get());
+            pb.push_back(B[k].get());
+            slots.push_back(std::max(A[k]->slots, B[k]->slots));
+            if (!fuse[k]) continue;
+            SfheInternal::Fma& f = fs[k - i];
+            if (adds[k].r) {
+                f.r0 = adds[k].r->c0;
+                f.r1 = adds[k].r->c1;
+                f.sign = adds[k].sign;
+            }
+            if (adds[k].c != 0.0) {
+                ks[k - i] = SfheInternal::constResidues(s, adds[k].c * s->scale[level + 1], ell - 1);
+                f.cst = ks[k - i].data();
+            }
+        }
+        auto r = SfheInternal::multRelinRescaleMany(this, pa, pb, level, slots, &fs);
+        for (size_t k = i; k < j; ++k) {
+            out[k] = SfheInternal::traced(this, r[k - i], "EvalMult");
+            if (fs[k - i].done)
+                SfheInternal::countFused(s, adds[k], ell - 1);
+            else
+                out[k] = addAfter(this, out[k], adds[k]);
+        }
         i = j;
     }
     return out;
@@ -3006,9 +3184,25 @@
 std::vector<Ciphertext<DCRTPoly>> CryptoContextImpl<DCRTPoly>::LinearWSumRescaleMulti(
     const std::vector<const uint64_t*>& in0, const std::vector<const uint64_t*>& in1,
     const std::vector<std::vector<double>>& w, uint32_t level, uint32_t slots, const std::vector<double>* inScale) {
+    return LinearWSumRescaleMulti(in0, in1, w, level, slots, inScale, nullptr, nullptr);
+}
+
+void CryptoContextImpl<DCRTPoly>::FusedSumCounts(uint64_t* sums, uint64_t* consts, uint64_t* pairedWsums) const {
+    OpLock g(st.get());
+    if (sums) *sums = st->fusedSums;
+    if (consts) *consts = st->fusedConsts;
+    if (pairedWsums) *pairedWsums = st->pairedWsums;
+}
+
+std::vector<Ciphertext<DCRTPoly>> CryptoContextImpl<DCRTPoly>::LinearWSumRescaleMulti(
+    const std::vector<const uint64_t*>& in0, const std::vector<const uint64_t*>& in1,
+    const std::vector<std::vector<double>>& w, uint32_t level, uint32_t slots, const std::vector<double>* inScale,
+    const std::vector<double>* constants, bool* constantsAdded) {
     OpLock g(st.get());
     SfheContextState* s = st.get();
     const uint32_t ell = s->ellOf(level), n = s->n;
+    if (constantsAdded) *constantsAdded = false;
+    if (constants && constants->size() != w.size()) SFHE_THROW("LinearWSumRescaleMulti: constant count");
     const uint32_t nin = (uint32_t)in0.size(), nout = (uint32_t)w.size();
     if (ell < 2) SFHE_THROW("no levels left (multiplicative depth exhausted)");
     if (nin == 0 || nin > SFP_MAX_WSUM || nout == 0) SFHE_THROW("LinearWSumRescaleMulti: bad sizes");
@@ -3025,9 +3219,27 @@
                        s->qmap(ell));
     const size_t qw = s->polyWords(level + 1);
     auto res = s->alloc((size_t)nout * 2 * qw);
+    std::vector<uint64_t> cst;
+    uint32_t ncst = 0;
+    if (constants && constantsAdded && psFma() && sfp_rescale_add && !s->shardAt(ell)) {
+        const uint32_t rows = s->rows(ell - 1);
+        cst.assign((size_t)2 * nout * rows, 0);
+        for (uint32_t o = 0; o < nout; ++o) {
+            if ((*constants)[o] == 0.0) continue;
+            auto k = SfheInternal::constResidues(s, (*constants)[o] * s->scale[level + 1], ell - 1);
+            std::copy(k.begin(), k.end(), cst.begin() + (size_t)2 * o * rows);
+            ++ncst;
+        }
+    }
     if (s->shardAt(ell))
         SfheInternal::rescaleShard(s, res->ptr, sums->ptr, ell, 2 * nout, pw, qw);
-    else
+    else if (ncst && sfp_rescale_add(s->dev, res->ptr, sums->ptr, ell, s->qInvTable[ell].data(), 2 * nout, pw, qw,
+                                     cst.data()) == 0) {
+        *constantsAdded = true;
+        s->fusedConsts += ncst;
+        s->stats.add += ncst;
+        s->countBytes(4.0 * (ell - 1) * n * 8 * ncst);
+    } else
         sfp_rescale(s->dev, res->ptr, sums->ptr, ell, s->qInvTable[ell].data(), 2 * nout, pw, qw);
     std::vector<Ciphertext<DCRTPoly>> out(nout);
     for (uint32_t o = 0; o < nout; ++o) {
@@ -3050,11 +3262,20 @@
 Ciphertext<DCRTPoly> CryptoContextImpl<DCRTPoly>::LinearWSumRescale(
     const std::vector<const uint64_t*>& in0, const std::vector<const uint64_t*>& in1,
     const std::vector<double>& w, uint32_t level, uint32_t slots, const std::vector<double>* inScale) {
+    return LinearWSumRescale(in0, in1, w, level, slots, inScale, 0.0);
+}
+
+Ciphertext<DCRTPoly> CryptoContextImpl<DCRTPoly>::LinearWSumRescale(
+    const std::vector<const uint64_t*>& in0, const std::vector<const uint64_t*>& in1,
+    const std::vector<double>& w, uint32_t level, uint32_t slots, const std::vector<double>* inScale,
+    double constant) {
     OpLock g(st.get());
     SfheContextState* s = st.get();
     const uint32_t ell = s->ellOf(level);
     if (ell < 2) SFHE_THROW("no levels left (multiplicative depth exhausted)");
     if (inScale && inScale->size() != w.size()) SFHE_THROW("LinearWSumRescale: scale count");
+    BatchScope pairLanes(this, psFma() && !s->shardAt(ell) ? 2u : 0u);
+    if (pairLanes) s->pairedWsums++;
     const size_t pw = s->polyWords(level);
     auto tmp = s->alloc(2 * pw);
     uint64_t* t0 = tmp->ptr;
@@ -3076,14 +3297,33 @@
             a1.push_back(in1[j]);
             weightResidues(s, w[j], level, ell, kk, inScale ? (*inScale)[j] : 0.0);
         }
+        pairLanes.lane(0);
         sfp_lin_wsum(s->dev, t0, a0.data(), kk.data(), (uint32_t)a0.size(), q);
+        pairLanes.lane(1);
         sfp_lin_wsum(s->dev, t1, a1.data(), kk.data(), (uint32_t)a1.size(), q);
         s->stats.wsum_terms += take;
         s->countBytes((double)(a0.size() + 1) * 2.0 * ell * s->n * 8);
         done += take;
         first = false;
     }
-    return SfheInternal::traced(this, SfheInternal::rescale(this, t0, t1, level, slots), "LinearWSumRescale");
+    pairLanes.end();
+    std::vector<uint64_t> cst;
+    bool cstDone = false;
+    if (constant != 0.0 && psFma() && !s->shardAt(ell)) {
+        cst = SfheInternal::constResidues(s, constant * s->scale[level + 1], ell - 1);
+        cst.resize(2 * cst.size(), 0);
+    }
+    auto out = SfheInternal::traced(
+        this, SfheInternal::rescale(this, t0, t1, level, slots, cst.empty() ? nullptr : cst.data(), &cstDone),
+        "LinearWSumRescale");
+    if (cstDone) {
+        s->fusedConsts++;
+        s->stats.add++;
+        s->countBytes(4.0 * (ell - 1) * s->n * 8);
+    } else if (constant != 0.0) {
+        out = EvalAdd(out, constant);
+    }
+    return out;
 }
 
 
diff --git a/sorting-fhe_amd/csrc/core/openfhe.h b/sorting-fhe_amd/csrc/core/openfhe.h
--- a/sorting-fhe_amd/csrc/core/openfhe.h
+++ b/sorting-fhe_amd/csrc/core/openfhe.h
@@ -309,6 +309,16 @@
     Ciphertext<DCRTPoly> EvalSquare(const Ciphertext<DCRTPoly>& a);
     std::vector<Ciphertext<DCRTPoly>> EvalMultMany(const std::vector<Ciphertext<DCRTPoly>>& a,
                                                    const std::vector<Ciphertext<DCRTPoly>>& b);
+    struct MultAddend {
+        Ciphertext<DCRTPoly> r;
+        int sign = 1;
+        double c = 0.0;
+    };
+    Ciphertext<DCRTPoly> EvalMultAdd(const Ciphertext<DCRTPoly>& a, const Ciphertext<DCRTPoly>& b,
+                                     const MultAddend& add);
+    std::vector<Ciphertext<DCRTPoly>> EvalMultManyAdd(const std::vector<Ciphertext<DCRTPoly>>& a,
+                                                      const std::vector<Ciphertext<DCRTPoly>>& b,
+                                                      const std::vector<MultAddend>& adds);
     Ciphertext<DCRTPoly> EvalMultAddPlain(const std::vector<Ciphertext<DCRTPoly>>& a,
                                           const std::vector<Plaintext>& p);
 
@@ -377,10 +387,19 @@
                                            const std::vector<const uint64_t*>& in1,
                                            const std::vector<double>& w, uint32_t level,
                                            uint32_t slots, const std::vector<double>* inScale = nullptr);
+    Ciphertext<DCRTPoly> LinearWSumRescale(const std::vector<const uint64_t*>& in0,
+                                           const std::vector<const uint64_t*>& in1,
+                                           const std::vector<double>& w, uint32_t level,
+                                           uint32_t slots, const std::vector<double>* inScale, double constant);
     std::vector<Ciphertext<DCRTPoly>> LinearWSumRescaleMulti(
         const std::vector<const uint64_t*>& in0, const std::vector<const uint64_t*>& in1,
         const std::vector<std::vector<double>>& w, uint32_t level, uint32_t slots,
         const std::vector<double>* inScale = nullptr);
+    std::vector<Ciphertext<DCRTPoly>> LinearWSumRescaleMulti(
+        const std::vector<const uint64_t*>& in0, const std::vector<const uint64_t*>& in1,
+        const std::vector<std::vector<double>>& w, uint32_t level, uint32_t slots,
+        const std::vector<double>* inScale, const std::vector<double>* constants, bool* constantsAdded);
+    void FusedSumCounts(uint64_t* sums, uint64_t* consts, uint64_t* pairedWsums) const;
     void Synchronize();
     void Settle(const Ciphertext<DCRTPoly>& ct);
     int LaneCount() const;
@@ -428,6 +447,7 @@
     void CopyCiphertextInto(const Ciphertext<DCRTPoly>& dst, const Ciphertext<DCRTPoly>& src);
 
   private:
+    bool multAddFusable(const Ciphertext<DCRTPoly>& a, const Ciphertext<DCRTPoly>& b, const MultAddend& add) const;
     std::unique_ptr<SfheContextState> st;
     uint32_t enabled = 0;
     BootstrapTap bootTap;
@@ -446,6 +466,10 @@
     explicit operator bool() const { return on_; }
     void lane(uint32_t i) {
         if (on_) cc_->BatchLane(i);
+    }
+    void end() {
+        if (on_) cc_->EndBatch();
+        on_ = false;
     }
 
   private:
diff --git a/sorting-fhe_amd/csrc/core/state.h b/sorting-fhe_amd/csrc/core/state.h
--- a/sorting-fhe_amd/csrc/core/state.h
+++ b/sorting-fhe_amd/csrc/core/state.h
@@ -149,6 +149,7 @@
     bool capturing = false;
     uint64_t captureEpoch = 0, epochCount = 0;
     uint32_t lazyHold = 0;
+    uint64_t fusedSums = 0, fusedConsts = 0, pairedWsums = 0;
     std::set<uint64_t> abandonedEpochs;
     std::vector<std::pair<uint64_t*, size_t>> capAllocs;
     std::unordered_map<uint64_t*, bool> graphOwned;
@@ -228,6 +229,14 @@
     return w;
 }
 
+inline bool psFma() {
+    static const bool on = [] {
+        const char* v = std::getenv("SFHE_PS_FMA");
+        return !v || *v != '0';
+    }();
+    return on;
+}
+
 class OpLock {
   public:
     explicit OpLock(SfheContextState* s) : s_(s), g_(s->opMu) {
diff --git a/sorting-fhe_amd/csrc/hip/prims_hip.hip b/sorting-fhe_amd/csrc/hip/prims_hip.hip
--- a/sorting-fhe_amd/csrc/hip/prims_hip.hip
+++ b/sorting-fhe_amd/csrc/hip/prims_hip.hip
@@ -655,10 +655,19 @@
     const double *cmD, *cmQ, *chD, *chQ;
     const u64* cmI;
     uint32_t cRows, cBig;
-    const u64 *postK, *postKS;
-    const double *postD, *postQ;
+    union {
+        struct {
+            const u64 *postK, *postKS;
+            const double *postD, *postQ;
+        };
+        struct {
+            RowPtr esum;
+            const u64* ecst;
+        };
+    };
     const struct MdColArgs* md;
     uint32_t icol;
+    uint32_t esumNeg;
     const u64 *iTw, *iTwS;
     const double* iTwD;
 };
@@ -689,6 +698,7 @@
 }
 template <int NG>
 using RowGroupSet = ArgSet<RowGroup, NG>;
+static_assert(sizeof(RowGroupSet<8>) + 96 <= 4096, "eight row groups by value exceed the kernel-argument limit");
 
 __device__ __forceinline__ u64* rowAt(const RowPtr& r, uint32_t p, uint32_t i) {
     return const_cast<u64*>(r.base) + p * r.ps + i * r.is;
@@ -1035,6 +1045,8 @@
     const u64 emk = emK ? G.emK[ii] : 0, emkS = emK ? G.emKS[ii] : 0;
     const sf_barrett EB = (emul || tens) ? loadBar(bar, prime) : sf_barrett{};
     const size_t trow = (size_t)ii << logn;
+    const u64* esm = !INV && epi && G.esum.base ? rowAt(G.esum, pp, ii) : nullptr;
+    const u64 ecs = !INV && epi && G.ecst ? G.ecst[pp * G.R + ii] : 0;
 #pragma unroll
     for (int k = 0; k < NPAIR; ++k) {
         const uint32_t e = 2 * (threadIdx.x + k * NT);
@@ -1110,6 +1122,15 @@
                 }
                 x.x = sf_add(x.x, sf_mul_shoup(o.x, ek2, ek2S, q), q);
                 x.y = sf_add(x.y, sf_mul_shoup(o.y, ek2, ek2S, q), q);
+            }
+            if (esm) {
+                const ulonglong2 r = *reinterpret_cast<const ulonglong2*>(esm + g);
+                x.x = G.esumNeg ? sf_sub(x.x, r.x, q) : sf_add(x.x, r.x, q);
+                x.y = G.esumNeg ? sf_sub(x.y, r.y, q) : sf_add(x.y, r.y, q);
+            }
+            if (ecs) {
+                x.x = sf_add(x.x, ecs, q);
+                x.y = sf_add(x.y, ecs, q);
             }
         }
         *reinterpret_cast<ulonglong2*>(out + g) = x;
@@ -1384,6 +1405,8 @@
     const bool emK = epi && G.emK;
     const u64 emk = emK ? G.emK[ii] : 0, emkS = emK ? G.emKS[ii] : 0;
     const sf_barrett EB = emul ? loadBar(bar, prime) : sf_barrett{};
+    const u64* esm = !INV && epi && G.esum.base ? rowAt(G.esum, pp, ii) : nullptr;
+    const u64 ecs = !INV && epi && G.ecst ? G.ecst[pp * G.R + ii] : 0;
     for (uint32_t x = threadIdx.x; x < n; x += kNttSmallThreads) {
         u64 v = s[x];
         if (INV) v = sf_mul_shoup(v, ninv[prime], ninvS[prime], q);
@@ -1394,6 +1417,8 @@
             v = sf_mul_shoup(sf_sub(a, v, q), ek, ekS, q);
             if ((G.addMask >> pp) & 1u) v = sf_add(v, out[x], q);
             if (ead) v = sf_add(v, sf_mul_shoup(ead[x], ek2, ek2S, q), q);
+            if (esm) v = G.esumNeg ? sf_sub(v, esm[x], q) : sf_add(v, esm[x], q);
+            if (ecs) v = sf_add(v, ecs, q);
         }
         out[x] = v;
     }
@@ -5017,7 +5042,7 @@
 
 static void rescaleCore(sfp_dev* d, uint64_t* out, const uint64_t* in, uint32_t ell, uint32_t dropPrime,
                         const uint64_t* qlinv, uint32_t npoly, size_t inStride, size_t outStride,
-                        const uint64_t* mulRows, const uint64_t* mulK) {
+                        const uint64_t* mulRows, const uint64_t* mulK, const uint64_t* cst = nullptr) {
     const uint32_t n = d->n;
     const uint32_t cnt = ell - 1;
     if (cnt > SFP_MAX_LIMBS || ell < 2) {
@@ -5075,7 +5100,14 @@
         B.emK = dmk;
         B.emKS = dmk + cnt;
     }
+    if (cst) B.ecst = devConst(d, cst, (size_t)npoly * cnt);
     nttRows(d, B, 0);
+}
+
+int sfp_rescale_add(sfp_dev* d, uint64_t* out, const uint64_t* in, uint32_t ell, const uint64_t* qlinv,
+                    uint32_t npoly, size_t inStride, size_t outStride, const uint64_t* cst) {
+    rescaleCore(d, out, in, ell, ell - 1, qlinv, npoly, inStride, outStride, nullptr, nullptr, cst);
+    return 0;
 }
 
 void sfp_rescale_ext(sfp_dev* d, uint64_t* out, const uint64_t* in, uint32_t ell, uint32_t dropPrime,
@@ -5779,10 +5811,23 @@
     return on;
 }
 
+struct EpiAdd {
+    const uint64_t *r0 = nullptr, *r1 = nullptr;
+    int sign = 1;
+    const uint64_t* cst = nullptr;
+};
+static void epiAddInto(sfp_dev* d, RowGroup& B, const EpiAdd& e, uint32_t npoly, uint32_t rows) {
+    if (e.r0) {
+        B.esum = RowPtr{e.r0, e.r1 ? (long long)(e.r1 - e.r0) : 0, (long long)d->n};
+        B.esumNeg = e.sign < 0 ? 1u : 0u;
+    }
+    if (e.cst) B.ecst = devConst(d, e.cst, (size_t)npoly * rows);
+}
+
 static void moddownRescaleCore(sfp_dev* d, uint64_t* out0, uint64_t* out1, const uint64_t* d0, const uint64_t* d1,
                                const uint64_t* const* T, uint64_t* acc, size_t accStride, uint32_t ell, uint32_t K,
                                uint32_t Lq, const sfp_conv* c, const uint64_t* pinv, const uint64_t* pmod,
-                               const uint64_t* qlinv, uint64_t* scr, int rowDone) {
+                               const uint64_t* qlinv, uint64_t* scr, int rowDone, const EpiAdd& ea = EpiAdd{}) {
     const uint32_t n = d->n, l = ell - 1;
     if (ell < 2 || ell > SFP_MAX_LIMBS || !c || c->ns > (uint32_t)kMaxConvSrc || c->nt < ell ||
         !limbsOk(d, sfp_limbs{K + 1, 1, Lq, l}, "moddown_rescale")) {
@@ -5904,6 +5949,7 @@
     B.kS = devConst(d, k1S, l);
     B.k2 = devConst(d, qlinv, l);
     B.k2S = devConst(d, k2S, l);
+    epiAddInto(d, B, ea, 2, l);
     nttRows(d, B, 0);
 }
 
@@ -5915,22 +5961,64 @@
                        rowDone);
 }
 
+static int multRelinRescaleCore(sfp_dev* d, uint64_t* out0, uint64_t* out1, const uint64_t* a0, const uint64_t* a1,
+                                const uint64_t* b0, const uint64_t* b1, uint32_t ell, uint32_t K, uint32_t Lq,
+                                uint32_t alpha, const sfp_conv* const* convs, const uint64_t* key, const sfp_conv* c,
+                                const uint64_t* pinv, const uint64_t* pmod, const uint64_t* qlinv, uint64_t* acc,
+                                uint64_t* ext, uint64_t* scr, const EpiAdd& ea) {
+    const uint32_t beta = (ell + alpha - 1) / alpha;
+    if (!ksFuse() || d->n <= (uint32_t)kNttTile) return -1;
+    if (ell < 2 || beta > (uint32_t)kMaxConvJobs || ell + K > SFP_MAX_LIMBS) {
+        record(d, "mult_relin_rescale (too many digits / limbs)", hipErrorInvalidValue);
+        return 0;
+    }
+    const uint64_t* T[4] = {a0, a1, b0, b1};
+    modupInnerCore(d, acc, acc + (size_t)(ell + K) * d->n, a1, b1, ell, K, Lq, alpha, convs, key, nullptr, nullptr,
+                   T, pmod[ell - 1], 0, ell - 1, ext, scr);
+    moddownRescaleCore(d, out0, out1, nullptr, nullptr, T, acc, (size_t)(ell + K) * d->n, ell, K, Lq, c, pinv, pmod,
+                       qlinv, scr, 1, ea);
+    return 0;
+}
+
 int sfp_mult_relin_rescale(sfp_dev* d, uint64_t* out0, uint64_t* out1, const uint64_t* a0, const uint64_t* a1,
                            const uint64_t* b0, const uint64_t* b1, uint32_t ell, uint32_t K, uint32_t Lq,
                            uint32_t alpha, const sfp_conv* const* convs, const uint64_t* key, const sfp_conv* c,
                            const uint64_t* pinv, const uint64_t* pmod, const uint64_t* qlinv, uint64_t* acc,
                            uint64_t* ext, uint64_t* scr) {
-    const uint32_t beta = (ell + alpha - 1) / alpha;
-    if (!ksFuse() || d->n <= (uint32_t)kNttTile) return -1;
-    if (ell < 2 || beta > (uint32_t)kMaxConvJobs || ell + K > SFP_MAX_LIMBS) {
-        record(d, "mult_relin_rescale (too many digits / limbs)", hipErrorInvalidValue);
-        return 0;
-    }
-    const uint64_t* T[4] = {a0, a1, b0, b1};
-    modupInnerCore(d, acc, acc + (size_t)(ell + K) * d->n, a1, b1, ell, K, Lq, alpha, convs, key, nullptr, nullptr,
-                   T, pmod[ell - 1], 0, ell - 1, ext, scr);
-    moddownRescaleCore(d, out0, out1, nullptr, nullptr, T, acc, (size_t)(ell + K) * d->n, ell, K, Lq, c, pinv, pmod,
-                       qlinv, scr, 1);
+    return multRelinRescaleCore(d, out0, out1, a0, a1, b0, b1, ell, K, Lq, alpha, convs, key, c, pinv, pmod, qlinv,
+                                acc, ext, scr, EpiAdd{});
+}
+
+static const uint64_t* cstBoth(const uint64_t* cst, uint32_t rows, uint64_t* buf) {
+    if (!cst) return nullptr;
+    for (uint32_t i = 0; i < rows; ++i) {
+        buf[i] = cst[i];
+        buf[rows + i] = 0;
+    }
+    return buf;
+}
+
+int sfp_mult_relin_rescale_add(sfp_dev* d, uint64_t* out0, uint64_t* out1, const uint64_t* a0, const uint64_t* a1,
+                               const uint64_t* b0, const uint64_t* b1, uint32_t ell, uint32_t K, uint32_t Lq,
+                               uint32_t alpha, const sfp_conv* const* convs, const uint64_t* key, const sfp_conv* c,
+                               const uint64_t* pinv, const uint64_t* pmod, const uint64_t* qlinv, uint64_t* acc,
+                               uint64_t* ext, uint64_t* scr, const uint64_t* r0, const uint64_t* r1, int sign,
+                               const uint64_t* cst) {
+    uint64_t kb[2 * SFP_MAX_LIMBS];
+    if (ell < 2 || ell > SFP_MAX_LIMBS) return -1;
+    return multRelinRescaleCore(d, out0, out1, a0, a1, b0, b1, ell, K, Lq, alpha, convs, key, c, pinv, pmod, qlinv,
+                                acc, ext, scr, EpiAdd{r0, r1, sign, cstBoth(cst, ell - 1, kb)});
+}
+
+int sfp_moddown_rescale_add(sfp_dev* d, uint64_t* out0, uint64_t* out1, const uint64_t* d0, const uint64_t* d1,
+                            uint64_t* acc, size_t accStride, uint32_t ell, uint32_t K, uint32_t Lq,
+                            const sfp_conv* c, const uint64_t* pinv, const uint64_t* pmod, const uint64_t* qlinv,
+                            uint64_t* scr, int rowDone, const uint64_t* r0, const uint64_t* r1, int sign,
+                            const uint64_t* cst) {
+    uint64_t kb[2 * SFP_MAX_LIMBS];
+    if (ell < 2 || ell > SFP_MAX_LIMBS) return -1;
+    moddownRescaleCore(d, out0, out1, d0, d1, nullptr, acc, accStride, ell, K, Lq, c, pinv, pmod, qlinv, scr,
+                       rowDone, EpiAdd{r0, r1, sign, cstBoth(cst, ell - 1, kb)});
     return 0;
 }
 
diff --git a/sorting-fhe_amd/csrc/prims.h b/sorting-fhe_amd/csrc/prims.h
--- a/sorting-fhe_amd/csrc/prims.h
+++ b/sorting-fhe_amd/csrc/prims.h
@@ -152,6 +152,26 @@
                            const uint64_t* pinv, const uint64_t* pmod, const uint64_t* qlinv, uint64_t* acc,
                            uint64_t* ext, uint64_t* scratch);
 
+#if defined(__GNUC__)
+#define SFP_OPTIONAL __attribute__((weak))
+#else
+#define SFP_OPTIONAL
+#endif
+SFP_OPTIONAL int sfp_mult_relin_rescale_add(sfp_dev* d, uint64_t* out0, uint64_t* out1, const uint64_t* a0,
+                                            const uint64_t* a1, const uint64_t* b0, const uint64_t* b1, uint32_t ell,
+                                            uint32_t K, uint32_t Lq, uint32_t alpha, const sfp_conv* const* convs,
+                                            const uint64_t* key, const sfp_conv* c, const uint64_t* pinv,
+                                            const uint64_t* pmod, const uint64_t* qlinv, uint64_t* acc, uint64_t* ext,
+                                            uint64_t* scratch, const uint64_t* r0, const uint64_t* r1, int sign,
+                                            const uint64_t* cst);
+SFP_OPTIONAL int sfp_moddown_rescale_add(sfp_dev* d, uint64_t* out0, uint64_t* out1, const uint64_t* d0,
+                                         const uint64_t* d1, uint64_t* acc, size_t acc_stride, uint32_t ell,
+                                         uint32_t K, uint32_t Lq, const sfp_conv* c, const uint64_t* pinv,
+                                         const uint64_t* pmod, const uint64_t* qlinv, uint64_t* scratch, int row_done,
+                                         const uint64_t* r0, const uint64_t* r1, int sign, const uint64_t* cst);
+SFP_OPTIONAL int sfp_rescale_add(sfp_dev* d, uint64_t* out, const uint64_t* in, uint32_t ell, const uint64_t* qlinv,
+                                 uint32_t npoly, size_t in_stride, size_t out_stride, const uint64_t* cst);
+
 void sfp_sample_uniform(sfp_dev* d, uint64_t* p, sfp_limbs m, uint64_t seed);
 void sfp_load_i64(sfp_dev* d, uint64_t* p, const int64_t* coeffs, sfp_limbs m);
 
```

Result: faster. 1.950 million cmp/s (median of 6 runs) (+1.7%).
